# protocol/vdf

Hardware: AMD Instinct MI355X
Metric: MSM GPoints/s at 2^20 (Pallas, Pedersen-commitment MSM of Nova prove_step); prove_step/s in `prove_step` (higher is better)
Workload: dtype u32

## Files before the change

### bindings/rust/vdf-hip-sys/src/lib.rs

```rust
#![allow(non_camel_case_types, non_snake_case)]
use std::os::raw::{c_char, c_int, c_void};

#[repr(C)] pub struct VdfCtx { _private: [u8; 0] }
#[repr(C)] pub struct VdfBases { _private: [u8; 0] }
#[repr(C)] pub struct VdfShape { _private: [u8; 0] }
#[repr(C)] pub struct VdfMsmJob { _private: [u8; 0] }
#[repr(C)] pub struct VdfPp { _private: [u8; 0] }
#[repr(C)] pub struct VdfCircuits { _private: [u8; 0] }
#[repr(C)] pub struct VdfProof { _private: [u8; 0] }
#[repr(C)] pub struct VdfSnark { _private: [u8; 0] }
#[repr(C)] pub struct VdfCs { _private: [u8; 0] }

#[repr(C)] #[derive(Clone, Copy, Debug, PartialEq, Eq)] pub struct VdfFe { pub l: [u64; 4] }
#[repr(C)] #[derive(Clone, Copy, Debug, PartialEq, Eq)] pub struct VdfAffine { pub x: VdfFe, pub y: VdfFe }
#[repr(C)] #[derive(Clone, Copy, Debug, PartialEq, Eq)] pub struct VdfJac { pub x: VdfFe, pub y: VdfFe, pub z: VdfFe }
#[repr(C)] #[derive(Clone, Copy, Debug, PartialEq, Eq)] pub struct VdfState { pub x: VdfFe, pub y: VdfFe, pub i: VdfFe }
pub type VdfAllgatherFn = Option<unsafe extern "C" fn(user: *mut c_void, send: *const c_void, recv: *mut c_void, bytes: usize, stream: *mut c_void) -> c_int>;
#[repr(C)] #[derive(Clone, Copy)] pub struct VdfStepCircuit { pub arity: usize, pub synthesize: Option<unsafe extern "C" fn(self_: *mut c_void, cs: *mut VdfCs, z_in: *const u32, z_out: *mut u32) -> c_int>, pub self_: *mut c_void }
#[repr(C)] #[derive(Clone, Copy, Debug)] pub struct VdfNovaStepInfo { pub comm_W1: VdfAffine, pub X1: [VdfFe; 2], pub comm_T1: VdfAffine, pub comm_T2: VdfAffine, pub r1: [u64; 4], pub r2: [u64; 4] }
#[repr(C)] #[derive(Clone, Copy, Debug)] pub struct VdfNovaAugInputs { pub params: VdfFe, pub i: VdfFe, pub z0: [VdfFe; 3], pub zi: [VdfFe; 3], pub U_comm_W: VdfAffine, pub U_comm_E: VdfAffine, pub U_u: VdfFe, pub U_X: [VdfFe; 2], pub u_comm_W: VdfAffine, pub u_X: [VdfFe; 2], pub T: VdfAffine }
#[repr(C)] #[derive(Clone, Copy, Debug)] pub struct VdfKernelEvent { pub name: [c_char; 24], pub bytes: f64, pub start_ms: f64, pub end_ms: f64 }
#[repr(C)] #[derive(Clone, Copy, Debug)] pub struct VdfHipTuning { pub struct_size: u32, pub msm_direct: i32, pub direct_priority: i32, pub direct_fused: i32, pub light_priority: i32, pub accumulate_fill: i32, pub accumulate_lds: i32, pub slice_len: i32, pub part_bits: i32, pub reduction: i32, pub reduction_quads: i32, pub heavy_min: i32, pub giant_span: i32, pub nifs_lanes: i32, pub shim_cache: i32, pub nifs_fused: i32, pub fold_u128: i32, pub fixup_serial: i32, pub sort_staged: i32, pub glv: i32 }
#[repr(C)] #[derive(Clone, Copy, Debug)] pub struct VdfNovaTuning { pub struct_size: u32, pub flags: u32, pub digit_budget_bytes: u64, pub digit_window: i32, pub early_rows: i32, pub stencil: i32, pub small_window: i32, pub big_window: i32, pub packed_commit: i32, pub lookahead_early: i32, pub gate_accumulate: i32, pub fold_on_rows: i32, pub nifs_ahead: i32, pub early_row_parts: i32, pub lookahead_priority: i32, pub side_accumulate_fill: i32, pub verbose: i32, pub compress_queues: i32, pub rows_at_challenge: i32, pub fold_fused: i32 }
#[repr(C)] #[derive(Clone, Copy, Debug, PartialEq, Eq)] pub struct VdfNovaRoParams { pub struct_size: u32, pub family: i32, pub width: i32, pub full_rounds: i32, pub partial_rounds: i32, pub alpha: i32, pub challenge_bits: i32, pub hash_bits: i32 }
#[repr(C)] #[derive(Clone, Copy, Debug)] pub struct VdfIpaOpening { pub weight: VdfFe, pub k: c_int, pub log_m: c_int, pub lo: *const VdfFe, pub hi: *const VdfFe, pub pattern: *const VdfFe }

#[link(name = "vdf_hip")]
extern "C" {
    pub fn vdf_ctx_create(device_ids: *const c_int, n_devices: c_int, out: *mut *mut VdfCtx) -> c_int;
    pub fn vdf_ctx_destroy(ctx: *mut VdfCtx);
    pub fn vdf_ctx_create_pooled(device_ids: *const c_int, n_devices: c_int, role: c_int, out: *mut *mut VdfCtx) -> c_int;
    pub fn vdf_ctx_create_pooled_near(parent: *mut VdfCtx, role: c_int, out: *mut *mut VdfCtx) -> c_int;
    pub fn vdf_ctx_queue_info(ctx: *mut VdfCtx, pooled: *mut c_int, sharers: *mut c_int, device_streams: *mut c_int) -> c_int;
    pub fn vdf_ctx_set_stream(ctx: *mut VdfCtx, hip_stream: *mut c_void) -> c_int;
    pub fn vdf_ctx_get_stream(ctx: *mut VdfCtx) -> *mut c_void;
    pub fn vdf_ctx_set_async(ctx: *mut VdfCtx, async_: c_int) -> c_int;
    pub fn vdf_ctx_get_async(ctx: *mut VdfCtx, async_: *mut c_int) -> c_int;
    pub fn vdf_ctx_sync(ctx: *mut VdfCtx) -> c_int;
    pub fn vdf_ctx_device(ctx: *mut VdfCtx) -> c_int;
    pub fn vdf_last_error(ctx: *mut VdfCtx) -> *const c_char;
    pub fn vdf_bases_upload(ctx: *mut VdfCtx, curve: c_int, bases: *const VdfAffine, n: usize, out: *mut *mut VdfBases) -> c_int;
    pub fn vdf_bases_validate(ctx: *mut VdfCtx, bases: *const VdfBases, first_bad: *mut usize) -> c_int;
    pub fn vdf_bases_generate(ctx: *mut VdfCtx, curve: c_int, seed: u64, n: usize, out: *mut *mut VdfBases) -> c_int;
    pub fn vdf_bases_generate_range(ctx: *mut VdfCtx, curve: c_int, seed: u64, start: usize, n: usize, out: *mut *mut VdfBases) -> c_int;
    pub fn vdf_bases_generate_family(ctx: *mut VdfCtx, curve: c_int, family: c_int, seed: u64, start: usize, n: usize, out: *mut *mut VdfBases) -> c_int;
    pub fn vdf_bases_generate_label(ctx: *mut VdfCtx, curve: c_int, label: *const u8, label_len: usize, start: usize, n: usize, out: *mut *mut VdfBases) -> c_int;
    pub fn vdf_bases_precompute(ctx: *mut VdfCtx, bases: *mut VdfBases, window_bits: c_int, sets: c_int) -> c_int;
    pub fn vdf_bases_window(bases: *const VdfBases) -> c_int;
    pub fn vdf_bases_precompute_digits(ctx: *mut VdfCtx, bases: *mut VdfBases, window_bits: c_int, ranges: c_int, begin: *const usize, count: *const usize) -> c_int;
    pub fn vdf_digit_table_bytes(window_bits: c_int, generators: usize) -> usize;
    pub fn vdf_bases_table_bytes(bases: *const VdfBases) -> usize;
    pub fn vdf_bases_digit_window(bases: *const VdfBases) -> c_int;
    pub fn vdf_bases_digit_table_bytes(bases: *const VdfBases) -> usize;
    pub fn vdf_bases_download(ctx: *mut VdfCtx, bases: *const VdfBases, offset: usize, n: usize, out: *mut VdfAffine) -> c_int;
    pub fn vdf_bases_len(bases: *const VdfBases) -> usize;
    pub fn vdf_bases_device_ptr(bases: *const VdfBases) -> *const c_void;
    pub fn vdf_bases_free(bases: *mut VdfBases);
    pub fn vdf_msm(ctx: *mut VdfCtx, bases: *const VdfBases, offset: usize, scalars: *const VdfFe, n: usize, is_mont: c_int, out: *mut VdfJac) -> c_int;
    pub fn vdf_msm_batch(ctx: *mut VdfCtx, bases: *const VdfBases, k: c_int, offset: *const usize, scalars: *const *const VdfFe, n: *const usize, is_mont: c_int, out: *mut VdfJac) -> c_int;
    pub fn vdf_msm_job_begin(ctx: *mut VdfCtx, bases: *const VdfBases, k: c_int, offset: *const usize, n: *const usize, is_mont: c_int, out: *mut *mut VdfMsmJob) -> c_int;
    pub fn vdf_msm_job_push(job: *mut VdfMsmJob, g: c_int, scalars: *const VdfFe) -> c_int;
    pub fn vdf_msm_job_finish(job: *mut VdfMsmJob, out: *mut VdfJac) -> c_int;
    pub fn vdf_ctx_set_msm_window(ctx: *mut VdfCtx, window_bits: c_int) -> c_int;
    pub fn vdf_point_sum(ctx: *mut VdfCtx, curve: c_int, points: *const VdfJac, n: usize, out: *mut VdfJac) -> c_int;
    pub fn vdf_msm_sharded(ctx: *mut VdfCtx, shard_bases: *const VdfBases, offset: usize, shard_scalars: *const VdfFe, n: usize, is_mont: c_int, rank: c_int, world: c_int, gather: VdfAllgatherFn, user: *mut c_void, flags: c_int, partial: *mut VdfJac, gathered: *mut VdfJac, out: *mut VdfJac) -> c_int;
    pub fn vdf_msm_multi(ctxs: *const *mut VdfCtx, bases: *const *const VdfBases, offsets: *const usize, scalars: *const *const VdfFe, n: *const usize, k: c_int, is_mont: c_int, out: *mut VdfJac) -> c_int;
    pub fn vdf_ctx_set_timing(ctx: *mut VdfCtx, enable: c_int) -> c_int;
    pub fn vdf_msm_timing(ctx: *mut VdfCtx, ms: *mut f32, calls: *mut c_int) -> c_int;
    pub fn vdf_ctx_set_kernel_timing(ctx: *mut VdfCtx, enable: c_int) -> c_int;
    pub fn vdf_ctx_kernel_events(ctx: *mut VdfCtx, out: *mut VdfKernelEvent, cap: usize, n: *mut usize) -> c_int;
    pub fn mult_pippenger_pallas(out: *mut VdfJac, points: *const VdfAffine, npoints: usize, scalars: *const VdfFe, is_mont: bool);
    pub fn mult_pippenger_vesta(out: *mut VdfJac, points: *const VdfAffine, npoints: usize, scalars: *const VdfFe, is_mont: bool);
    pub fn vdf_shim_set_cache(entries: c_int) -> c_int;
    pub fn vdf_shape_create(ctx: *mut VdfCtx, field: c_int, num_cons: usize, num_cols: usize, rows: *const *const u32, cols: *const *const u32, vals: *const *const VdfFe, nnz: *const usize, out: *mut *mut VdfShape) -> c_int;
    pub fn vdf_shape_free(shape: *mut VdfShape);
    pub fn vdf_spmv3(ctx: *mut VdfCtx, shape: *const VdfShape, z: *const VdfFe, Az: *mut VdfFe, Bz: *mut VdfFe, Cz: *mut VdfFe) -> c_int;
    pub fn vdf_cross_term(ctx: *mut VdfCtx, field: c_int, Az1: *const VdfFe, Bz1: *const VdfFe, Cz1: *const VdfFe, Az2: *const VdfFe, Bz2: *const VdfFe, Cz2: *const VdfFe, u1: *const VdfFe, n: usize, T: *mut VdfFe) -> c_int;
    pub fn vdf_vec_is_zero(ctx: *mut VdfCtx, v: *const VdfFe, n: usize, is_zero: *mut c_int) -> c_int;
    pub fn vdf_axpy(ctx: *mut VdfCtx, field: c_int, a: *const VdfFe, r: *const VdfFe, b: *const VdfFe, n: usize, out: *mut VdfFe) -> c_int;
    pub fn vdf_minroot_witness(ctx: *mut VdfCtx, field: c_int, trace_xy: *const VdfFe, i0: *const VdfFe, t: u64, W_segment: *mut VdfFe) -> c_int;
    pub fn vdf_minroot_step_z(ctx: *mut VdfCtx, field: c_int, trace_xy: *const VdfFe, t: u64, z_in: *const VdfFe, i0: *const VdfFe, u: *const VdfFe, X: *const VdfFe, z: *mut VdfFe) -> c_int;
    pub fn vdf_minroot_step_z_packed(ctx: *mut VdfCtx, field: c_int, trace_xy: *const VdfFe, t: u64, z_in: *const VdfFe, i0: *const VdfFe, u: *const VdfFe, X: *const VdfFe, z: *mut VdfFe, w_packed: *mut VdfFe) -> c_int;
    pub fn vdf_minroot_step_segment(ctx: *mut VdfCtx, field: c_int, trace_xy: *const VdfFe, t: u64, i0: *const VdfFe, vars_per_round: c_int, out: *mut VdfFe) -> c_int;
    pub fn vdf_minroot_step_segment_packed(ctx: *mut VdfCtx, field: c_int, trace_xy: *const VdfFe, t: u64, i0: *const VdfFe, i_in: *const VdfFe, out: *mut VdfFe, packed: *mut VdfFe) -> c_int;
    pub fn vdf_nifs_cross_term(ctx: *mut VdfCtx, shape: *const VdfShape, z2: *const VdfFe, Az1: *const VdfFe, Bz1: *const VdfFe, Cz1: *const VdfFe, u1: *const VdfFe, Az2: *mut VdfFe, Bz2: *mut VdfFe, Cz2: *mut VdfFe, T: *mut VdfFe) -> c_int;
    pub fn vdf_nifs_cross_term_rows(ctx: *mut VdfCtx, shape: *const VdfShape, row_begin: usize, row_count: usize, part: c_int, z2: *const VdfFe, Az1: *const VdfFe, Bz1: *const VdfFe, Cz1: *const VdfFe, u1: *const VdfFe, Az2: *mut VdfFe, Bz2: *mut VdfFe, Cz2: *mut VdfFe, T: *mut VdfFe) -> c_int;
    pub fn vdf_nifs_cross_term_minroot(ctx: *mut VdfCtx, field: c_int, vars_per_round: c_int, t: u64, seg_begin: usize, one_col: usize, row_begin: usize, z2: *const VdfFe, Az1: *const VdfFe, Bz1: *const VdfFe, Cz1: *const VdfFe, u1: *const VdfFe, Az2: *mut VdfFe, Bz2: *mut VdfFe, Cz2: *mut VdfFe, T: *mut VdfFe) -> c_int;
    pub fn vdf_nifs_cross_term_minroot_fold(ctx: *mut VdfCtx, field: c_int, vars_per_round: c_int, t: u64, seg_begin: usize, one_col: usize, row_begin: usize, z2: *const VdfFe, r: *const VdfFe, Az1: *mut VdfFe, Bz1: *mut VdfFe, Cz1: *mut VdfFe, E1: *mut VdfFe, T_prev: *const VdfFe, u1: *const VdfFe, Az2: *mut VdfFe, Bz2: *mut VdfFe, Cz2: *mut VdfFe, T: *mut VdfFe) -> c_int;
    pub fn vdf_fold_many(ctx: *mut VdfCtx, field: c_int, r: *const VdfFe, k: c_int, acc: *const *mut VdfFe, add: *const *const VdfFe, n: *const usize) -> c_int;
    pub fn vdf_ctx_wait(ctx: *mut VdfCtx, other: *mut VdfCtx) -> c_int;
    pub fn vdf_ctx_mark(ctx: *mut VdfCtx, slot: c_int) -> c_int;
    pub fn vdf_ctx_sync_mark(ctx: *mut VdfCtx, slot: c_int) -> c_int;
    pub fn vdf_ctx_wait_mark(ctx: *mut VdfCtx, other: *mut VdfCtx, slot: c_int) -> c_int;
    pub fn vdf_ctx_gate_accumulate(ctx: *mut VdfCtx, other: *mut VdfCtx, slot: c_int) -> c_int;
    pub fn vdf_ctx_set_light_priority(ctx: *mut VdfCtx, priority: c_int) -> c_int;
    pub fn vdf_pair_table(ctx: *mut VdfCtx, field: c_int, lo: *const VdfFe, hi: *const VdfFe, k: c_int, out: *mut VdfFe) -> c_int;
    pub fn vdf_pair_table_pattern(ctx: *mut VdfCtx, field: c_int, lo: *const VdfFe, hi: *const VdfFe, k: c_int, pattern: *const VdfFe, log_m: c_int, out: *mut VdfFe) -> c_int;
    pub fn vdf_ipa_coefficients(ctx: *mut VdfCtx, field: c_int, ops: *const VdfIpaOpening, count: c_int, n: usize, out: *mut VdfFe) -> c_int;
    pub fn vdf_fold_halves(ctx: *mut VdfCtx, field: c_int, k: c_int, v: *const *mut VdfFe, c_lo: *const VdfFe, c_hi: *const VdfFe, n: usize) -> c_int;
    pub fn vdf_reduce(ctx: *mut VdfCtx, field: c_int, kind: c_int, tables: *const *const VdfFe, u: *const VdfFe, n: usize, out: *mut VdfFe) -> c_int;
    pub fn vdf_spmv3_t(ctx: *mut VdfCtx, shape: *const VdfShape, eq: *const VdfFe, rho: *const VdfFe, out: *mut VdfFe) -> c_int;
    pub fn vdf_reduce_batch(ctx: *mut VdfCtx, field: c_int, kind: c_int, count: usize, tables: *const *const VdfFe, u: *const VdfFe, n: usize, out: *mut VdfFe) -> c_int;
    pub fn vdf_fold_halves_batch(ctx: *mut VdfCtx, field: c_int, k: c_int, v: *const *mut VdfFe, c_lo: *const VdfFe, c_hi: *const VdfFe, n: usize) -> c_int;
    pub fn vdf_spmv3_t_batch(ctx: *mut VdfCtx, shape: *const VdfShape, count: usize, eq: *const *const VdfFe, rho: *const VdfFe, out: *const *mut VdfFe) -> c_int;
    pub fn vdf_lincomb_u128(ctx: *mut VdfCtx, field: c_int, count: c_int, v: *const *const VdfFe, n: *const usize, w: *const VdfFe, n_out: usize, out: *mut VdfFe) -> c_int;
    pub fn vdf_relaxed_residual_batch(ctx: *mut VdfCtx, shape: *const VdfShape, count: c_int, z: *const *const VdfFe, E: *const *const VdfFe, u: *const VdfFe, rho: *const VdfFe, out: *mut VdfFe) -> c_int;
    pub fn vdf_ipa_scalars(ctx: *mut VdfCtx, field: c_int, a: *const VdfFe, s: *const VdfFe, n: usize, nj: usize, sL: *mut VdfFe, sR: *mut VdfFe) -> c_int;
    pub fn vdf_scale_pattern(ctx: *mut VdfCtx, field: c_int, s: *mut VdfFe, n: usize, nj: usize, x_lo: *const VdfFe, x_hi: *const VdfFe) -> c_int;
    pub fn vdf_fe_mul(ctx: *mut VdfCtx, field: c_int, a: *const VdfFe, b: *const VdfFe, n: usize, out: *mut VdfFe) -> c_int;
    pub fn vdf_fe_to_mont(ctx: *mut VdfCtx, field: c_int, a: *const VdfFe, n: usize, out: *mut VdfFe) -> c_int;
    pub fn vdf_fe_from_mont(ctx: *mut VdfCtx, field: c_int, a: *const VdfFe, n: usize, out: *mut VdfFe) -> c_int;
    pub fn vdf_fe_mul_chain(ctx: *mut VdfCtx, field: c_int, a: *const VdfFe, n: usize, iters: c_int, out: *mut VdfFe) -> c_int;
    pub fn vdf_hip_tuning_get(out: *mut VdfHipTuning) -> c_int;
    pub fn vdf_hip_tuning_set(in_: *const VdfHipTuning) -> c_int;
    pub fn vdf_ctx_set_accumulate_fill(ctx: *mut VdfCtx, workgroups_per_cu: c_int) -> c_int;
    pub fn vdf_ctx_clock_probe(ctx: *mut VdfCtx, iters: c_int, shader_mhz: *mut f64, kernel_ms: *mut f64) -> c_int;
    pub fn vdf_dev_alloc(ctx: *mut VdfCtx, bytes: usize, out: *mut *mut c_void) -> c_int;
    pub fn vdf_dev_free(ctx: *mut VdfCtx, p: *mut c_void) -> c_int;
    pub fn vdf_dev_mem_info(ctx: *mut VdfCtx, free_bytes: *mut usize, total_bytes: *mut usize) -> c_int;
    pub fn vdf_dev_memcpy(ctx: *mut VdfCtx, dst: *mut c_void, src: *const c_void, bytes: usize) -> c_int;
    pub fn vdf_host_alloc(ctx: *mut VdfCtx, bytes: usize, out: *mut *mut c_void) -> c_int;
    pub fn vdf_host_free(ctx: *mut VdfCtx, p: *mut c_void) -> c_int;
    pub fn vdf_dev_memset(ctx: *mut VdfCtx, dst: *mut c_void, value: c_int, bytes: usize) -> c_int;
    pub fn vdf_version() -> *const c_char;
}

#[link(name = "vdf_nova")]
extern "C" {
    pub fn vdf_minroot_forward_step(field: c_int, mode: c_int, x: *const VdfFe, out: *mut VdfFe) -> c_int;
    pub fn vdf_minroot_inverse_step(field: c_int, x: *const VdfFe, out: *mut VdfFe) -> c_int;
    pub fn vdf_minroot_round(field: c_int, mode: c_int, s: *const VdfState, out: *mut VdfState) -> c_int;
// ... 81 lines not shown
```

### include/vdf_hip.h

```cpp
#ifndef VDF_HIP_H
#define VDF_HIP_H

#include <stdbool.h>
#include <stddef.h>
#include <stdint.h>

#ifdef __cplusplus
extern "C" {
#endif

typedef struct { uint64_t l[4]; } vdf_fe;
typedef struct { vdf_fe x, y; } vdf_affine;
typedef struct { vdf_fe x, y, z; } vdf_jac;

typedef struct vdf_ctx vdf_ctx;
typedef struct vdf_bases vdf_bases;
typedef struct vdf_shape vdf_shape;

enum {
  VDF_OK = 0,
  VDF_ERR_BAD_ARG = 1,
  VDF_ERR_BAD_LENGTH = 2,
  VDF_ERR_NONCANONICAL = 3,
  VDF_ERR_DEVICE = 4,
  VDF_ERR_OOM = 5,
  VDF_ERR_NO_DEVICE = 6
};

enum { VDF_CURVE_PALLAS = 0, VDF_CURVE_VESTA = 1 };
enum { VDF_FIELD_FP = 0, VDF_FIELD_FQ = 1 };

int  vdf_ctx_create(const int* device_ids, int n_devices, vdf_ctx** out);
void vdf_ctx_destroy(vdf_ctx* ctx);
#define VDF_QUEUE_CRITICAL 1
#define VDF_QUEUE_SIDE 2
int  vdf_ctx_create_pooled(const int* device_ids, int n_devices, int role, vdf_ctx** out);
int  vdf_ctx_create_pooled_near(vdf_ctx* parent, int role, vdf_ctx** out);
int  vdf_ctx_queue_info(vdf_ctx* ctx, int* pooled, int* sharers, int* device_streams);
int  vdf_ctx_set_stream(vdf_ctx* ctx, void* hip_stream);
void* vdf_ctx_get_stream(vdf_ctx* ctx);
int  vdf_ctx_set_async(vdf_ctx* ctx, int async);
int  vdf_ctx_get_async(vdf_ctx* ctx, int* async);
int  vdf_ctx_sync(vdf_ctx* ctx);
int  vdf_ctx_device(vdf_ctx* ctx);
const char* vdf_last_error(vdf_ctx* ctx);

int  vdf_bases_upload(vdf_ctx* ctx, int curve, const vdf_affine* bases, size_t n, vdf_bases** out);
int  vdf_bases_validate(vdf_ctx* ctx, const vdf_bases* bases, size_t* first_bad);
int  vdf_bases_generate(vdf_ctx* ctx, int curve, uint64_t seed, size_t n, vdf_bases** out);
int  vdf_bases_generate_range(vdf_ctx* ctx, int curve, uint64_t seed, size_t start, size_t n, vdf_bases** out);
enum { VDF_GENS_KNOWN_DLOG = 0, VDF_GENS_TRY_AND_INCREMENT = 1, VDF_GENS_LABEL_SHAKE = 2  };
int  vdf_bases_generate_family(vdf_ctx* ctx, int curve, int family, uint64_t seed, size_t start, size_t n, vdf_bases** out);
int  vdf_bases_generate_label(vdf_ctx* ctx, int curve, const uint8_t* label, size_t label_len, size_t start, size_t n, vdf_bases** out);
int  vdf_bases_precompute(vdf_ctx* ctx, vdf_bases* bases, int window_bits, int sets);
int  vdf_bases_window(const vdf_bases* bases);
int  vdf_bases_precompute_digits(vdf_ctx* ctx, vdf_bases* bases, int window_bits, int ranges, const size_t begin[], const size_t count[]);
size_t vdf_digit_table_bytes(int window_bits, size_t generators);
size_t vdf_bases_table_bytes(const vdf_bases* bases);
int  vdf_bases_digit_window(const vdf_bases* bases);
size_t vdf_bases_digit_table_bytes(const vdf_bases* bases);
int  vdf_bases_download(vdf_ctx* ctx, const vdf_bases* bases, size_t offset, size_t n, vdf_affine* out);
size_t vdf_bases_len(const vdf_bases* bases);
const void* vdf_bases_device_ptr(const vdf_bases* bases);
void vdf_bases_free(vdf_bases* bases);

int  vdf_msm(vdf_ctx* ctx, const vdf_bases* bases, size_t offset, const vdf_fe* scalars, size_t n,
             int is_mont, vdf_jac* out);
int  vdf_msm_batch(vdf_ctx* ctx, const vdf_bases* bases, int k, const size_t offset[], const vdf_fe* const scalars[],
                   const size_t n[], int is_mont, vdf_jac out[]);
typedef struct vdf_msm_job vdf_msm_job;
int  vdf_msm_job_begin(vdf_ctx* ctx, const vdf_bases* bases, int k, const size_t offset[], const size_t n[], int is_mont,
                       vdf_msm_job** out);
int  vdf_msm_job_push(vdf_msm_job* job, int g, const vdf_fe* scalars);
int  vdf_msm_job_finish(vdf_msm_job* job, vdf_jac out[]);
int  vdf_ctx_set_msm_window(vdf_ctx* ctx, int window_bits);
int  vdf_point_sum(vdf_ctx* ctx, int curve, const vdf_jac* points, size_t n, vdf_jac* out);
typedef int (*vdf_allgather_fn)(void* user, const void* send, void* recv, size_t bytes, void* stream);
enum { VDF_SHARDED_ALWAYS_GATHER = 1 };
int  vdf_msm_sharded(vdf_ctx* ctx, const vdf_bases* shard_bases, size_t offset, const vdf_fe* shard_scalars, size_t n, int is_mont,
                     int rank, int world, vdf_allgather_fn gather, void* user, int flags, vdf_jac* partial, vdf_jac* gathered,
                     vdf_jac* out);
int  vdf_msm_multi(vdf_ctx* const ctxs[], const vdf_bases* const bases[], const size_t offsets[], const vdf_fe* const scalars[],
                   const size_t n[], int k, int is_mont, vdf_jac* out);
int  vdf_ctx_set_timing(vdf_ctx* ctx, int enable);
int  vdf_msm_timing(vdf_ctx* ctx, float ms[4], int* calls);
typedef struct { char name[24]; double bytes; double start_ms, end_ms; } vdf_kernel_event;
int  vdf_ctx_set_kernel_timing(vdf_ctx* ctx, int enable);
int  vdf_ctx_kernel_events(vdf_ctx* ctx, vdf_kernel_event* out, size_t cap, size_t* n);

void mult_pippenger_pallas(vdf_jac* out, const vdf_affine* points, size_t npoints, const vdf_fe* scalars, bool is_mont);
void mult_pippenger_vesta(vdf_jac* out, const vdf_affine* points, size_t npoints, const vdf_fe* scalars, bool is_mont);
int  vdf_shim_set_cache(int entries);

int  vdf_shape_create(vdf_ctx* ctx, int field, size_t num_cons, size_t num_cols,
                      const uint32_t* const rows[3], const uint32_t* const cols[3],
                      const vdf_fe* const vals[3], const size_t nnz[3], vdf_shape** out);
void vdf_shape_free(vdf_shape* shape);
int  vdf_spmv3(vdf_ctx* ctx, const vdf_shape* shape, const vdf_fe* z, vdf_fe* Az, vdf_fe* Bz, vdf_fe* Cz);

int  vdf_cross_term(vdf_ctx* ctx, int field, const vdf_fe* Az1, const vdf_fe* Bz1, const vdf_fe* Cz1,
                    const vdf_fe* Az2, const vdf_fe* Bz2, const vdf_fe* Cz2, const vdf_fe* u1,
                    size_t n, vdf_fe* T);
int  vdf_vec_is_zero(vdf_ctx* ctx, const vdf_fe* v, size_t n, int* is_zero);
int  vdf_axpy(vdf_ctx* ctx, int field, const vdf_fe* a, const vdf_fe* r, const vdf_fe* b, size_t n, vdf_fe* out);

int  vdf_minroot_witness(vdf_ctx* ctx, int field, const vdf_fe* trace_xy, const vdf_fe* i0, uint64_t t,
                         vdf_fe* W_segment);


int  vdf_minroot_step_z(vdf_ctx* ctx, int field, const vdf_fe* trace_xy, uint64_t t, const vdf_fe z_in[3],
                        const vdf_fe* i0, const vdf_fe* u, const vdf_fe X[6], vdf_fe* z);
int  vdf_minroot_step_z_packed(vdf_ctx* ctx, int field, const vdf_fe* trace_xy, uint64_t t, const vdf_fe z_in[3],
                               const vdf_fe* i0, const vdf_fe* u, const vdf_fe X[6], vdf_fe* z, vdf_fe* w_packed);
int  vdf_minroot_step_segment(vdf_ctx* ctx, int field, const vdf_fe* trace_xy, uint64_t t, const vdf_fe* i0, int vars_per_round,
                              vdf_fe* out);
int  vdf_minroot_step_segment_packed(vdf_ctx* ctx, int field, const vdf_fe* trace_xy, uint64_t t, const vdf_fe* i0, const vdf_fe* i_in,
                                     vdf_fe* out, vdf_fe* packed);
int  vdf_nifs_cross_term(vdf_ctx* ctx, const vdf_shape* shape, const vdf_fe* z2, const vdf_fe* Az1, const vdf_fe* Bz1,
                         const vdf_fe* Cz1, const vdf_fe* u1, vdf_fe* Az2, vdf_fe* Bz2, vdf_fe* Cz2, vdf_fe* T);
#define VDF_ROWS_ALL 0
#define VDF_ROWS_INSIDE 1
#define VDF_ROWS_OUTSIDE 2
int  vdf_nifs_cross_term_rows(vdf_ctx* ctx, const vdf_shape* shape, size_t row_begin, size_t row_count, int part, const vdf_fe* z2,
                              const vdf_fe* Az1, const vdf_fe* Bz1, const vdf_fe* Cz1, const vdf_fe* u1, vdf_fe* Az2, vdf_fe* Bz2,
                              vdf_fe* Cz2, vdf_fe* T);
int  vdf_nifs_cross_term_minroot(vdf_ctx* ctx, int field, int vars_per_round, uint64_t t, size_t seg_begin, size_t one_col, size_t row_begin,
                                 const vdf_fe* z2, const vdf_fe* Az1, const vdf_fe* Bz1, const vdf_fe* Cz1, const vdf_fe* u1, vdf_fe* Az2,
                                 vdf_fe* Bz2, vdf_fe* Cz2, vdf_fe* T);
int  vdf_nifs_cross_term_minroot_fold(vdf_ctx* ctx, int field, int vars_per_round, uint64_t t, size_t seg_begin, size_t one_col,
                                      size_t row_begin, const vdf_fe* z2, const vdf_fe* r, vdf_fe* Az1, vdf_fe* Bz1, vdf_fe* Cz1,
                                      vdf_fe* E1, const vdf_fe* T_prev, const vdf_fe* u1, vdf_fe* Az2, vdf_fe* Bz2, vdf_fe* Cz2,
                                      vdf_fe* T);
int  vdf_fold_many(vdf_ctx* ctx, int field, const vdf_fe* r, int k, vdf_fe* const acc[], const vdf_fe* const add[],
                   const size_t n[]);
int  vdf_ctx_wait(vdf_ctx* ctx, vdf_ctx* other);
#define VDF_MARK_SLOTS 16
int  vdf_ctx_mark(vdf_ctx* ctx, int slot);
int  vdf_ctx_sync_mark(vdf_ctx* ctx, int slot);
int  vdf_ctx_wait_mark(vdf_ctx* ctx, vdf_ctx* other, int slot);
int  vdf_ctx_gate_accumulate(vdf_ctx* ctx, vdf_ctx* other, int slot);
int  vdf_ctx_set_light_priority(vdf_ctx* ctx, int priority);

int  vdf_pair_table(vdf_ctx* ctx, int field, const vdf_fe* lo, const vdf_fe* hi, int k, vdf_fe* out);
int  vdf_pair_table_pattern(vdf_ctx* ctx, int field, const vdf_fe* lo, const vdf_fe* hi, int k, const vdf_fe* pattern, int log_m,
                            vdf_fe* out);
typedef struct vdf_ipa_opening {
  vdf_fe weight;
  int k, log_m;
  const vdf_fe* lo;
  const vdf_fe* hi;
  const vdf_fe* pattern;
} vdf_ipa_opening;
int  vdf_ipa_coefficients(vdf_ctx* ctx, int field, const vdf_ipa_opening* ops, int count, size_t n, vdf_fe* out);
int  vdf_fold_halves(vdf_ctx* ctx, int field, int k, vdf_fe* const v[], const vdf_fe c_lo[], const vdf_fe c_hi[], size_t n);
enum { VDF_REDUCE_DOT = 0, VDF_REDUCE_QUADRATIC_ROUND = 1, VDF_REDUCE_R1CS_ROUND = 2, VDF_REDUCE_IPA_CROSS = 3 };
int  vdf_reduce(vdf_ctx* ctx, int field, int kind, const vdf_fe* const tables[], const vdf_fe* u, size_t n, vdf_fe* out);
int  vdf_spmv3_t(vdf_ctx* ctx, const vdf_shape* shape, const vdf_fe* eq, const vdf_fe* rho, vdf_fe* out);
int  vdf_reduce_batch(vdf_ctx* ctx, int field, int kind, size_t count, const vdf_fe* const tables[], const vdf_fe* u, size_t n,
                      vdf_fe* out);
int  vdf_fold_halves_batch(vdf_ctx* ctx, int field, int k, vdf_fe* const v[], const vdf_fe c_lo[], const vdf_fe c_hi[], size_t n);
int  vdf_spmv3_t_batch(vdf_ctx* ctx, const vdf_shape* shape, size_t count, const vdf_fe* const eq[], const vdf_fe rho[],
                       vdf_fe* const out[]);
int  vdf_lincomb_u128(vdf_ctx* ctx, int field, int count, const vdf_fe* const v[], const size_t n[], const vdf_fe w[],
                      size_t n_out, vdf_fe* out);
int  vdf_relaxed_residual_batch(vdf_ctx* ctx, const vdf_shape* shape, int count, const vdf_fe* const z[], const vdf_fe* const E[],
                                const vdf_fe u[], const vdf_fe rho[], vdf_fe* out);
int  vdf_ipa_scalars(vdf_ctx* ctx, int field, const vdf_fe* a, const vdf_fe* s, size_t n, size_t nj, vdf_fe* sL, vdf_fe* sR);
int  vdf_scale_pattern(vdf_ctx* ctx, int field, vdf_fe* s, size_t n, size_t nj, const vdf_fe* x_lo, const vdf_fe* x_hi);

int  vdf_fe_mul(vdf_ctx* ctx, int field, const vdf_fe* a, const vdf_fe* b, size_t n, vdf_fe* out);
int  vdf_fe_to_mont(vdf_ctx* ctx, int field, const vdf_fe* a, size_t n, vdf_fe* out);
int  vdf_fe_from_mont(vdf_ctx* ctx, int field, const vdf_fe* a, size_t n, vdf_fe* out);
int  vdf_fe_mul_chain(vdf_ctx* ctx, int field, const vdf_fe* a, size_t n, int iters, vdf_fe* out);
typedef struct vdf_hip_tuning {
  uint32_t struct_size;
  int32_t msm_direct;
  int32_t direct_priority;
  int32_t direct_fused;
  int32_t light_priority;
  int32_t accumulate_fill;
  int32_t accumulate_lds;
  int32_t slice_len;
  int32_t part_bits;
  int32_t reduction;
  int32_t reduction_quads;
  int32_t heavy_min;
  int32_t giant_span;
  int32_t nifs_lanes;
  int32_t shim_cache;
  int32_t nifs_fused;
  int32_t fold_u128;
  int32_t fixup_serial;
  int32_t sort_staged;
  int32_t glv;
} vdf_hip_tuning;
int  vdf_hip_tuning_get(vdf_hip_tuning* out);
int  vdf_hip_tuning_set(const vdf_hip_tuning* in);
int  vdf_ctx_set_accumulate_fill(vdf_ctx* ctx, int workgroups_per_cu);
int  vdf_ctx_clock_probe(vdf_ctx* ctx, int iters, double* shader_mhz, double* kernel_ms);
int  vdf_dev_alloc(vdf_ctx* ctx, size_t bytes, void** out);
int  vdf_dev_free(vdf_ctx* ctx, void* p);
int  vdf_dev_mem_info(vdf_ctx* ctx, size_t* free_bytes, size_t* total_bytes);
int  vdf_dev_memcpy(vdf_ctx* ctx, void* dst, const void* src, size_t bytes);
int  vdf_host_alloc(vdf_ctx* ctx, size_t bytes, void** out);
int  vdf_host_free(vdf_ctx* ctx, void* p);
int  vdf_dev_memset(vdf_ctx* ctx, void* dst, int value, size_t bytes);
const char* vdf_version(void);

#ifdef __cplusplus
}
#endif
#endif
```

### vdf_amd/_lib.py

```python
from __future__ import annotations

import ctypes as C
import os

_HERE = os.path.dirname(os.path.abspath(__file__))
LIB_PATH = os.environ.get("VDF_HIP_LIB") or os.path.join(_HERE, "libvdf_hip.so")
IS_OVERRIDE = bool(os.environ.get("VDF_HIP_LIB"))

VDF_OK, VDF_ERR_BAD_ARG, VDF_ERR_BAD_LENGTH, VDF_ERR_NONCANONICAL, VDF_ERR_DEVICE, VDF_ERR_OOM, VDF_ERR_NO_DEVICE = range(7)
CURVE_PALLAS, CURVE_VESTA = 0, 1
FIELD_FP, FIELD_FQ = 0, 1
GENS_KNOWN_DLOG, GENS_TRY_AND_INCREMENT = 0, 1

_vp, _sz, _i, _u64 = C.c_void_p, C.c_size_t, C.c_int, C.c_uint64
PROTOTYPES = {
    "vdf_ctx_create": (_i, [C.POINTER(_i), _i, C.POINTER(_vp)]),
    "vdf_ctx_destroy": (None, [_vp]),
    "vdf_ctx_create_pooled": (_i, [C.POINTER(_i), _i, _i, C.POINTER(_vp)]),
    "vdf_ctx_create_pooled_near": (_i, [_vp, _i, C.POINTER(_vp)]),
    "vdf_ctx_queue_info": (_i, [_vp, C.POINTER(_i), C.POINTER(_i), C.POINTER(_i)]),
    "vdf_ctx_set_stream": (_i, [_vp, _vp]),
    "vdf_ctx_get_stream": (_vp, [_vp]),
    "vdf_ctx_set_async": (_i, [_vp, _i]),
    "vdf_ctx_get_async": (_i, [_vp, C.POINTER(_i)]),
    "vdf_ctx_sync": (_i, [_vp]),
    "vdf_ctx_wait": (_i, [_vp, _vp]),
    "vdf_shim_set_cache": (_i, [_i]),
    "vdf_ctx_mark": (_i, [_vp, _i]),
    "vdf_ctx_sync_mark": (_i, [_vp, _i]),
    "vdf_ctx_wait_mark": (_i, [_vp, _vp, _i]),
    "vdf_ctx_gate_accumulate": (_i, [_vp, _vp, _i]),
    "vdf_ctx_set_light_priority": (_i, [_vp, _i]),
    "vdf_ctx_device": (_i, [_vp]),
    "vdf_last_error": (C.c_char_p, [_vp]),
    "vdf_bases_upload": (_i, [_vp, _i, _vp, _sz, C.POINTER(_vp)]),
    "vdf_bases_validate": (_i, [_vp, _vp, C.POINTER(_sz)]),
    "vdf_bases_generate": (_i, [_vp, _i, _u64, _sz, C.POINTER(_vp)]),
    "vdf_bases_generate_range": (_i, [_vp, _i, _u64, _sz, _sz, C.POINTER(_vp)]),
    "vdf_bases_generate_family": (_i, [_vp, _i, _i, _u64, _sz, _sz, C.POINTER(_vp)]),
    "vdf_bases_generate_label": (_i, [_vp, _i, _vp, _sz, _sz, _sz, C.POINTER(_vp)]),
    "vdf_bases_precompute": (_i, [_vp, _vp, _i, _i]),
    "vdf_bases_download": (_i, [_vp, _vp, _sz, _sz, _vp]),
    "vdf_bases_window": (_i, [_vp]),
    "vdf_bases_precompute_digits": (_i, [_vp, _vp, _i, _i, _vp, _vp]),
    "vdf_bases_digit_window": (_i, [_vp]),
    "vdf_bases_digit_table_bytes": (C.c_size_t, [_vp]),
    "vdf_digit_table_bytes": (C.c_size_t, [_i, _sz]),
    "vdf_bases_table_bytes": (C.c_size_t, [_vp]),
    "vdf_bases_len": (_sz, [_vp]),
    "vdf_bases_device_ptr": (_vp, [_vp]),
    "vdf_bases_free": (None, [_vp]),
    "vdf_msm": (_i, [_vp, _vp, _sz, _vp, _sz, _i, _vp]),
    "vdf_msm_batch": (_i, [_vp, _vp, _i, C.POINTER(_sz), C.POINTER(_vp), C.POINTER(_sz), _i, _vp]),
    "vdf_msm_job_begin": (_i, [_vp, _vp, _i, C.POINTER(_sz), C.POINTER(_sz), _i, C.POINTER(_vp)]),
    "vdf_msm_job_push": (_i, [_vp, _i, _vp]),
    "vdf_msm_job_finish": (_i, [_vp, _vp]),
    "vdf_ctx_set_msm_window": (_i, [_vp, _i]),
    "vdf_point_sum": (_i, [_vp, _i, _vp, _sz, _vp]),
    "vdf_ctx_set_timing": (_i, [_vp, _i]),
    "vdf_msm_sharded": (_i, [_vp, _vp, _sz, _vp, _sz, _i, _i, _i, _vp, _vp, _i, _vp, _vp, _vp]),
    "vdf_msm_multi": (_i, [C.POINTER(_vp), C.POINTER(_vp), C.POINTER(_sz), C.POINTER(_vp), C.POINTER(_sz), _i, _i, _vp]),
    "vdf_msm_timing": (_i, [_vp, C.POINTER(C.c_float), C.POINTER(_i)]),
    "vdf_ctx_set_kernel_timing": (_i, [_vp, _i]),
    "vdf_ctx_kernel_events": (_i, [_vp, _vp, _sz, C.POINTER(_sz)]),
    "mult_pippenger_pallas": (None, [_vp, _vp, _sz, _vp, C.c_bool]),
    "mult_pippenger_vesta": (None, [_vp, _vp, _sz, _vp, C.c_bool]),
    "vdf_shape_create": (_i, [_vp, _i, _sz, _sz, C.POINTER(_vp), C.POINTER(_vp), C.POINTER(_vp), C.POINTER(_sz), C.POINTER(_vp)]),
    "vdf_shape_free": (None, [_vp]),
    "vdf_spmv3": (_i, [_vp, _vp, _vp, _vp, _vp, _vp]),
    "vdf_cross_term": (_i, [_vp, _i, _vp, _vp, _vp, _vp, _vp, _vp, _vp, _sz, _vp]),
    "vdf_axpy": (_i, [_vp, _i, _vp, _vp, _vp, _sz, _vp]),
    "vdf_minroot_witness": (_i, [_vp, _i, _vp, _vp, _u64, _vp]),
    "vdf_minroot_step_z": (_i, [_vp, _i, _vp, _u64, _vp, _vp, _vp, _vp, _vp]),
    "vdf_minroot_step_z_packed": (_i, [_vp, _i, _vp, _u64, _vp, _vp, _vp, _vp, _vp, _vp]),
    "vdf_minroot_step_segment": (_i, [_vp, _i, _vp, _u64, _vp, _i, _vp]),
    "vdf_minroot_step_segment_packed": (_i, [_vp, _i, _vp, _u64, _vp, _vp, _vp, _vp]),
    "vdf_vec_is_zero": (_i, [_vp, _vp, _sz, C.POINTER(C.c_int)]),
    "vdf_nifs_cross_term": (_i, [_vp, _vp, _vp, _vp, _vp, _vp, _vp, _vp, _vp, _vp, _vp]),
    "vdf_nifs_cross_term_rows": (_i, [_vp, _vp, C.c_size_t, C.c_size_t, C.c_int, _vp, _vp, _vp, _vp, _vp, _vp, _vp, _vp, _vp]),
    "vdf_nifs_cross_term_minroot": (_i, [_vp, _i, _i, _u64, _sz, _sz, _sz, _vp, _vp, _vp, _vp, _vp, _vp, _vp, _vp, _vp]),
    "vdf_nifs_cross_term_minroot_fold": (_i, [_vp, _i, _i, _u64, _sz, _sz, _sz, _vp, _vp, _vp, _vp, _vp, _vp, _vp, _vp, _vp, _vp, _vp, _vp]),
    "vdf_fold_many": (_i, [_vp, _i, _vp, _i, C.POINTER(_vp), C.POINTER(_vp), C.POINTER(_sz)]),
    "vdf_pair_table": (_i, [_vp, _i, _vp, _vp, _i, _vp]),
    "vdf_pair_table_pattern": (_i, [_vp, _i, _vp, _vp, _i, _vp, _i, _vp]),
    "vdf_ipa_coefficients": (_i, [_vp, _i, _vp, _i, _sz, _vp]),
    "vdf_fold_halves": (_i, [_vp, _i, _i, C.POINTER(_vp), _vp, _vp, _sz]),
    "vdf_reduce": (_i, [_vp, _i, _i, C.POINTER(_vp), _vp, _sz, _vp]),
    "vdf_spmv3_t": (_i, [_vp, _vp, _vp, _vp, _vp]),
    "vdf_reduce_batch": (_i, [_vp, _i, _i, _sz, C.POINTER(_vp), _vp, _sz, _vp]),
    "vdf_fold_halves_batch": (_i, [_vp, _i, _i, C.POINTER(_vp), _vp, _vp, _sz]),
    "vdf_spmv3_t_batch": (_i, [_vp, _vp, _sz, C.POINTER(_vp), _vp, C.POINTER(_vp)]),
    "vdf_lincomb_u128": (_i, [_vp, _i, _i, C.POINTER(_vp), C.POINTER(_sz), _vp, _sz, _vp]),
    "vdf_relaxed_residual_batch": (_i, [_vp, _vp, _i, C.POINTER(_vp), C.POINTER(_vp), _vp, _vp, _vp]),
    "vdf_ipa_scalars": (_i, [_vp, _i, _vp, _vp, _sz, _sz, _vp, _vp]),
    "vdf_scale_pattern": (_i, [_vp, _i, _vp, _sz, _sz, _vp, _vp]),
    "vdf_fe_mul": (_i, [_vp, _i, _vp, _vp, _sz, _vp]),
    "vdf_fe_to_mont": (_i, [_vp, _i, _vp, _sz, _vp]),
    "vdf_fe_from_mont": (_i, [_vp, _i, _vp, _sz, _vp]),
    "vdf_fe_mul_chain": (_i, [_vp, _i, _vp, _sz, _i, _vp]),
    "vdf_hip_tuning_get": (_i, [_vp]),
    "vdf_hip_tuning_set": (_i, [_vp]),
    "vdf_ctx_set_accumulate_fill": (_i, [_vp, _i]),
    "vdf_ctx_clock_probe": (_i, [_vp, _i, C.POINTER(C.c_double), C.POINTER(C.c_double)]),
    "vdf_dev_alloc": (_i, [_vp, _sz, C.POINTER(_vp)]),
    "vdf_dev_free": (_i, [_vp, _vp]),
    "vdf_dev_mem_info": (_i, [_vp, C.POINTER(_sz), C.POINTER(_sz)]),
    "vdf_dev_memcpy": (_i, [_vp, _vp, _vp, _sz]),
    "vdf_dev_memset": (_i, [_vp, _vp, _i, _sz]),
    "vdf_host_alloc": (_i, [_vp, _sz, C.POINTER(_vp)]),
    "vdf_host_free": (_i, [_vp, _vp]),
    "vdf_version": (C.c_char_p, []),
}


def load() -> C.CDLL:
    if not os.path.exists(LIB_PATH):
        raise ImportError(
            f"{LIB_PATH} is missing: build it with `python -c 'import __graft_entry__ as g; g.build()'` "
            "(hipcc --offload-arch=gfx950). vdf_amd has no CPU fallback.")
    if IS_OVERRIDE:
        import sys
        print("vdf_amd: VDF_HIP_LIB override in force: loading %s (not the shipped library)" % LIB_PATH, file=sys.stderr)
    lib = C.CDLL(LIB_PATH, mode=C.RTLD_GLOBAL)
    for name, (res, args) in PROTOTYPES.items():
        fn = getattr(lib, name)
        fn.restype = res
# ... 6 lines not shown
```

### vdf_amd/csrc/abi.hip

```cpp
#include <algorithm>
#include <cstring>
#include <cstdio>
#include <cstdlib>
#include <thread>
#include <functional>
#include <map>
#include <array>
#include <new>
#include <memory>
#include <atomic>
#include <deque>
#include <mutex>
#include <initializer_list>
#include <utility>
#include "internal.h"
#include "fe.cuh"

using vdf::Status;

namespace {

thread_local std::string g_create_err;
std::mutex g_default_mu;
vdf_ctx* g_default_ctx = nullptr;
// ... 9 lines not shown

bool ptr_is_device(const void* p) {
  if (!p) return false;
  if (ptr_is_mapped_host(p)) return true;
  hipPointerAttribute_t a;
  hipError_t e = hipPointerGetAttributes(&a, p);
  if (e != hipSuccess) { (void)hipGetLastError(); return false; }
  return a.type == hipMemoryTypeDevice || a.type == hipMemoryTypeManaged;
}

struct Staging {
  vdf_ctx* ctx;
  std::vector<void*> temps;
  struct Out { void* host; void* dev; size_t bytes; };
  std::vector<Out> outs;
  Out pinned_out{nullptr, nullptr, 0};
  bool any_host = false;
  size_t small_used = 0;
  explicit Staging(vdf_ctx* c) : ctx(c) {}
  ~Staging() { for (void* t : temps) (void)hipFree(t); }
  Status temp(size_t bytes, void** t) {
    const size_t need = (bytes + 255) / 256 * 256;
    if (need <= 1024 && ctx->small_pool && small_used + need <= vdf_ctx::SMALL_POOL_BYTES) {
      *t = vdf::bytes_of(ctx->small_pool) + small_used;
      small_used += need;
      return Status{};
    }
    VDF_TRY_HIP(hipMalloc(t, bytes));
    temps.push_back(*t);
    return Status{};
  }
  Status in(const void* p, size_t bytes, const void** dev) {
    if (bytes == 0) { *dev = p; return Status{}; }
    if (!p) return Status{VDF_ERR_BAD_ARG, "null input pointer"};
    if (ptr_is_device(p)) { *dev = p; return Status{}; }
    any_host = true;
    void* t = nullptr;
    VDF_TRY(temp(bytes, &t));
    VDF_TRY_HIP(hipMemcpyAsync(t, p, bytes, hipMemcpyHostToDevice, ctx->stream));
    *dev = t;
    return Status{};
  }
  Status out(void* p, size_t bytes, void** dev) {
    if (bytes == 0) { *dev = p; return Status{}; }
    if (!p) return Status{VDF_ERR_BAD_ARG, "null output pointer"};
    if (ptr_is_device(p)) { *dev = p; return Status{}; }
    any_host = true;
    if (bytes <= vdf_ctx::PINNED_OUT_BYTES && ctx->h_out && !pinned_out.host) {
      pinned_out = {p, ctx->h_out, bytes};
      *dev = ctx->h_out_dev;
      return Status{};
    }
    void* t = nullptr;
    VDF_TRY(temp(bytes, &t));
    outs.push_back({p, t, bytes});
    *dev = t;
    return Status{};
  }
  Status finish() {
    for (auto& o : outs) VDF_TRY_HIP(hipMemcpyAsync(o.host, o.dev, o.bytes, hipMemcpyDeviceToHost, ctx->stream));
    if (any_host || !ctx->async) VDF_TRY_HIP(hipStreamSynchronize(ctx->stream));
    if (pinned_out.host) std::memcpy(pinned_out.host, pinned_out.dev, pinned_out.bytes);
    return Status{};
  }
};

int fail(vdf_ctx* ctx, const Status& s) {
  if (ctx) ctx->err = s.msg; else g_create_err = s.msg;
  return s.code;
}


std::once_flag g_tune_once;
std::mutex g_tune_mu;
std::deque<vdf_hip_tuning> g_tune_snapshots;
std::atomic<const vdf_hip_tuning*> g_tune{nullptr};
vdf_hip_tuning tuning_defaults() {
  vdf_hip_tuning t{};
  t.struct_size = (uint32_t)sizeof(vdf_hip_tuning);
  t.msm_direct = 1; t.direct_priority = 2; t.direct_fused = 1; t.light_priority = 3; t.accumulate_fill = 0;
  t.accumulate_lds = 0; t.slice_len = 0; t.part_bits = -1; t.reduction = 1; t.reduction_quads = 0; t.heavy_min = 0;
  t.giant_span = 0; t.nifs_lanes = 0; t.shim_cache = 0; t.nifs_fused = 1; t.fold_u128 = 1;
  t.fixup_serial = 1; t.sort_staged = 1; t.glv = 1;
  return t;
}
bool tuning_valid(const vdf_hip_tuning& t) {
  auto in = [](int v, int lo, int hi) { return v >= lo && v <= hi; };
  return in(t.msm_direct, 0, 1) && in(t.direct_priority, 0, 3) && in(t.direct_fused, 0, 1) && in(t.light_priority, 0, 3) &&
         in(t.accumulate_fill, 0, 3) && in(t.accumulate_lds, 0, 65536) && in(t.slice_len, 0, 65536) && in(t.part_bits, -1, 19) &&
         in(t.reduction, 0, 1) && (t.reduction_quads == 0 || in(t.reduction_quads, 64, 65536)) &&
         (t.heavy_min == 0 || in(t.heavy_min, 1, 4096)) && (t.giant_span == 0 || in(t.giant_span, 16, 1 << 20)) &&
         (t.nifs_lanes == 0 || t.nifs_lanes == 1 || t.nifs_lanes == 4 || t.nifs_lanes == 8) && in(t.shim_cache, 0, 64) &&
         in(t.nifs_fused, 0, 1) && in(t.fold_u128, 0, 1) && in(t.fixup_serial, 0, 1) && in(t.sort_staged, 0, 1) && in(t.glv, 0, 1);
}
void tuning_publish(const vdf_hip_tuning& t) {
  g_tune_snapshots.push_back(t);
  g_tune_snapshots.back().struct_size = (uint32_t)sizeof(vdf_hip_tuning);
  g_tune.store(&g_tune_snapshots.back(), std::memory_order_release);
}
void tuning_from_env() {
  vdf_hip_tuning t = tuning_defaults();
  const struct { const char* name; int32_t* field; } vars[] = {
      {"VDF_MSM_DIRECT", &t.msm_direct}, {"VDF_MSM_DIRECT_PRIO", &t.direct_priority}, {"VDF_MSM_DIRECT_FUSED", &t.direct_fused},
      {"VDF_MSM_LIGHT_PRIO", &t.light_priority}, {"VDF_MSM_ACC_WG", &t.accumulate_fill}, {"VDF_MSM_ACC_LDS", &t.accumulate_lds},
      {"VDF_MSM_L", &t.slice_len}, {"VDF_MSM_PB", &t.part_bits}, {"VDF_MSM_RED", &t.reduction},
      {"VDF_MSM_RED_QUADS", &t.reduction_quads}, {"VDF_MSM_HEAVY_MIN", &t.heavy_min}, {"VDF_MSM_GIANT_SPAN", &t.giant_span},
      {"VDF_NIFS_LANES", &t.nifs_lanes}, {"VDF_SHIM_CACHE", &t.shim_cache}, {"VDF_NIFS_FUSED", &t.nifs_fused}, {"VDF_FOLD_U128", &t.fold_u128},
      {"VDF_MSM_FIXUP_SERIAL", &t.fixup_serial}, {"VDF_MSM_SORT_STAGED", &t.sort_staged}, {"VDF_MSM_GLV", &t.glv}};
  for (const auto& v : vars) {
    const char* e = std::getenv(v.name);
    if (!e || !*e) continue;
    const int32_t old = *v.field;
    *v.field = (int32_t)std::atol(e);
    if (!tuning_valid(t)) *v.field = old;
  }
  std::lock_guard<std::mutex> lock(g_tune_mu);
  tuning_publish(t);
}
}
namespace vdf {
thread_local KSink* tl_ksink = nullptr;
const vdf_hip_tuning& tuning() {
  std::call_once(g_tune_once, tuning_from_env);
  return *g_tune.load(std::memory_order_acquire);
}
}
extern "C" int vdf_hip_tuning_get(vdf_hip_tuning* out) {
  if (!out) return VDF_ERR_BAD_ARG;
  *out = vdf::tuning();
  return VDF_OK;
}
extern "C" int vdf_hip_tuning_set(const vdf_hip_tuning* in) {
  if (!in || in->struct_size != sizeof(vdf_hip_tuning) || !tuning_valid(*in)) return VDF_ERR_BAD_ARG;
  (void)vdf::tuning();
  std::lock_guard<std::mutex> lock(g_tune_mu);
  tuning_publish(*in);
  return VDF_OK;
}
namespace {
struct SinkScope {
  vdf::KSink* prev;
  explicit SinkScope(vdf_ctx* c) : prev(vdf::tl_ksink) { vdf::tl_ksink = c->ktiming ? &c->ksink : nullptr; }
  ~SinkScope() { vdf::tl_ksink = prev; }
};

template <class F>
int guarded(vdf_ctx* ctx, F&& body) {
  if (!ctx) { g_create_err = "null context"; return VDF_ERR_BAD_ARG; }
  try {
    std::lock_guard<std::mutex> lock(ctx->mu);
    SinkScope sink_scope(ctx);
    hipError_t e = hipSetDevice(ctx->device);
    if (e != hipSuccess) return fail(ctx, vdf::hip_status(e, "hipSetDevice"));
    Status s = body();
    if (!s.ok()) return fail(ctx, s);
    return VDF_OK;
  } catch (const std::bad_alloc&) {
    ctx->err = "host allocation failed";
    return VDF_ERR_OOM;
  } catch (const std::exception& ex) {
    ctx->err = ex.what();
    return VDF_ERR_DEVICE;
  } catch (...) {
    ctx->err = "unknown failure";
    return VDF_ERR_DEVICE;
  }
}

Status ensure_ws(vdf_ctx* ctx, size_t bytes) {
  if (ctx->ws_bytes >= bytes) return Status{};
  if (ctx->job_open) return Status{VDF_ERR_BAD_ARG, "the MSM workspace cannot grow while a job is open on this context"};
  if (ctx->ws) { VDF_TRY_HIP(hipStreamSynchronize(ctx->stream)); (void)hipFree(ctx->ws); ctx->ws = nullptr; ctx->ws_bytes = 0; }
  VDF_TRY_HIP(hipMalloc(&ctx->ws, bytes));
  ctx->ws_bytes = bytes;
  return Status{};
}

constexpr size_t DIRECT_MAX_SCALARS = (size_t)1 << 17;
bool direct_enabled() { return vdf::tuning().msm_direct != 0; }

constexpr size_t GLV_MIN_POINTS = 1u << 12;
#ifndef VDF_GLV_MAX_LOG2
#define VDF_GLV_MAX_LOG2 21
#endif
constexpr size_t GLV_MAX_POINTS = (size_t)1 << VDF_GLV_MAX_LOG2;
Status msm_core(vdf_ctx* ctx, const vdf_bases* bases, int groups, const size_t* offset, const vdf_fe* const* scalars,
                const size_t* n, int is_mont, vdf_jac* out) {
  if (!bases || !out || !offset || !scalars || !n) return Status{VDF_ERR_BAD_ARG, "null bases/out/arrays"};
  if (groups < 1 || groups > vdf::MSM_MAX_GROUPS) return Status{VDF_ERR_BAD_ARG, "1..4 MSMs per batch"};
  if (ctx->job_open) return Status{VDF_ERR_BAD_ARG, "an MSM job is open on this context: its workspace is in use"};
  if (bases->ctx != ctx && bases->ctx->device != ctx->device) return Status{VDF_ERR_BAD_ARG, "bases live on another device"};
  size_t ntot = 0, nmax = 0;
  for (int g = 0; g < groups; ++g) {
    if (offset[g] > bases->n || n[g] > bases->n - offset[g]) return Status{VDF_ERR_BAD_LENGTH, "offset + n exceeds the generator table"};
    ntot += n[g];
    if (n[g] > nmax) nmax = n[g];
  }
  if (ntot >= (1ull << 27)) return Status{VDF_ERR_BAD_LENGTH, "n too large (max 2^27 - 1 points per call)"};
  Staging st(ctx);
  void* d_out = nullptr;
  VDF_TRY(st.out(out, groups * sizeof(vdf_jac), &d_out));
  if (ntot == 0) {
    VDF_TRY_HIP(hipMemsetAsync(d_out, 0, groups * sizeof(vdf_jac), ctx->stream));
    return st.finish();
  }
  const void* d_scalars[vdf::MSM_MAX_GROUPS] = {nullptr, nullptr, nullptr, nullptr};
  for (int g = 0; g < groups; ++g) VDF_TRY(st.in(scalars[g], n[g] * sizeof(vdf_fe), &d_scalars[g]));
  if (bases->d_digits && ctx->msm_window == 0 && ntot <= DIRECT_MAX_SCALARS && direct_enabled()) {
    size_t slot0[vdf::MSM_MAX_GROUPS] = {0, 0, 0, 0};
    bool inside = true;
    for (int g = 0; g < groups && inside; ++g) {
      int r = 0;
      while (r < bases->dg_ranges && !(offset[g] >= bases->dg_begin[r] && offset[g] + n[g] <= bases->dg_begin[r] + bases->dg_count[r])) ++r;
      if (r == bases->dg_ranges) inside = n[g] == 0;
      else slot0[g] = bases->dg_slot0[r] + (offset[g] - bases->dg_begin[r]);
    }
    if (inside) {
      VDF_TRY(ensure_ws(ctx, vdf::direct_ws_bytes(groups, n, bases->dg_c, ctx->num_cus)));
      hipEvent_t* dev = nullptr;
      vdf_ctx::TimedCall dtc;
      int have = 0;
      struct Giveback { vdf_ctx* c; vdf_ctx::TimedCall* t; int* have; bool armed; ~Giveback() { if (armed) for (int i = 0; i < *have; ++i) c->ev_pool.push_back(t->ev[i]); } }
          giveback{ctx, &dtc, &have, true};
      if (ctx->timing) {
        for (int i = 0; i < 4; ++i) {
          if (!ctx->ev_pool.empty()) { dtc.ev[i] = ctx->ev_pool.back(); ctx->ev_pool.pop_back(); }
          else VDF_TRY_HIP(hipEventCreate(&dtc.ev[i]));
          have = i + 1;
        }
        dev = dtc.ev;
        VDF_TRY_HIP(hipEventRecord(dev[0], ctx->stream));
        VDF_TRY_HIP(hipEventRecord(dev[1], ctx->stream));
      }
      if (!ctx->direct_arrived) {
        VDF_TRY_HIP(hipMalloc(reinterpret_cast<void**>(&ctx->direct_arrived), 64));
        VDF_TRY_HIP(hipMemsetAsync(ctx->direct_arrived, 0, 64, ctx->stream));
      }
      VDF_TRY(vdf::msm_direct_run(bases->curve, groups, n, slot0, d_scalars, is_mont != 0, bases->dg_c, ctx->num_cus, bases->d_digits, ctx->ws, d_out,
                                  ctx->direct_arrived, ctx->stream));
      if (dev) {
        VDF_TRY_HIP(hipEventRecord(dev[2], ctx->stream));
        VDF_TRY_HIP(hipEventRecord(dev[3], ctx->stream));
        ctx->timed.push_back(dtc);
      }
      giveback.armed = false;
      return st.finish();
    }
  }
  vdf::MsmPlan plan;
  const char* pts;
  if (bases->d_table && (ctx->msm_window == 0 || ctx->msm_window == bases->tbl_c)) {
    if (!vdf::msm_plan_feasible(groups, bases->tbl_c, bases->tbl_sets))
      return Status{VDF_ERR_BAD_ARG, "a batch this wide does not fit the sort under this table's window and bucket sets: fewer MSMs per call"};
    plan = vdf::msm_make_plan(groups, n, offset, bases->tbl_c, bases->tbl_sets, bases->tbl_tables, ctx->num_cus, ctx->acc_fill);
    plan.tstride = (uint32_t)bases->n;
    pts = vdf::cbytes_of(bases->d_table);
  } else if (groups == 1 && offset[0] == 0 && n[0] == bases->n && n[0] >= GLV_MIN_POINTS && n[0] <= GLV_MAX_POINTS && ctx->msm_window == 0 &&
             vdf::tuning().glv) {
    vdf_bases* mb = const_cast<vdf_bases*>(bases);
    const void* pts2 = nullptr;
    if (bases->ephemeral) {
      const size_t pbytes = 2 * bases->n * sizeof(vdf_affine);
      if (ctx->glv_pts_bytes < pbytes) {
        VDF_TRY_HIP(hipStreamSynchronize(ctx->stream));
        if (ctx->glv_pts) (void)hipFree(ctx->glv_pts);
        ctx->glv_pts = nullptr; ctx->glv_pts_bytes = 0;
        VDF_TRY_HIP(hipMalloc(&ctx->glv_pts, pbytes));
        ctx->glv_pts_bytes = pbytes;
      }
      VDF_TRY(vdf::glv_points(bases->curve, bases->d_pts, bases->n, ctx->glv_pts, ctx->stream));
      pts2 = ctx->glv_pts;
    } else {
      std::lock_guard<std::mutex> lock(mb->glv_mu);
      if (!mb->d_pts2) {
        void* p2 = nullptr;
        VDF_TRY_HIP(hipMalloc(&p2, 2 * bases->n * sizeof(vdf_affine)));
        Status sg = vdf::glv_points(bases->curve, bases->d_pts, bases->n, p2, ctx->stream);
        if (sg.code == VDF_OK && hipStreamSynchronize(ctx->stream) != hipSuccess) sg = Status{VDF_ERR_DEVICE, "glv points"};
        if (sg.code != VDF_OK) { (void)hipFree(p2); return sg; }
        mb->d_pts2 = p2;
      }
      pts2 = mb->d_pts2;
    }
    const size_t need = 2 * n[0] * sizeof(vdf_fe);
    if (ctx->glv_bytes < need) {
      VDF_TRY_HIP(hipStreamSynchronize(ctx->stream));
      if (ctx->glv_scalars) (void)hipFree(ctx->glv_scalars);
      ctx->glv_scalars = nullptr; ctx->glv_bytes = 0;
      VDF_TRY_HIP(hipMalloc(&ctx->glv_scalars, need));
      ctx->glv_bytes = need;
    }
    VDF_TRY(vdf::glv_split(bases->curve, d_scalars[0], n[0], is_mont != 0, ctx->glv_scalars, ctx->stream));
    d_scalars[0] = ctx->glv_scalars;
    is_mont = 0;
    const size_t n2[1] = {2 * n[0]}, off2[1] = {0};
    const int ca = vdf::msm_auto_window(n2[0]);
    const int c = ca >= 15 ? 16 : 13;
    plan = vdf::msm_make_plan(1, n2, off2, c, 0, 0, ctx->num_cus, ctx->acc_fill, 132);
    plan.tstride = 0;
    pts = vdf::cbytes_of(pts2);
    ntot = n2[0];
  } else {
    int c = ctx->msm_window ? ctx->msm_window : vdf::msm_auto_window(nmax);
    while (c > 4 && !vdf::msm_plan_feasible(groups, c, 0)) --c;
    plan = vdf::msm_make_plan(groups, n, offset, c, 0, 0, ctx->num_cus, ctx->acc_fill);
    plan.tstride = 0;
    pts = vdf::cbytes_of(bases->d_pts);
  }
  if ((size_t)plan.tstride * plan.tables + bases->n >= (1ull << 31)) return Status{VDF_ERR_BAD_LENGTH, "table index exceeds 31 bits"};
  if ((uint64_t)ntot * plan.windows >= 0xFFF00000ull) return Status{VDF_ERR_BAD_LENGTH, "n * windows exceeds 32-bit entry positions"};
  VDF_TRY(ensure_ws(ctx, plan.ws_bytes));
  hipEvent_t* ev = nullptr;
  vdf_ctx::TimedCall tc;
  if (ctx->timing) {
    for (int i = 0; i < 4; ++i) {
      if (!ctx->ev_pool.empty()) { tc.ev[i] = ctx->ev_pool.back(); ctx->ev_pool.pop_back(); }
      else VDF_TRY_HIP(hipEventCreate(&tc.ev[i]));
    }
    ev = tc.ev;
  }
  hipEvent_t gate = ctx->acc_gate;
  ctx->acc_gate = nullptr;
  VDF_TRY(vdf::msm_run(bases->curve, plan, pts, d_scalars, is_mont != 0, ctx->ws, d_out, ctx->stream, ev, nullptr, gate, std::min(ctx->light_prio, (int)vdf::tuning().light_priority)));
  if (ev) ctx->timed.push_back(tc);
  return st.finish();
}

vdf_ctx* default_ctx() {
  std::lock_guard<std::mutex> lock(g_default_mu);
  if (!g_default_ctx) {
    int dev = 0;
    if (vdf_ctx_create(&dev, 1, &g_default_ctx) != VDF_OK) g_default_ctx = nullptr;
  }
  return g_default_ctx;
// ... 325 lines not shown
    if (n && !bases) return Status{VDF_ERR_BAD_ARG, "null bases"};
    vdf_bases* b = new vdf_bases();
    b->ctx = ctx; b->curve = curve; b->n = n;
    if (n) {
      hipError_t e = hipMalloc(&b->d_pts, n * sizeof(vdf_affine));
      if (e != hipSuccess) { delete b; return vdf::hip_status(e, "hipMalloc(bases)"); }
      e = hipMemcpyAsync(b->d_pts, bases, n * sizeof(vdf_affine), hipMemcpyDefault, ctx->stream);
      if (e == hipSuccess) e = hipStreamSynchronize(ctx->stream);
      if (e != hipSuccess) { (void)hipFree(b->d_pts); delete b; return vdf::hip_status(e, "upload bases"); }
    }
    *out = b;
    return Status{};
  });
}

int vdf_bases_validate(vdf_ctx* ctx, const vdf_bases* bases, size_t* first_bad) {
  return guarded(ctx, [&]() -> Status {
    if (!bases || (bases->ctx != ctx && bases->ctx->device != ctx->device)) return Status{VDF_ERR_BAD_ARG, "bad bases handle"};
    if (first_bad) *first_bad = 0;
    if (bases->n == 0) return Status{};
    uint32_t* d_flags = reinterpret_cast<uint32_t*>(ctx->small_pool);
    const uint32_t init[2] = {0u, 0xFFFFFFFFu};
    VDF_TRY_HIP(hipMemcpyAsync(d_flags, init, sizeof(init), hipMemcpyHostToDevice, ctx->stream));
    VDF_TRY(vdf::bases_validate(bases->curve, bases->d_pts, bases->n, d_flags, ctx->stream));
    uint32_t res[2];
    VDF_TRY_HIP(hipMemcpyAsync(res, d_flags, sizeof(res), hipMemcpyDeviceToHost, ctx->stream));
    VDF_TRY_HIP(hipStreamSynchronize(ctx->stream));
    if (res[0] == 0) return Status{};
    if (first_bad) *first_bad = res[1];
    if (res[0] & 1u) return Status{VDF_ERR_NONCANONICAL, "a generator coordinate is not a canonical field element"};
    return Status{VDF_ERR_BAD_ARG, "a generator is neither the identity nor a point of the curve"};
  });
}

int vdf_bases_generate(vdf_ctx* ctx, int curve, uint64_t seed, size_t n, vdf_bases** out) {
  return vdf_bases_generate_range(ctx, curve, seed, 0, n, out);
}

int vdf_bases_generate_range(vdf_ctx* ctx, int curve, uint64_t seed, size_t start, size_t n, vdf_bases** out) {
  return vdf_bases_generate_family(ctx, curve, VDF_GENS_KNOWN_DLOG, seed, start, n, out);
}

int vdf_bases_generate_family(vdf_ctx* ctx, int curve, int family, uint64_t seed, size_t start, size_t n, vdf_bases** out) {
  return guarded(ctx, [&]() -> Status {
    if (!out) return Status{VDF_ERR_BAD_ARG, "null out"};
    *out = nullptr;
    VDF_TRY(vdf::check_curve(curve));
    if (n >= (1ull << 31)) return Status{VDF_ERR_BAD_LENGTH, "too many bases"};
    vdf_bases* b = new vdf_bases();
    b->ctx = ctx; b->curve = curve; b->n = n;
    if (n) {
      hipError_t e = hipMalloc(&b->d_pts, n * sizeof(vdf_affine));
      if (e != hipSuccess) { delete b; return vdf::hip_status(e, "hipMalloc(bases)"); }
      Status s = vdf::bases_generate(curve, family, seed, start, n, b->d_pts, ctx->stream);
      if (s.ok()) s = vdf::hip_status(hipStreamSynchronize(ctx->stream), "bases_generate");
      if (!s.ok()) { (void)hipFree(b->d_pts); delete b; return s; }
    }
    *out = b;
    return Status{};
  });
}

int vdf_bases_generate_label(vdf_ctx* ctx, int curve, const uint8_t* label, size_t label_len, size_t start, size_t n, vdf_bases** out) {
  return guarded(ctx, [&]() -> Status {
    if (!out) return Status{VDF_ERR_BAD_ARG, "null out"};
    *out = nullptr;
    VDF_TRY(vdf::check_curve(curve));
    if (n >= (1ull << 31)) return Status{VDF_ERR_BAD_LENGTH, "too many bases"};
    if (label_len > 64 || (label_len && !label)) return Status{VDF_ERR_BAD_LENGTH, "label of at most 64 bytes"};
    vdf_bases* b = new vdf_bases();
    b->ctx = ctx; b->curve = curve; b->n = n;
    if (n) {
      hipError_t e = hipMalloc(&b->d_pts, n * sizeof(vdf_affine));
      if (e != hipSuccess) { delete b; return vdf::hip_status(e, "hipMalloc(bases)"); }
      Status s = vdf::bases_generate_label(curve, label, label_len, start, n, b->d_pts, ctx->stream);
      if (s.ok()) s = vdf::hip_status(hipStreamSynchronize(ctx->stream), "bases_generate_label");
      if (!s.ok()) { (void)hipFree(b->d_pts); delete b; return s; }
    }
    *out = b;
    return Status{};
  });
}

int vdf_bases_precompute(vdf_ctx* ctx, vdf_bases* bases, int window_bits, int sets) {
  return guarded(ctx, [&]() -> Status {
    if (!bases || bases->ctx != ctx) return Status{VDF_ERR_BAD_ARG, "bad bases handle"};
    if (window_bits == 0) window_bits = bases->n >= ((size_t)1 << 22) ? 20 : (bases->n >= ((size_t)1 << 19) ? 17 : 16);
    if (window_bits < 4 || window_bits > 20) return Status{VDF_ERR_BAD_ARG, "window_bits must be 0 (recommended) or 4..20"};
    const int windows = (256 + window_bits - 1) / window_bits;
    if (sets <= 0) sets = 1;
    if (sets > windows) sets = windows;
    while (windows % sets) ++sets;
    const int tables = windows / sets;
    if (bases->d_table) { (void)hipFree(bases->d_table); bases->d_table = nullptr; }
    bases->tbl_c = bases->tbl_sets = bases->tbl_tables = 0;
    if (bases->n == 0 || tables == 1) return Status{};
    VDF_TRY_HIP(hipMalloc(&bases->d_table, (size_t)tables * bases->n * sizeof(vdf_affine)));
    Status s = vdf::bases_precompute(bases->curve, bases->d_pts, bases->n, window_bits, sets, tables, bases->d_table, ctx->stream);
    if (s.ok()) s = vdf::hip_status(hipStreamSynchronize(ctx->stream), "bases_precompute");
    if (!s.ok()) { (void)hipFree(bases->d_table); bases->d_table = nullptr; return s; }
    bases->tbl_c = window_bits; bases->tbl_sets = sets; bases->tbl_tables = tables;
    return Status{};
  });
}

int vdf_bases_precompute_digits(vdf_ctx* ctx, vdf_bases* bases, int window_bits, int ranges, const size_t begin[], const size_t count[]) {
  return guarded(ctx, [&]() -> Status {
    if (!bases || bases->ctx != ctx) return Status{VDF_ERR_BAD_ARG, "bad bases handle"};
    if (bases->d_digits) { (void)hipFree(bases->d_digits); bases->d_digits = nullptr; }
    bases->dg_c = bases->dg_ranges = 0;
    if (ranges == 0) return Status{};
    if (ranges < 0 || ranges > 4 || !begin || !count) return Status{VDF_ERR_BAD_ARG, "1..4 generator ranges"};
    if (window_bits == 0) window_bits = 10;
    if (window_bits < 4 || window_bits > 12) return Status{VDF_ERR_BAD_ARG, "digit window must be 0 (recommended) or 4..12"};
    size_t slots = 0;
    for (int r = 0; r < ranges; ++r) {
      if (begin[r] > bases->n || count[r] > bases->n - begin[r]) return Status{VDF_ERR_BAD_LENGTH, "range exceeds the generator table"};
      for (int q = 0; q < r; ++q)
        if (begin[r] < begin[q] + count[q] && begin[q] < begin[r] + count[r]) return Status{VDF_ERR_BAD_ARG, "generator ranges overlap"};
      slots += count[r];
    }
    if (slots == 0) return Status{};
    const int W = vdf::direct_windows(window_bits);
    if (slots * W >= (1ull << 31)) return Status{VDF_ERR_BAD_LENGTH, "too many generators for a digit table"};
    const size_t bytes = ((slots * W) << (window_bits - 1)) * sizeof(vdf_affine);
    size_t free_b = 0, total_b = 0;
    VDF_TRY_HIP(hipMemGetInfo(&free_b, &total_b));
    if (bytes + ((size_t)1 << 30) > free_b) return Status{VDF_ERR_OOM, "the digit table does not fit the free device memory"};
    if (hipMalloc(&bases->d_digits, bytes) != hipSuccess) {
      (void)hipGetLastError();
      bases->d_digits = nullptr;
      return Status{VDF_ERR_OOM, "the digit table could not be allocated"};
    }
    size_t slot0 = 0;
    Status s{};
    for (int r = 0; r < ranges && s.ok(); ++r) {
      s = vdf::digits_build(bases->curve, bases->d_pts, begin[r], count[r], slot0, window_bits, bases->d_digits, ctx->stream);
      bases->dg_begin[r] = begin[r]; bases->dg_count[r] = count[r]; bases->dg_slot0[r] = slot0;
      slot0 += count[r];
    }
    if (!s.ok()) { (void)hipFree(bases->d_digits); bases->d_digits = nullptr; return s; }
    bases->dg_c = window_bits; bases->dg_ranges = ranges; bases->dg_bytes = bytes;
    return Status{};
  });
}

int vdf_bases_digit_window(const vdf_bases* bases) { return bases && bases->d_digits ? bases->dg_c : 0; }
size_t vdf_bases_digit_table_bytes(const vdf_bases* bases) { return bases && bases->d_digits ? bases->dg_bytes : 0; }

int vdf_bases_window(const vdf_bases* bases) { return bases && bases->d_table ? bases->tbl_c : 0; }
size_t vdf_bases_table_bytes(const vdf_bases* bases) { return bases && bases->d_table ? (size_t)bases->tbl_tables * bases->n * 64 : 0; }
size_t vdf_digit_table_bytes(int window_bits, size_t generators) {
  if (window_bits < 4 || window_bits > 12) return 0;
  return generators * (size_t)vdf::direct_windows(window_bits) * ((size_t)64 << (window_bits - 1));
}

int vdf_bases_download(vdf_ctx* ctx, const vdf_bases* bases, size_t offset, size_t n, vdf_affine* out) {
  return guarded(ctx, [&]() -> Status {
    if (!bases || bases->ctx != ctx || (n && !out)) return Status{VDF_ERR_BAD_ARG, "bad arguments"};
    if (offset > bases->n || n > bases->n - offset) return Status{VDF_ERR_BAD_LENGTH, "range exceeds the generator table"};
    if (n == 0) return Status{};
    VDF_TRY_HIP(hipMemcpyAsync(out, vdf::cbytes_of(bases->d_pts) + offset * 64, n * 64, hipMemcpyDefault, ctx->stream));
    VDF_TRY_HIP(hipStreamSynchronize(ctx->stream));
    return Status{};
  });
}

size_t vdf_bases_len(const vdf_bases* bases) { return bases ? bases->n : 0; }
const void* vdf_bases_device_ptr(const vdf_bases* bases) { return bases ? bases->d_pts : nullptr; }

void vdf_bases_free(vdf_bases* bases) {
  if (!bases) return;
  if (bases->ctx) {
    std::lock_guard<std::mutex> lock(bases->ctx->mu);
    (void)hipSetDevice(bases->ctx->device);
    (void)hipStreamSynchronize(bases->ctx->stream);
    if (bases->d_pts) (void)hipFree(bases->d_pts);
    if (bases->d_table) (void)hipFree(bases->d_table);
    if (bases->d_digits) (void)hipFree(bases->d_digits);
    if (bases->d_pts2) (void)hipFree(bases->d_pts2);
  }
  delete bases;
}

int vdf_msm(vdf_ctx* ctx, const vdf_bases* bases, size_t offset, const vdf_fe* scalars, size_t n, int is_mont, vdf_jac* out) {
  return guarded(ctx, [&]() -> Status { return msm_core(ctx, bases, 1, &offset, &scalars, &n, is_mont, out); });
}

int vdf_msm_batch(vdf_ctx* ctx, const vdf_bases* bases, int k, const size_t offset[], const vdf_fe* const scalars[],
                  const size_t n[], int is_mont, vdf_jac out[]) {
  return guarded(ctx, [&]() -> Status { return msm_core(ctx, bases, k, offset, scalars, n, is_mont, out); });
}

struct vdf_msm_job {
  vdf_ctx* ctx = nullptr;
  const vdf_bases* bases = nullptr;
  int k = 0, is_mont = 0;
  vdf::MsmPlan plan[vdf::MSM_MAX_GROUPS];
  size_t ws_off[vdf::MSM_MAX_GROUPS] = {0, 0, 0, 0};
  size_t tail_off = 0;
  bool pushed[vdf::MSM_MAX_GROUPS] = {false, false, false, false};
  const char* pts = nullptr;
};

int vdf_msm_job_begin(vdf_ctx* ctx, const vdf_bases* bases, int k, const size_t offset[], const size_t n[], int is_mont,
                      vdf_msm_job** out) {
  return guarded(ctx, [&]() -> Status {
    if (!out) return Status{VDF_ERR_BAD_ARG, "null out"};
    *out = nullptr;
    if (!bases || !offset || !n) return Status{VDF_ERR_BAD_ARG, "null argument"};
    if (k < 1 || k > vdf::MSM_MAX_GROUPS) return Status{VDF_ERR_BAD_ARG, "1..4 vectors per job"};
    if (bases->ctx != ctx && bases->ctx->device != ctx->device) return Status{VDF_ERR_BAD_ARG, "bases live on another device"};
    if (ctx->job_open) return Status{VDF_ERR_BAD_ARG, "another MSM job is open on this context"};
    if (!bases->d_table || bases->tbl_sets != 1)
      return Status{VDF_ERR_BAD_ARG, "MSM jobs need a fixed-base table with one bucket set (vdf_bases_precompute(c, 1))"};
    std::unique_ptr<vdf_msm_job> job(new vdf_msm_job());
    job->ctx = ctx; job->bases = bases; job->k = k; job->is_mont = is_mont;
    job->pts = vdf::cbytes_of(bases->d_table);
    size_t off = 0;
    for (int g = 0; g < k; ++g) {
      if (offset[g] > bases->n || n[g] > bases->n - offset[g]) return Status{VDF_ERR_BAD_LENGTH, "offset + n exceeds the generator table"};
      if (n[g] == 0 || n[g] >= (1ull << 27)) return Status{VDF_ERR_BAD_LENGTH, "every vector of a job needs 1 .. 2^27 - 1 elements"};
      job->plan[g] = vdf::msm_make_plan(1, &n[g], &offset[g], bases->tbl_c, 1, bases->tbl_tables, ctx->num_cus, ctx->acc_fill);
      job->plan[g].tstride = (uint32_t)bases->n;
      if ((uint64_t)n[g] * job->plan[g].windows >= 0xFFF00000ull) return Status{VDF_ERR_BAD_LENGTH, "n * windows exceeds 32-bit entry positions"};
      job->ws_off[g] = off;
      off += (job->plan[g].ws_bytes + 255) / 256 * 256;
    }
    if ((size_t)bases->n * (bases->tbl_tables + 1) >= (1ull << 31)) return Status{VDF_ERR_BAD_LENGTH, "table index exceeds 31 bits"};
    job->tail_off = off;
    off += vdf::msm_tail_ws_bytes(k, 1, job->plan[0].nbk);
    VDF_TRY(ensure_ws(ctx, off));
    for (int g = 0; g < k; ++g) {
      if (!ctx->side[g]) VDF_TRY_HIP(hipStreamCreateWithFlags(&ctx->side[g], hipStreamNonBlocking));
      if (!ctx->side_go[g]) VDF_TRY_HIP(hipEventCreateWithFlags(&ctx->side_go[g], hipEventDisableTiming));
      if (!ctx->side_done[g]) VDF_TRY_HIP(hipEventCreateWithFlags(&ctx->side_done[g], hipEventDisableTiming));
    }
    ctx->job_open = true;
    *out = job.release();
    return Status{};
  });
}

int vdf_msm_job_push(vdf_msm_job* job, int g, const vdf_fe* scalars) {
  if (!job) return VDF_ERR_BAD_ARG;
  vdf_ctx* ctx = job->ctx;
  return guarded(ctx, [&]() -> Status {
    if (g < 0 || g >= job->k) return Status{VDF_ERR_BAD_ARG, "vector index out of range"};
    if (job->pushed[g]) return Status{VDF_ERR_BAD_ARG, "vector already pushed"};
    if (!ptr_is_device(scalars)) return Status{VDF_ERR_BAD_ARG, "job vectors live in device memory"};
    VDF_TRY_HIP(hipEventRecord(ctx->side_go[g], ctx->stream));
    VDF_TRY_HIP(hipStreamWaitEvent(ctx->side[g], ctx->side_go[g], 0));
    const void* sc[vdf::MSM_MAX_GROUPS] = {scalars, nullptr, nullptr, nullptr};
    char* ws = vdf::bytes_of(ctx->ws);
    char* buckets = ws + job->tail_off + (size_t)g * job->plan[g].nbk * 128;
    VDF_TRY(vdf::msm_run(job->bases->curve, job->plan[g], job->pts, sc, job->is_mont != 0, ws + job->ws_off[g], nullptr,
                         ctx->side[g], nullptr, buckets));
    VDF_TRY_HIP(hipEventRecord(ctx->side_done[g], ctx->side[g]));
    job->pushed[g] = true;
    return Status{};
  });
}
// ... 1038 lines not shown
```

### vdf_amd/csrc/internal.h

```cpp
#pragma once
#include <hip/hip_runtime.h>
#include <stdint.h>
#include <memory>
#include <mutex>
#include <string>
#include <type_traits>
#include <vector>
#include "../../include/vdf_hip.h"
#include "pasta_constants.h"

namespace vdf {
struct KRecord { const char* name; double bytes; hipEvent_t e0, e1; };
struct KSink {
  std::vector<KRecord> rec;
  std::vector<hipEvent_t> pool;
};
extern thread_local KSink* tl_ksink;
struct KTimer {
  hipStream_t s; KSink* k; KRecord r;
  KTimer(hipStream_t st, const char* name, double bytes) : s(st), k(tl_ksink) {
    if (!k) return;
    r.name = name; r.bytes = bytes; r.e0 = r.e1 = nullptr;
    for (hipEvent_t* e : {&r.e0, &r.e1}) {
      if (!k->pool.empty()) { *e = k->pool.back(); k->pool.pop_back(); }
      else if (hipEventCreate(e) != hipSuccess) { (void)hipGetLastError(); *e = nullptr; }
    }
    if (r.e0 && r.e1) (void)hipEventRecord(r.e0, s); else k = nullptr;
  }
  ~KTimer() {
    if (!k) return;
    (void)hipEventRecord(r.e1, s);
    k->rec.push_back(r);
  }
  KTimer(const KTimer&) = delete;
  KTimer& operator=(const KTimer&) = delete;
};
}

namespace vdf { const vdf_hip_tuning& tuning(); }

struct vdf_queue_family {
  int device = 0;
  static constexpr int N = 3;
  hipStream_t s[N] = {};
  bool used[N] = {};
  ~vdf_queue_family();
};

struct vdf_ctx {
  int device = 0;
  hipStream_t stream = nullptr;
  int pool_slot = -1;
  std::shared_ptr<vdf_queue_family> family;
  int family_idx = -1;
  bool foreign_stream = false;
  bool async = false;
  int msm_window = 0;
  std::mutex mu;
  std::string err;
  void* ws = nullptr;
  size_t ws_bytes = 0;
  void* d_out = nullptr;
  static constexpr size_t SMALL_POOL_BYTES = 16 * 1024;
  void* small_pool = nullptr;
  static constexpr size_t PINNED_OUT_BYTES = 256;
  void* h_out = nullptr;
  void* h_out_dev = nullptr;
  int num_cus = 256;
  bool timing = false;
  bool ktiming = false;
  vdf::KSink ksink;
  struct TimedCall { hipEvent_t ev[4]; };
  std::vector<TimedCall> timed;
  std::vector<hipEvent_t> ev_pool;
  hipEvent_t wait_ev = nullptr;
  hipEvent_t marks[VDF_MARK_SLOTS] = {};
  hipStream_t side[4] = {nullptr, nullptr, nullptr, nullptr};
  hipEvent_t side_go[4] = {nullptr, nullptr, nullptr, nullptr}, side_done[4] = {nullptr, nullptr, nullptr, nullptr};
  bool job_open = false;
  void* reduce_scratch = nullptr;
  void* ipa_host = nullptr;
  void* ipa_dev = nullptr;
  size_t ipa_cap = 0;
  hipEvent_t ipa_copied = nullptr;
  int acc_fill = 0;
  int light_prio = 3;
  hipEvent_t acc_gate = nullptr;
  void* glv_scalars = nullptr;
  size_t glv_bytes = 0;
  void* glv_pts = nullptr;
  size_t glv_pts_bytes = 0;
  uint32_t* direct_arrived = nullptr;
};

struct vdf_bases {
  vdf_ctx* ctx = nullptr;
  int curve = 0;
  size_t n = 0;
  void* d_pts = nullptr;
  void* d_pts2 = nullptr;
  std::mutex glv_mu;
  bool ephemeral = false;
  int tbl_c = 0, tbl_sets = 0, tbl_tables = 0;
  void* d_table = nullptr;
  int dg_c = 0, dg_ranges = 0;
  size_t dg_begin[4] = {0, 0, 0, 0}, dg_count[4] = {0, 0, 0, 0}, dg_slot0[4] = {0, 0, 0, 0};
  void* d_digits = nullptr;
  size_t dg_bytes = 0;
};

struct vdf_shape {
  vdf_ctx* ctx = nullptr;
  int field = 0;
  size_t num_cons = 0, num_cols = 0;
  size_t nnz[3] = {0, 0, 0};
  uint32_t* d_rowptr[3] = {nullptr, nullptr, nullptr};
  uint32_t* d_col[3] = {nullptr, nullptr, nullptr};
  uint32_t* d_coef[3] = {nullptr, nullptr, nullptr};
  void* d_dict = nullptr;
  size_t dict_len = 0;
  uint32_t* d_t_colptr = nullptr;
  uint32_t* d_t_row = nullptr;
  uint32_t* d_t_cm = nullptr;
  uint32_t* d_t_heavy = nullptr;
  size_t t_nheavy = 0, t_nbig = 0;
  uint32_t* d_long = nullptr;
  size_t n_long = 0;
  uint32_t* d_long_rowlist = nullptr;
  size_t n_long_rowlist = 0;
  std::vector<uint64_t> h_nnz_prefix;
  std::vector<uint32_t> h_long_rows;
};
#define VDF_LONG_ROW 8

namespace vdf {

struct Status {
  int code = VDF_OK;
  std::string msg;
  bool ok() const { return code == VDF_OK; }
};

inline Status hip_status(hipError_t e, const char* what) {
  Status s;
  if (e != hipSuccess) {
    s.code = (e == hipErrorOutOfMemory) ? VDF_ERR_OOM : VDF_ERR_DEVICE;
    s.msg = std::string(what) + ": " + hipGetErrorString(e);
  }
  return s;
}

#define VDF_TRY_HIP(expr)                                   \
  do {                                                      \
    hipError_t e__ = (expr);                                \
    if (e__ != hipSuccess) return ::vdf::hip_status(e__, #expr); \
  } while (0)
#define VDF_TRY(expr)                 \
  do {                                \
    ::vdf::Status s__ = (expr);       \
    if (!s__.ok()) return s__;        \
  } while (0)

template <class P> struct FieldTag { using type = P; };
template <class Tag> using tag_t = typename Tag::type;
constexpr int field_id(FieldTag<FpParams>) { return VDF_FIELD_FP; }
constexpr int field_id(FieldTag<FqParams>) { return VDF_FIELD_FQ; }

template <class F, class... Tags> Status dispatch_body(F&& f, Tags... tags) {
  if constexpr (std::is_void<decltype(f(tags...))>::value) {
    f(tags...);
    VDF_TRY_HIP(hipGetLastError());
    return Status{};
  } else {
    return f(tags...);
  }
}

template <class F> Status with_field(int field, F&& f) {
  if (field == VDF_FIELD_FP) return dispatch_body(f, FieldTag<FpParams>{});
  if (field == VDF_FIELD_FQ) return dispatch_body(f, FieldTag<FqParams>{});
  return Status{VDF_ERR_BAD_ARG, "unknown field"};
}
template <class F> Status with_curve(int curve, F&& f) {
  if (curve == VDF_CURVE_PALLAS) return dispatch_body(f, FieldTag<FpParams>{}, FieldTag<FqParams>{});
  if (curve == VDF_CURVE_VESTA) return dispatch_body(f, FieldTag<FqParams>{}, FieldTag<FpParams>{});
  return Status{VDF_ERR_BAD_ARG, "unknown curve"};
}
inline Status check_field(int field) { return with_field(field, [](auto) { return Status{}; }); }
inline Status check_curve(int curve) { return with_curve(curve, [](auto, auto) { return Status{}; }); }
inline int field_of_curve_scalar(int curve) {
  int field = -1;
  (void)with_curve(curve, [&](auto, auto scalar) { field = field_id(scalar); return Status{}; });
  return field;
}
template <int... Vs, class F> Status with_int(int v, const char* otherwise, F&& f) {
  Status st{VDF_ERR_BAD_ARG, otherwise};
  (void)(... || (v == Vs && ((st = dispatch_body(f, std::integral_constant<int, Vs>{})), true)));
  return st;
}
template <class F> Status with_bool(bool v, F&& f) {
  return v ? dispatch_body(f, std::true_type{}) : dispatch_body(f, std::false_type{});
}

inline const char* cbytes_of(const void* p) { return static_cast<const char*>(p); }
inline char* bytes_of(void* p) { return static_cast<char*>(p); }
inline dim3 grid_for(size_t n) { return dim3((unsigned)((n + 255) / 256)); }

constexpr int MSM_MAX_GROUPS = 4;
struct MsmPlan {
  int groups = 1;
  uint32_t gn[MSM_MAX_GROUPS] = {0, 0, 0, 0};
  uint32_t goff[MSM_MAX_GROUPS] = {0, 0, 0, 0};
  uint32_t gblk_end[MSM_MAX_GROUPS] = {0, 0, 0, 0};
  uint32_t n = 0;
  int c = 0;
  int windows = 0;
  bool signed_scalars = false;
  int sets = 0;
  int gsets = 0;
  int tables = 0;
  uint32_t nbk = 0;
  int pb = 0, fb = 0;
  uint32_t bins = 0;
  uint32_t chA = 0;
  uint32_t nblkA = 0;
  uint32_t L = 0;
  uint32_t Lfixed = 0;
  uint32_t slots = 0;
  uint32_t nthreads = 0;
  uint32_t tstride = 0;
  size_t ws_bytes = 0;
};
MsmPlan msm_make_plan(int groups, const size_t* n, const size_t* offsets, int c, int sets, int tables, int num_cus, int acc_fill = 0,
                      int scalar_bits = 256);
Status glv_points(int curve, const void* d_pts, size_t n, void* d_out, hipStream_t stream);
Status glv_split(int curve, const void* d_scalars, size_t n, bool is_mont, void* d_out, hipStream_t stream);
inline MsmPlan msm_make_plan(size_t n, int c, int sets, int tables, int num_cus) {
  const size_t zero = 0;
  return msm_make_plan(1, &n, &zero, c, sets, tables, num_cus);
}
int msm_auto_window(size_t n);
bool msm_plan_feasible(int groups, int c, int sets);
Status msm_run(int curve, const MsmPlan& plan, const void* d_points, const void* const* d_scalars, bool is_mont,
               void* ws, void* d_out, hipStream_t stream, hipEvent_t* ev = nullptr, void* ext_bucket_acc = nullptr,
               hipEvent_t acc_gate = nullptr, int prio = 3);
size_t msm_tail_ws_bytes(int groups, int sets, uint32_t nbk);
Status msm_tail(int curve, int c, int sets, int groups, uint32_t nbk, void* tail_ws, void* d_out, hipStream_t stream, int prio = 3);
Status bases_generate(int curve, int family, uint64_t seed, size_t start, size_t n, void* d_pts, hipStream_t stream);
int direct_windows(int c);
Status digits_build(int curve, const void* d_pts, size_t first, size_t nslots, size_t slot0, int c, void* d_digits, hipStream_t stream);
size_t direct_ws_bytes(int groups, const size_t* n, int c, int num_cus);
Status msm_direct_run(int curve, int groups, const size_t* n, const size_t* slot0, const void* const* d_scalars, bool is_mont,
                      int c, int num_cus, const void* d_digits, void* ws, void* d_out, uint32_t* arrived, hipStream_t stream);
Status bases_generate_label(int curve, const uint8_t* label, size_t len, size_t start, size_t n, void* d_pts, hipStream_t stream);
Status point_sum(int curve, const void* d_jac, size_t n, void* d_out, hipStream_t stream);
Status bases_validate(int curve, const void* d_pts, size_t n, uint32_t* d_flags, hipStream_t stream);
Status bases_precompute(int curve, const void* d_pts, size_t n, int c, int sets, int tables, void* d_table,
                        hipStream_t stream);

Status vec_axpy(int field, const void* a, const void* r, const void* b, size_t n, void* out, hipStream_t s);
Status vec_cross_term(int field, const void* az1, const void* bz1, const void* cz1, const void* az2,
                      const void* bz2, const void* cz2, const void* u1, size_t n, void* T, hipStream_t s);
Status vec_minroot_witness(int field, const void* trace_xy, const void* i0, uint64_t t, void* W, hipStream_t s);
Status vec_spmv_long(int field, const uint32_t* const rowptr[3], const uint32_t* const col[3], const uint32_t* const coef[3],
                     const void* dict, const void* z, const uint32_t* long_rows, size_t n_long, void* const out[3], hipStream_t s);
Status vec_spmv(int field, const uint32_t* rowptr, const uint32_t* col, const uint32_t* coef, const void* dict,
                const void* z, size_t rows, void* out, hipStream_t s);
Status vec_step_segment(int field, const void* trace_xy, uint64_t t, const vdf_fe* i0, int per, void* out, void* packed,
                        const vdf_fe* i_in, hipStream_t s);
Status vec_step_z(int field, const void* trace_xy, uint64_t t, const vdf_fe z_in[3], const vdf_fe* i0, const vdf_fe* u,
                  const vdf_fe X[6], void* z, void* packed, hipStream_t s);
Status vec_nifs_cross(int field, const uint32_t* const rowptr[3], const uint32_t* const col[3],
                      const uint32_t* const coef[3], const void* dict, const void* z2, const void* az1, const void* bz1,
                      const void* cz1, const vdf_fe* u1, size_t rows, size_t skip_begin, size_t skip_len,
                      const uint32_t* long_rowlist, size_t n_long_rows, void* az2, void* bz2, void* cz2, void* T,
                      double alg_bytes, hipStream_t s);
int nifs_cross_lanes(size_t rows);
Status vec_nifs_cross_minroot(int field, int per, uint64_t t, size_t seg_begin, size_t one_col, size_t row0, const void* z2,
                              const void* az1, const void* bz1, const void* cz1, const vdf_fe* u1, void* az2, void* bz2, void* cz2,
                              void* T, hipStream_t s);
Status vec_nifs_cross_minroot_fold(int field, int per, uint64_t t, size_t seg_begin, size_t one_col, size_t row0, const void* z2,
                                   const vdf_fe* r, void* az1, void* bz1, void* cz1, void* e1, const void* tprev, const vdf_fe* u1,
                                   void* az2, void* bz2, void* cz2, void* T, hipStream_t s);
Status vec_fold_many(int field, const vdf_fe* r, int k, void* const acc[], const void* const add[], const size_t n[],
                     hipStream_t s);
constexpr int LINCOMB_MAX = 64;
constexpr int RESIDUAL_BATCH_MAX = 64;
Status vec_lincomb_u128(int field, int count, const void* const v[], const size_t n[], const vdf_fe w[], size_t n_out, void* out,
                        hipStream_t s);
size_t residual_item_bytes();
void residual_pack(int count, const void* const z[], const void* const E[], const vdf_fe u[], const vdf_fe rho[], void* block);
Status vec_relaxed_residual_batch(int field, const uint32_t* const rowptr[3], const uint32_t* const col[3], const uint32_t* const coef[3],
                                  const void* dict, const void* block, int count, size_t rows, const uint32_t* long_rowlist,
                                  size_t n_long_rows, void* out, double alg_bytes, hipStream_t s);
Status vec_mul(int field, const void* a, const void* b, size_t n, void* out, hipStream_t s);
Status vec_any_nonzero(const void* v, size_t n, uint32_t* d_flag, hipStream_t s);
Status vec_to_mont(int field, const void* a, size_t n, void* out, hipStream_t s);
Status vec_from_mont(int field, const void* a, size_t n, void* out, hipStream_t s);
Status vec_mul_chain(int field, const void* a, size_t n, int iters, void* out, hipStream_t s);
Status vec_clock_probe(int iters, int workgroups, unsigned long long* d_out3, hipStream_t s);

Status snark_pair_table(int field, const vdf_fe* lo, const vdf_fe* hi, int k, void* out, hipStream_t s);
size_t snark_ipa_block_bytes(int count);
void snark_ipa_pack(const vdf_ipa_opening* ops, int count, void* block);
Status snark_field_one(int field, vdf_fe* out);
Status snark_ipa_coefficients(int field, const void* block, int count, size_t n, void* out, hipStream_t s);
Status snark_fold_halves(int field, int k, void* const v[], const vdf_fe c_lo[], const vdf_fe c_hi[], size_t n, hipStream_t s);
size_t snark_reduce_scratch_bytes();
Status snark_reduce(int field, int kind, const void* const tables[], const vdf_fe* u, size_t n, void* scratch, void* out,
                    hipStream_t s);
Status snark_spmvt(int field, const uint32_t* colptr, const uint32_t* rows, const uint32_t* cm, const uint32_t* heavy,
                   size_t nheavy, size_t nbig, const void* dict, const void* eq, const vdf_fe* rho, size_t ncols, void* out, void* scratch,
                   hipStream_t s);
Status snark_ipa_scalars(int field, const void* a, const void* sv, size_t n, size_t nj, void* sL, void* sR, hipStream_t s);
Status snark_scale_pattern(int field, void* sv, size_t n, size_t nj, const vdf_fe* x_lo, const vdf_fe* x_hi, hipStream_t s);
constexpr int SNARK_FOLD_BATCH_MAX = 320;
constexpr int SNARK_REDUCE_BATCH_MAX = 512;
// ... 15 lines not shown
```

### vdf_amd/csrc/msm.hip

```cpp
#include <cstdlib>
#include <cstring>
#include "internal.h"
#include "ec.cuh"
#include "ecq.cuh"

namespace vdf {

static constexpr uint32_t SIGN_BIT = 0x80000000u;

__device__ __forceinline__ void raise_wave_priority(int wave_prio = 3) {
  if (wave_prio >= 3) __builtin_amdgcn_s_setprio(3);
  else if (wave_prio == 2) __builtin_amdgcn_s_setprio(2);
  else if (wave_prio == 1) __builtin_amdgcn_s_setprio(1);
}
static constexpr int ACC_WG_PER_CU = 3;
static constexpr int ACC_WG_FILL = 2;
static constexpr uint32_t HEAVY_MIN = 6;
static constexpr uint32_t GIANT_SPAN = 64;
static constexpr uint32_t GIANT_CHUNK = 32;
static constexpr uint32_t GIANT_PARTS = 256;
static constexpr uint32_t MAX_GIANTS = 192;
__device__ __forceinline__ uint32_t giant_parts(uint32_t span) {
  const uint32_t p = (span + GIANT_CHUNK - 1) / GIANT_CHUNK;
  return p > GIANT_PARTS ? GIANT_PARTS : p;
}

__device__ __forceinline__ uint32_t slice_len(uint32_t ne, uint32_t slots, uint32_t fixed) {
  if (fixed) return fixed;
  const uint32_t L = (ne + slots - 1) / slots;
  return L < 8u ? 8u : L;
}
static constexpr uint32_t RED_QUADS = 8192;

struct WsLayout {
  size_t countsA, pcount, pstart, recs, bcount, bstart, tstart, sorted, bucket_acc, heads, heavy, giant, partials, wsum, total;
  uint32_t red_seg, red_threads_per_set, red_block, red_blocks_per_set;
};

static size_t align_up(size_t x, size_t a) { return (x + a - 1) / a * a; }

struct RedGeom { uint32_t seg, threads_per_set, block, blocks_per_set; };
static RedGeom red_geom(size_t nkeys, uint32_t nbk) {
  RedGeom r;
  uint32_t seg = 2;
  const uint32_t quads = tuning().reduction_quads ? (uint32_t)tuning().reduction_quads : RED_QUADS;
  while (seg < 64 && nkeys / seg > quads) seg <<= 1;
  if (seg > nbk) seg = nbk;
  r.seg = seg;
  r.threads_per_set = nbk / seg;
  r.block = r.threads_per_set < 64 ? r.threads_per_set : 64;
  r.blocks_per_set = r.threads_per_set / r.block;
  return r;
}

struct MatGeom {
  uint32_t Lb, nrows, ncols, nsums;
  uint32_t Q, sums_per_wg, wgs_per_set;
  uint32_t bA, bB;
  size_t sums_bytes, scratch_bytes;
};
static MatGeom mat_geom(size_t gsets, uint32_t nbk) {
  MatGeom g;
  uint32_t m = 0;
  while ((1u << m) < nbk) ++m;
  g.Lb = (m + 1) / 2;
  g.ncols = 1u << g.Lb;
  g.nrows = nbk >> g.Lb;
  g.nsums = g.nrows + g.ncols;
  uint32_t q = g.nrows / 2;
  if (q < 1) q = 1;
  if (q > 64) q = 64;
  g.Q = q;
  g.sums_per_wg = 64 / g.Q;
  g.wgs_per_set = (g.nsums + g.sums_per_wg - 1) / g.sums_per_wg;
  g.bA = (g.ncols + 63) / 64;
  g.bB = (g.nrows + 63) / 64;
  g.sums_bytes = align_up(gsets * g.nsums * 128, 256);
  g.scratch_bytes = g.sums_bytes + align_up(gsets * (g.bA + g.bB) * 128, 256);
  return g;
}
static bool use_matrix_reduction(uint32_t nbk) {
  return tuning().reduction != 0 && nbk >= 16;
}

static WsLayout ws_layout(const MsmPlan& p) {
  WsLayout w{};
  size_t off = 0;
  const size_t nkeys = (size_t)p.gsets * p.nbk;
  auto take = [&](size_t bytes) { size_t o = off; off = align_up(off + bytes, 256); return o; };
  w.countsA = take((size_t)p.nblkA * p.bins * 4);
  w.pcount = take((size_t)p.bins * 4);
  w.pstart = take(((size_t)p.bins + 1) * 4);
  w.recs = take((size_t)p.windows * p.n * 8);
  w.bcount = take(nkeys * 4);
  w.bstart = take((nkeys + 1) * 4);
  w.tstart = take(((size_t)p.nthreads + 1) * 4);
  w.sorted = take(((size_t)p.windows * p.n + 64) * 4);
  w.bucket_acc = take(nkeys * 128);
  w.heads = take((size_t)p.nthreads * 128);
  w.heavy = take((nkeys + 4 + 2 * MAX_GIANTS) * 4);
  w.giant = take((size_t)MAX_GIANTS * GIANT_PARTS * 128);
  const RedGeom rg = red_geom(nkeys, p.nbk);
  w.red_seg = rg.seg; w.red_threads_per_set = rg.threads_per_set; w.red_block = rg.block;
  w.red_blocks_per_set = rg.blocks_per_set;
  {
    const size_t seg_bytes = (size_t)p.gsets * w.red_blocks_per_set * 128;
    const size_t mat_bytes = mat_geom(p.gsets, p.nbk).scratch_bytes;
    w.partials = take(seg_bytes > mat_bytes ? seg_bytes : mat_bytes);
  }
  w.wsum = take((size_t)p.gsets * 128);
  w.total = off;
  return w;
}

int msm_auto_window(size_t n) {
  int lg = 0;
  while (((size_t)1 << (lg + 1)) <= n) ++lg;
  int c = lg - 4;
  if (c < 4) c = 4;
  if (c > 16) c = 16;
  return c;
}

bool msm_plan_feasible(int groups, int c, int sets) {
  const int windows = (256 + c - 1) / c;
  if (sets <= 0) sets = windows;
  const int over = c - 1 - 10;
  return ((uint64_t)groups * sets << (over > 0 ? over : 0)) <= 8192u;
}

MsmPlan msm_make_plan(int groups, const size_t* gn, const size_t* goff, int c, int sets, int tables, int num_cus, int acc_fill, int scalar_bits) {
  MsmPlan p;
  p.groups = groups;
  size_t n = 0, nmax = 0;
  for (int g = 0; g < groups; ++g) {
    p.gn[g] = (uint32_t)gn[g];
    p.goff[g] = (uint32_t)goff[g];
    n += gn[g];
    if (gn[g] > nmax) nmax = gn[g];
  }
  p.n = (uint32_t)n;
  p.c = c;
  p.windows = (scalar_bits + c - 1) / c;
  p.signed_scalars = scalar_bits != 256;
  if (sets <= 0 || tables <= 0) { sets = p.windows; tables = 1; }
  p.sets = sets;
  p.gsets = groups * sets;
  p.tables = tables;
  p.nbk = 1u << (c - 1);
  p.pb = 0;
  while (p.pb < c - 1 && ((uint32_t)p.gsets << p.pb) < (uint32_t)num_cus) ++p.pb;
  if (tuning().part_bits >= 0 && tuning().part_bits <= c - 1) p.pb = tuning().part_bits;
  const int fine_max = c >= 18 && tuning().part_bits < 0 && !tuning().sort_staged ? 8 : 10;
  while (c - 1 - p.pb > fine_max) ++p.pb;
  while (p.pb > 0 && ((uint32_t)p.gsets << p.pb) > 8192u) --p.pb;
  p.fb = c - 1 - p.pb;
  p.bins = (uint32_t)p.gsets << p.pb;
  size_t chA = (n + 511) / 512;
  chA = (chA + 255) / 256 * 256;
  if (chA < 256) chA = 256;
  const size_t chA_max = p.bins > 512 ? 16384 : 4096;
  if (chA > chA_max) chA = chA_max;
  p.chA = (uint32_t)chA;
  uint32_t blk = 0;
  for (int g = 0; g < groups; ++g) {
    blk += (uint32_t)((gn[g] + chA - 1) / chA);
    p.gblk_end[g] = blk;
  }
  p.nblkA = blk ? blk : 1;
  size_t ne = (size_t)n * p.windows;
  int acc_wg = acc_fill ? acc_fill : tuning().accumulate_fill;
  if (acc_wg == 0) acc_wg = (groups == 1 && ne >= ((size_t)1 << 22)) ? ACC_WG_PER_CU : ACC_WG_FILL;
  if (acc_wg < 1 || acc_wg > ACC_WG_PER_CU) acc_wg = ACC_WG_FILL;
  const size_t slots = (size_t)num_cus * acc_wg * 256;
  size_t L = (ne + slots - 1) / slots;
  if (L < 8) L = 8;
  p.L = (uint32_t)L;
  p.Lfixed = 0;
  p.slots = (uint32_t)slots;
  p.nthreads = (uint32_t)slots;
  if (tuning().slice_len >= 1 && tuning().slice_len <= 65536) {
    const long v = tuning().slice_len;
    p.L = p.Lfixed = (uint32_t)v; p.nthreads = (uint32_t)((ne + v - 1) / v); if (p.nthreads < 1) p.nthreads = 1;
  }
  p.ws_bytes = ws_layout(p).total;
  return p;
}

struct DigitIter {
  const uint32_t* col;
  uint32_t carry;
  __device__ __forceinline__ uint32_t next(int w, int c) {
    const int bit = w * c;
    const int l = bit >> 5, sh = bit & 31;
    const uint32_t lo = (l < 8) ? col[l * 256] : 0u;
    const uint32_t hi = (l + 1 < 9) ? col[(l + 1) * 256] : 0u;
    const uint64_t two = ((uint64_t)hi << 32) | lo;
    const uint32_t raw = ((uint32_t)(two >> sh) & ((1u << c) - 1u)) + carry;
    if (raw > (1u << (c - 1))) { carry = 1; return ((1u << c) - raw) | SIGN_BIT; }
    carry = 0;
    return raw;
  }
};
template <class SP>
__device__ __forceinline__ void stage_scalar(uint32_t* limbs, Fe<SP> s, int is_mont) {
  if (is_mont) s = fe_from_mont(s);
#pragma unroll
  for (int l = 0; l < 8; ++l) limbs[l * 256 + threadIdx.x] = s.v[l];
  limbs[8 * 256 + threadIdx.x] = 0;
}

struct PartGroups {
  const uint32_t* scalars[MSM_MAX_GROUPS];
  uint32_t n[MSM_MAX_GROUPS], off[MSM_MAX_GROUPS], blk_end[MSM_MAX_GROUPS];
  int groups;
  int signed_scalars;
};

template <class SP, bool SCATTER>
__global__ __launch_bounds__(256) void k_part(PartGroups pg, int is_mont, int c, int windows, int sets, int pb, int fb,
                                              uint32_t bins, uint32_t chA, uint32_t tstride,
                                              uint32_t* __restrict__ countsA, const uint32_t* __restrict__ pstart,
                                              uint32_t* __restrict__ recsP, uint16_t* __restrict__ recsK, int wave_prio) {
  raise_wave_priority(wave_prio);
  __shared__ uint32_t limbs[9 * 256];
  extern __shared__ uint32_t cur[];
  uint32_t* mine = countsA + (size_t)blockIdx.x * bins;
  for (uint32_t b = threadIdx.x; b < bins; b += 256) cur[b] = SCATTER ? pstart[b] + mine[b] : 0u;
  __syncthreads();
  int g = 0;
  while (g < pg.groups - 1 && blockIdx.x >= pg.blk_end[g]) ++g;
  const uint32_t blk0 = g ? pg.blk_end[g - 1] : 0u;
  const uint32_t* __restrict__ scalars = pg.scalars[g];
  const uint32_t n = pg.n[g];
  const uint32_t lo = (blockIdx.x - blk0) * chA;
  const uint32_t hi = (lo + chA < n) ? lo + chA : n;
  const uint32_t fmask = (1u << fb) - 1u;
  const uint32_t set0 = (uint32_t)g * (uint32_t)sets;
  const uint32_t pbase = pg.off[g];
  uint32_t i = lo + threadIdx.x;
  Fe<SP> nxt = fe_zero<SP>();
  if (i < hi) nxt = fe_load<SP>(scalars + (size_t)i * 8);
  for (; i < hi; i += 256) {
    const Fe<SP> curs = nxt;
    if (i + 256 < hi) nxt = fe_load<SP>(scalars + (size_t)(i + 256) * 8);
    Fe<SP> mags = curs;
    uint32_t ssign = 0;
    if (pg.signed_scalars) { ssign = mags.v[7] & SIGN_BIT; mags.v[7] &= ~SIGN_BIT; }
    stage_scalar<SP>(limbs, mags, is_mont);
    DigitIter it{limbs + threadIdx.x, 0u};
    for (int w = 0; w < windows; ++w) {
      const uint32_t d = it.next(w, c) ^ ssign;
      const uint32_t mag = d & ~SIGN_BIT;
      if (!mag) continue;
      const uint32_t s = (uint32_t)w % (uint32_t)sets, j = (uint32_t)w / (uint32_t)sets;
      const uint32_t bin = ((set0 + s) << pb) | ((mag - 1) >> fb);
      const uint32_t pos = atomicAdd(&cur[bin], 1u);
      if (SCATTER) { recsP[pos] = (j * tstride + pbase + i) | (d & SIGN_BIT); recsK[pos] = (uint16_t)((mag - 1) & fmask); }
    }
  }
  if (!SCATTER) {
    __syncthreads();
    for (uint32_t b = threadIdx.x; b < bins; b += 256) mine[b] = cur[b];
  }
}

static constexpr uint32_t PART_STAGE_BINS = 512;
template <class SP>
__global__ __launch_bounds__(256) void k_part_staged(PartGroups pg, int is_mont, int c, int windows, int sets, int pb, int fb,
                                                     uint32_t bins, uint32_t chA, uint32_t tstride,
                                                     const uint32_t* __restrict__ countsA, const uint32_t* __restrict__ pstart,
                                                     uint32_t* __restrict__ recsP, uint16_t* __restrict__ recsK, int wave_prio) {
  raise_wave_priority(wave_prio);
  __shared__ uint32_t limbs[9 * 256];
  __shared__ uint32_t cur[PART_STAGE_BINS];
  __shared__ uint32_t tcnt[PART_STAGE_BINS];
  __shared__ uint32_t toff[PART_STAGE_BINS + 1];
  __shared__ uint32_t tpos[PART_STAGE_BINS];
  __shared__ uint32_t stage[256 * 16];
  __shared__ uint32_t skb[256 * 16];
  const uint32_t* mine = countsA + (size_t)blockIdx.x * bins;
  for (uint32_t b = threadIdx.x; b < bins; b += 256) { cur[b] = pstart[b] + mine[b]; tcnt[b] = 0; }
  int g = 0;
  while (g < pg.groups - 1 && blockIdx.x >= pg.blk_end[g]) ++g;
  const uint32_t blk0 = g ? pg.blk_end[g - 1] : 0u;
  const uint32_t* __restrict__ scalars = pg.scalars[g];
  const uint32_t n = pg.n[g];
  const uint32_t lo = (blockIdx.x - blk0) * chA;
  const uint32_t hi = (lo + chA < n) ? lo + chA : n;
  const uint32_t fmask = (1u << fb) - 1u;
  const uint32_t set0 = (uint32_t)g * (uint32_t)sets;
  const uint32_t pbase = pg.off[g];
  const uint32_t per_lane = (bins + 63) / 64;
  Fe<SP> nxt = fe_zero<SP>();
  if (lo + threadIdx.x < hi) nxt = fe_load<SP>(scalars + (size_t)(lo + threadIdx.x) * 8);
  __syncthreads();
  for (uint32_t base = lo; base < hi; base += 256) {
    const uint32_t i = base + threadIdx.x;
    Fe<SP> mags = nxt;
    if (i + 256 < hi) nxt = fe_load<SP>(scalars + (size_t)(i + 256) * 8);
    uint32_t ssign = 0;
    if (i < hi) {
      if (pg.signed_scalars) { ssign = mags.v[7] & SIGN_BIT; mags.v[7] &= ~SIGN_BIT; }
      stage_scalar<SP>(limbs, mags, is_mont);
      DigitIter it{limbs + threadIdx.x, 0u};
      for (int w = 0; w < windows; ++w) {
        const uint32_t mag = it.next(w, c) & ~SIGN_BIT;
        if (!mag) continue;
        atomicAdd(&tcnt[((set0 + (uint32_t)w % (uint32_t)sets) << pb) | ((mag - 1) >> fb)], 1u);
      }
    }
    __syncthreads();
    if (threadIdx.x < 64) {
      uint32_t run = 0;
      const uint32_t b0 = threadIdx.x * per_lane;
      for (uint32_t k = 0; k < per_lane; ++k) if (b0 + k < bins) run += tcnt[b0 + k];
      uint32_t incl = run;
#pragma unroll
      for (int d = 1; d < 64; d <<= 1) { const uint32_t o = __shfl_up(incl, d, 64); if ((int)threadIdx.x >= d) incl += o; }
      uint32_t off = incl - run;
      for (uint32_t k = 0; k < per_lane; ++k) if (b0 + k < bins) { toff[b0 + k] = off; tpos[b0 + k] = off; off += tcnt[b0 + k]; }
      if (threadIdx.x == 63) toff[bins] = incl;
    }
    __syncthreads();
    if (i < hi) {
      DigitIter it{limbs + threadIdx.x, 0u};
      for (int w = 0; w < windows; ++w) {
        const uint32_t d = it.next(w, c) ^ ssign;
        const uint32_t mag = d & ~SIGN_BIT;
        if (!mag) continue;
        const uint32_t s = (uint32_t)w % (uint32_t)sets, j = (uint32_t)w / (uint32_t)sets;
        const uint32_t bin = ((set0 + s) << pb) | ((mag - 1) >> fb);
        const uint32_t p = atomicAdd(&tpos[bin], 1u);
        stage[p] = (j * tstride + pbase + i) | (d & SIGN_BIT);
        skb[p] = ((mag - 1) & fmask) | (bin << 16);
      }
    }
    __syncthreads();
    const uint32_t tile_n = toff[bins];
    for (uint32_t q = threadIdx.x; q < tile_n; q += 256) {
      const uint32_t kb = skb[q], b = kb >> 16;
      const uint32_t pos = cur[b] + (q - toff[b]);
      recsP[pos] = stage[q];
      recsK[pos] = (uint16_t)kb;
    }
    __syncthreads();
    for (uint32_t b = threadIdx.x; b < bins; b += 256) { cur[b] += tcnt[b]; tcnt[b] = 0; }
    __syncthreads();
  }
}

__global__ __launch_bounds__(256) void k_part_scan(uint32_t* __restrict__ countsA, uint32_t bins, uint32_t nblk,
                                                   uint32_t* __restrict__ pcount, uint32_t* __restrict__ heavy,
                                                   uint32_t* __restrict__ giant_done, int wave_prio) {
  raise_wave_priority(wave_prio);
  __shared__ uint32_t sc[256];
  const uint32_t b = blockIdx.x;
  uint32_t carry = 0;
  for (uint32_t k0 = 0; k0 < nblk; k0 += 256) {
    const uint32_t k = k0 + threadIdx.x;
    const uint32_t v = (k < nblk) ? countsA[(size_t)k * bins + b] : 0u;
    sc[threadIdx.x] = v;
    __syncthreads();
    for (uint32_t d = 1; d < 256; d <<= 1) {
      const uint32_t t = (threadIdx.x >= d) ? sc[threadIdx.x - d] : 0u;
      __syncthreads();
      sc[threadIdx.x] += t;
      __syncthreads();
    }
    if (k < nblk) countsA[(size_t)k * bins + b] = carry + sc[threadIdx.x] - v;
    const uint32_t tot = sc[255];
    __syncthreads();
    carry += tot;
  }
  if (threadIdx.x == 0) pcount[b] = carry;
  if (b == 0 && threadIdx.x == 0) { heavy[0] = 0; giant_done[-1] = 0; }
  if (b == 0 && threadIdx.x < MAX_GIANTS) giant_done[threadIdx.x] = 0;
}

__global__ __launch_bounds__(1024) void k_scan_keys(const uint32_t* __restrict__ bcount, uint32_t nkeys,
                                                    uint32_t* __restrict__ bstart, int wave_prio) {
  raise_wave_priority(wave_prio);
  __shared__ uint32_t part[1024];
  const uint32_t per = (nkeys + 1023) / 1024;
  const uint32_t lo = threadIdx.x * per < nkeys ? threadIdx.x * per : nkeys;
  const uint32_t hi = (lo + per < nkeys) ? lo + per : nkeys;
  uint32_t sum = 0;
  uint32_t i = lo;
  for (; i + 8 <= hi; i += 8) {
    uint32_t v[8];
#pragma unroll
    for (int u = 0; u < 8; ++u) v[u] = bcount[i + u];
#pragma unroll
    for (int u = 0; u < 8; ++u) sum += v[u];
  }
  for (; i < hi; ++i) sum += bcount[i];
  part[threadIdx.x] = sum;
  __syncthreads();
  for (uint32_t d = 1; d < 1024; d <<= 1) {
    uint32_t v = (threadIdx.x >= d) ? part[threadIdx.x - d] : 0u;
    __syncthreads();
    part[threadIdx.x] += v;
    __syncthreads();
  }
  uint32_t run = part[threadIdx.x] - sum;
  i = lo;
  for (; i + 8 <= hi; i += 8) {
    uint32_t v[8];
#pragma unroll
    for (int u = 0; u < 8; ++u) v[u] = bcount[i + u];
#pragma unroll
    for (int u = 0; u < 8; ++u) { bstart[i + u] = run; run += v[u]; }
  }
  for (; i < hi; ++i) { bstart[i] = run; run += bcount[i]; }
  if (threadIdx.x == 1023) bstart[nkeys] = part[1023];
}

__device__ __forceinline__ uint32_t lds_take_slot(uint32_t* h, uint32_t key) {
  const uint32_t first = __builtin_amdgcn_readfirstlane(key);
// ... 317 lines not shown
    bool queued = false;
    if (tl - tf > giant_span) {
      const uint32_t idx = atomicAdd(q.giant_count, 1u);
      if (idx < MAX_GIANTS) { q.giants[idx] = g; queued = true; }
    }
    if (!queued) q.items[atomicAdd(q.count, 1u)] = g;
    return;
  }
  XYZZ<P> acc = xyzz_load<P>(bucket_acc + (size_t)g * 128);
  bool have = !fe_is_zero(acc.zz), flip = false;
  if (have) { acc.x = fe_canon(acc.x); acc.y = fe_canon(acc.y); acc.zz = fe_canon(acc.zz); acc.zzz = fe_canon(acc.zzz); }
  XYZZ<P> nxt = xyzz_load<P>(heads + (size_t)(tf + 1) * 128);
  for (uint32_t t = tf + 1; t <= tl; ++t) {
    XYZZ<P> cur = nxt;
    if (t < tl) nxt = xyzz_load<P>(heads + (size_t)(t + 1) * 128);
    if (fe_is_zero(cur.zz)) continue;
    cur.x = fe_canon(cur.x); cur.y = fe_canon(cur.y); cur.zz = fe_canon(cur.zz); cur.zzz = fe_canon(cur.zzz);
    if (have && flip) cur.y = fe_neg_nz(cur.y);
    xyzz_add_lazy<P>(acc, have, flip, cur);
  }
  xyzz_store<P>(bucket_acc + (size_t)g * 128, xyzz_lazy_resolve<P>(acc, have, flip));
}

template <class P>
__global__ __launch_bounds__(64) void k_fixup_heavy(const uint32_t* __restrict__ bstart, uint32_t nkeys, uint32_t slots,
                                                    uint32_t Lfixed, char* __restrict__ bucket_acc,
                                                    const char* __restrict__ heads, uint32_t* __restrict__ heavy,
                                                    char* __restrict__ giant, int wave_prio) {
  raise_wave_priority(wave_prio);
  const HeavyLayout q = heavy_layout(heavy, nkeys);
  const uint32_t count = *q.count;
  uint32_t ngiant = *q.giant_count;
  if (ngiant > MAX_GIANTS) ngiant = MAX_GIANTS;
  if (count == 0 && ngiant == 0) return;
  const uint32_t L = slice_len(bstart[nkeys], slots, Lfixed);
  const uint32_t quad = threadIdx.x >> 2;
  const uint32_t part = blockIdx.x % GIANT_PARTS, ngroups = gridDim.x / GIANT_PARTS;
  if (blockIdx.x < ngroups * GIANT_PARTS)
    for (uint32_t my = blockIdx.x / GIANT_PARTS; my < ngiant; my += ngroups) {
      const uint32_t g = q.giants[my];
      const uint32_t s = bstart[g], e = bstart[g + 1];
      const uint32_t tf = s / L, tl = (e - 1) / L, span = tl - tf;
      const uint32_t parts = giant_parts(span);
      if (part >= parts) continue;
      const uint32_t chunk = (span + parts - 1) / parts;
      const uint32_t t0 = tf + 1 + part * chunk;
      const uint32_t t1 = (t0 + chunk - 1 < tl) ? t0 + chunk - 1 : tl;
      QPoint<P> acc = qpoint_identity<P>();
      for (uint32_t t = t0 + quad; t <= t1; t += 16) acc = qpoint_add<P>(acc, qpoint_load_lazy<P>(heads + (size_t)t * 128));
      acc = qpoint_wave_sum(acc);
      char* slot = giant + ((size_t)my * GIANT_PARTS + part) * 128;
      if (quad == 0) qpoint_store<P>(slot, acc);
      __threadfence();
      uint32_t arrived = 0;
      if (threadIdx.x == 0) arrived = atomicAdd(&q.done[my], 1u);
      arrived = (uint32_t)__builtin_amdgcn_readfirstlane(arrived);
      if (arrived != parts - 1) continue;
      __threadfence();
      QPoint<P> tot = qpoint_identity<P>();
      for (uint32_t p = quad; p < parts; p += 16) tot = qpoint_add<P>(tot, qpoint_load<P>(giant + ((size_t)my * GIANT_PARTS + p) * 128));
      tot = qpoint_wave_sum(tot);
      if (quad == 0) {
        QPoint<P> base = qpoint_load_lazy<P>(bucket_acc + (size_t)g * 128);
        qpoint_store<P>(bucket_acc + (size_t)g * 128, qpoint_add<P>(base, tot));
      }
    }
  for (uint32_t item = blockIdx.x; item < count; item += gridDim.x) {
    const uint32_t g = q.items[item];
    const uint32_t s = bstart[g], e = bstart[g + 1];
    const uint32_t tf = s / L, tl = (e - 1) / L;
    QPoint<P> acc = qpoint_identity<P>();
    for (uint32_t t = tf + 1 + quad; t <= tl; t += 16) acc = qpoint_add<P>(acc, qpoint_load_lazy<P>(heads + (size_t)t * 128));
    acc = qpoint_wave_sum(acc);
    if (quad == 0) {
      QPoint<P> base = qpoint_load_lazy<P>(bucket_acc + (size_t)g * 128);
      qpoint_store<P>(bucket_acc + (size_t)g * 128, qpoint_add<P>(base, acc));
    }
  }
}

template <class P>
__global__ __launch_bounds__(256) void k_reduce1(const char* __restrict__ bucket_acc, uint32_t nbk, uint32_t nseg,
                                                 uint32_t threads_per_set, uint32_t blocks_per_set,
                                                 char* __restrict__ partials, int wave_prio) {
  raise_wave_priority(wave_prio);
  extern __shared__ __align__(16) char lds_raw[];
  const uint32_t nlog = blockDim.x >> 2;
  const uint32_t lt = threadIdx.x >> 2;
  const uint32_t set = blockIdx.x / blocks_per_set;
  const uint32_t blk = blockIdx.x % blocks_per_set;
  const uint32_t seg = blk * nlog + lt;
  const uint32_t base = seg * nseg;
  QPoint<P> run = qpoint_identity<P>(), tot = qpoint_identity<P>();
  if (seg < threads_per_set) {
    const char* bp = bucket_acc + ((size_t)set * nbk + base) * 128;
    for (int l = (int)nseg - 1; l >= 0; --l) {
      run = qpoint_add<P>(run, qpoint_load_lazy<P>(bp + (size_t)l * 128));
      tot = qpoint_add<P>(tot, run);
    }
    if (base) {
      QPoint<P> m = qpoint_identity<P>();
      for (int bit = 31 - __builtin_clz(base); bit >= 0; --bit) {
        m = qpoint_dbl<P>(m);
        if ((base >> bit) & 1u) m = qpoint_add<P>(m, run);
      }
      tot = qpoint_add<P>(tot, m);
    }
  }
  qpoint_store<P>(lds_raw + (size_t)lt * 128, tot);
  __syncthreads();
  for (uint32_t stride = nlog >> 1; stride >= 1; stride >>= 1) {
    if (lt < stride) {
      tot = qpoint_add<P>(tot, qpoint_load<P>(lds_raw + (size_t)(lt + stride) * 128));
      qpoint_store<P>(lds_raw + (size_t)lt * 128, tot);
    }
    __syncthreads();
  }
  if (lt == 0) qpoint_store<P>(partials + (size_t)blockIdx.x * 128, tot);
}

template <class P>
__global__ __launch_bounds__(256) void k_reduce2(const char* __restrict__ partials, uint32_t blocks_per_set,
                                                 char* __restrict__ wsum, int wave_prio) {
  raise_wave_priority(wave_prio);
  __shared__ __align__(16) char lds_raw[64 * 128];
  const uint32_t set = blockIdx.x;
  const uint32_t lt = threadIdx.x >> 2;
  QPoint<P> acc = qpoint_identity<P>();
  for (uint32_t i = lt; i < blocks_per_set; i += 64)
    acc = qpoint_add<P>(acc, qpoint_load<P>(partials + ((size_t)set * blocks_per_set + i) * 128));
  qpoint_store<P>(lds_raw + (size_t)lt * 128, acc);
  __syncthreads();
  for (uint32_t stride = 32; stride >= 1; stride >>= 1) {
    if (lt < stride) {
      acc = qpoint_add<P>(acc, qpoint_load<P>(lds_raw + (size_t)(lt + stride) * 128));
      qpoint_store<P>(lds_raw + (size_t)lt * 128, acc);
    }
    __syncthreads();
  }
  if (lt == 0) qpoint_store<P>(wsum + (size_t)set * 128, acc);
}

template <class P>
__global__ __launch_bounds__(256) void k_red_sums(const char* __restrict__ bucket_acc, uint32_t nbk, uint32_t Lb, uint32_t Q,
                                                  uint32_t wgs_per_set, char* __restrict__ sums, int wave_prio) {
  raise_wave_priority(wave_prio);
  __shared__ __align__(16) char lds_raw[64 * 128];
  const uint32_t ncols = 1u << Lb, nrows = nbk >> Lb, nsums = nrows + ncols;
  const uint32_t set = blockIdx.x / wgs_per_set, blk = blockIdx.x % wgs_per_set;
  const uint32_t lt = threadIdx.x >> 2, sub = lt / Q, qi = lt % Q;
  const uint32_t sidx = blk * (64 / Q) + sub;
  const char* bp = bucket_acc + (size_t)set * nbk * 128;
  QPoint<P> acc = qpoint_identity<P>();
  if (sidx < nrows) {
    for (uint32_t l = qi; l < ncols; l += Q) acc = qpoint_add<P>(acc, qpoint_load_lazy<P>(bp + ((size_t)sidx * ncols + l) * 128));
  } else if (sidx < nsums) {
    const uint32_t l = sidx - nrows;
    for (uint32_t h = qi; h < nrows; h += Q) acc = qpoint_add<P>(acc, qpoint_load_lazy<P>(bp + ((size_t)h * ncols + l) * 128));
  }
  qpoint_store<P>(lds_raw + (size_t)lt * 128, acc);
  __syncthreads();
  for (uint32_t stride = Q >> 1; stride >= 1; stride >>= 1) {
    if (qi < stride) {
      acc = qpoint_add<P>(acc, qpoint_load<P>(lds_raw + (size_t)(lt + stride) * 128));
      qpoint_store<P>(lds_raw + (size_t)lt * 128, acc);
    }
    __syncthreads();
  }
  if (qi == 0 && sidx < nsums) qpoint_store<P>(sums + ((size_t)set * nsums + sidx) * 128, acc);
}

template <class P>
__global__ __launch_bounds__(256) void k_red_weights(const char* __restrict__ sums, uint32_t nbk, uint32_t Lb, uint32_t bA,
                                                     uint32_t bB, char* __restrict__ partials, int wave_prio) {
  raise_wave_priority(wave_prio);
  __shared__ __align__(16) char lds_raw[64 * 128];
  const uint32_t ncols = 1u << Lb, nrows = nbk >> Lb, nsums = nrows + ncols;
  const uint32_t set = blockIdx.x / (bA + bB), blk = blockIdx.x % (bA + bB);
  const uint32_t lt = threadIdx.x >> 2;
  const bool col = blk < bA;
  const uint32_t idx = (col ? blk : blk - bA) * 64 + lt;
  const uint32_t weight = col ? idx + 1 : idx;
  QPoint<P> tot = qpoint_identity<P>();
  if (idx < (col ? ncols : nrows) && weight) {
    const QPoint<P> pt = qpoint_load<P>(sums + ((size_t)set * nsums + (col ? nrows + idx : idx)) * 128);
    const QPoint<P> mpt = qpoint_neg<P>(pt);
    const uint32_t h3 = 3u * weight;
    for (int bit = 31 - __builtin_clz(h3); bit >= 1; --bit) {
      tot = qpoint_dbl<P>(tot);
      const uint32_t hb = (h3 >> bit) & 1u, wb = (weight >> bit) & 1u;
      if (hb != wb) tot = qpoint_add<P>(tot, hb ? pt : mpt);
    }
  }
  qpoint_store<P>(lds_raw + (size_t)lt * 128, tot);
  __syncthreads();
  for (uint32_t stride = 32; stride >= 1; stride >>= 1) {
    if (lt < stride) {
      tot = qpoint_add<P>(tot, qpoint_load<P>(lds_raw + (size_t)(lt + stride) * 128));
      qpoint_store<P>(lds_raw + (size_t)lt * 128, tot);
    }
    __syncthreads();
  }
  if (lt == 0) qpoint_store<P>(partials + ((size_t)set * (bA + bB) + blk) * 128, tot);
}

template <class P>
__global__ __launch_bounds__(256) void k_red_combine(const char* __restrict__ partials, uint32_t Lb, uint32_t bA, uint32_t bB,
                                                     char* __restrict__ wsum, char* __restrict__ out_jac, int wave_prio) {
  raise_wave_priority(wave_prio);
  __shared__ __align__(16) char lds_raw[64 * 128];
  const uint32_t set = blockIdx.x;
  const uint32_t lt = threadIdx.x >> 2, half = lt >> 5, qi = lt & 31u;
  const char* base = partials + (size_t)set * (bA + bB) * 128 + (half ? (size_t)bA * 128 : 0);
  const uint32_t count = half ? bB : bA;
  QPoint<P> acc = qpoint_identity<P>();
  for (uint32_t i = qi; i < count; i += 32) acc = qpoint_add<P>(acc, qpoint_load<P>(base + (size_t)i * 128));
  qpoint_store<P>(lds_raw + (size_t)lt * 128, acc);
  __syncthreads();
  for (uint32_t stride = 16; stride >= 1; stride >>= 1) {
    if (qi < stride) {
      acc = qpoint_add<P>(acc, qpoint_load<P>(lds_raw + (size_t)(lt + stride) * 128));
      qpoint_store<P>(lds_raw + (size_t)lt * 128, acc);
    }
    __syncthreads();
  }
  if (lt == 32) {
    for (uint32_t k = 0; k < Lb; ++k) acc = qpoint_dbl<P>(acc);
    qpoint_store<P>(lds_raw + (size_t)32 * 128, acc);
  }
  __syncthreads();
  if (lt == 0) {
    const QPoint<P> res = qpoint_add<P>(acc, qpoint_load<P>(lds_raw + (size_t)32 * 128));
    if (!out_jac) {
      qpoint_store<P>(wsum + (size_t)set * 128, res);
    } else {
      const Jac<P> j = xyzz_to_jac(qpoint_gather(res));
      if (threadIdx.x == 0) {
        fe_store<P>(out_jac + (size_t)set * 96, j.x);
        fe_store<P>(out_jac + (size_t)set * 96 + 32, j.y);
        fe_store<P>(out_jac + (size_t)set * 96 + 64, j.z);
      }
    }
  }
}

template <class P>
__global__ __launch_bounds__(64) void k_final(const char* __restrict__ wsum_all, int sets, int c, char* __restrict__ out_all, int wave_prio) {
  raise_wave_priority(wave_prio);
  if (threadIdx.x >= 4) return;
  const char* wsum = wsum_all + (size_t)blockIdx.x * sets * 128;
  char* out_jac = out_all + (size_t)blockIdx.x * 96;
  QPoint<P> acc = qpoint_identity<P>();
  for (int s = sets - 1; s >= 0; --s) {
    if (s != sets - 1)
      for (int k = 0; k < c; ++k) acc = qpoint_dbl<P>(acc);
    acc = qpoint_add<P>(acc, qpoint_load<P>(wsum + (size_t)s * 128));
  }
  const Jac<P> j = xyzz_to_jac(qpoint_gather(acc));
  if (threadIdx.x == 0) {
    fe_store<P>(out_jac, j.x);
    fe_store<P>(out_jac + 32, j.y);
    fe_store<P>(out_jac + 64, j.z);
  }
}

__device__ __forceinline__ uint64_t splitmix64(uint64_t x) {
  uint64_t z = x + 0x9E3779B97F4A7C15ull;
  z = (z ^ (z >> 30)) * 0xBF58476D1CE4E5B9ull;
  z = (z ^ (z >> 27)) * 0x94D049BB133111EBull;
  return z ^ (z >> 31);
}

template <class P>
__global__ __launch_bounds__(256) void k_bases_generate(uint64_t seed, uint64_t start, uint32_t n, char* __restrict__ pts) {
  const uint32_t i = blockIdx.x * 256 + threadIdx.x;
  if (i >= n) return;
  const uint64_t k = splitmix64(seed * 0xD1342543DE82EF95ull + (start + i)) | 1ull;
  Affine<P> g;
#pragma unroll
  for (int l = 0; l < 8; ++l) { g.x.v[l] = P::GEN_X[l]; g.y.v[l] = P::GEN_Y[l]; }
  XYZZ<P> r = xyzz_mul_u64(g, k);
  affine_store<P>(pts + (size_t)i * 64, xyzz_to_affine(r));
}

template <class P>
__device__ bool fe_sqrt(const Fe<P>& a, Fe<P>& root) {
  if (fe_is_zero(a)) { root = a; return true; }
  uint32_t e[8];
  Fe<P> z;
#pragma unroll
  for (int i = 0; i < 8; ++i) { e[i] = P::TS_EXP[i]; z.v[i] = P::TS_Z[i]; }
  const Fe<P> w = fe_pow(a, e);
  Fe<P> x = fe_mul(a, w);
  Fe<P> b = fe_mul(x, w);
  const Fe<P> one = fe_one<P>();
  int v = 32;
  while (!fe_eq(b, one)) {
    int k = 0;
    Fe<P> t = b;
    while (!fe_eq(t, one)) { t = fe_sqr(t); ++k; if (k == v) return false; }
    Fe<P> zz = z;
    for (int i = 0; i < v - k - 1; ++i) zz = fe_sqr(zz);
    x = fe_mul(x, zz);
    z = fe_sqr(zz);
    b = fe_mul(b, z);
    v = k;
  }
  root = x;
  return true;
}

__device__ __forceinline__ uint64_t rotl64(uint64_t x, int k) { return (x << k) | (x >> (64 - k)); }
// ... 188 lines not shown
    uint32_t carry = 0;
#pragma unroll
    for (int j = 0; j < 5; ++j) {
      if (i + j < 8) {
        const uint64_t t = (uint64_t)c[i] * m[j] + p[i + j] + carry;
        p[i + j] = (uint32_t)t;
        carry = (uint32_t)(t >> 32);
      }
    }
    if (i + 5 < 8) p[i + 5] = carry;
  }
  uint64_t cy = 0;
#pragma unroll
  for (int i = 0; i < 8; ++i) {
    if (SUB) { const uint64_t d = (uint64_t)acc[i] - p[i] - cy; acc[i] = (uint32_t)d; cy = (d >> 63) & 1u; }
    else { const uint64_t d = (uint64_t)acc[i] + p[i] + cy; acc[i] = (uint32_t)d; cy = d >> 32; }
  }
}
__device__ __forceinline__ void to_sign_magnitude(uint32_t v[8]) {
  const uint32_t neg = v[7] >> 31;
  if (neg) {
    uint64_t cy = 1;
#pragma unroll
    for (int i = 0; i < 8; ++i) { const uint64_t d = (uint64_t)(~v[i]) + cy; v[i] = (uint32_t)d; cy = d >> 32; }
  }
  v[7] = (v[7] & 0x7FFFFFFFu) | (neg << 31);
}
template <class SP>
__global__ __launch_bounds__(256) void k_glv_split(const uint32_t* __restrict__ scalars, uint32_t n, int is_mont, uint32_t* __restrict__ out) {
  const uint32_t i = blockIdx.x * 256 + threadIdx.x;
  if (i >= n) return;
  Fe<SP> k = fe_load<SP>(scalars + (size_t)i * 8);
  if (is_mont) k = fe_from_mont(k);
  uint32_t g1[8], g2[8], a1[5], a2[5], nb1[5], b2[5], c1[5], c2[5];
#pragma unroll
  for (int l = 0; l < 8; ++l) { g1[l] = SP::GLV_G1[l]; g2[l] = SP::GLV_G2[l]; }
#pragma unroll
  for (int l = 0; l < 5; ++l) { a1[l] = SP::GLV_A1[l]; a2[l] = SP::GLV_A2[l]; nb1[l] = SP::GLV_NB1[l]; b2[l] = SP::GLV_B2[l]; }
  mul_shift_382(k.v, g1, c1);
  mul_shift_382(k.v, g2, c2);
  uint32_t k1[8], k2[8];
#pragma unroll
  for (int l = 0; l < 8; ++l) { k1[l] = k.v[l]; k2[l] = 0; }
  muladd_5x5<true>(k1, c1, a1);
  muladd_5x5<true>(k1, c2, a2);
  muladd_5x5<false>(k2, c1, nb1);
  muladd_5x5<true>(k2, c2, b2);
  to_sign_magnitude(k1);
  to_sign_magnitude(k2);
#pragma unroll
  for (int l = 0; l < 8; ++l) { out[(size_t)i * 8 + l] = k1[l]; out[((size_t)n + i) * 8 + l] = k2[l]; }
}
Status glv_points(int curve, const void* d_pts, size_t n, void* d_out, hipStream_t stream) {
  return with_curve(curve, [&](auto base, auto) {
    hipLaunchKernelGGL((k_glv_points<tag_t<decltype(base)>>), grid_for(n), dim3(256), 0, stream, cbytes_of(d_pts), (uint32_t)n, bytes_of(d_out));
  });
}
Status glv_split(int curve, const void* d_scalars, size_t n, bool is_mont, void* d_out, hipStream_t stream) {
  KTimer kt(stream, "k_glv_split", 96.0 * n);
  return with_curve(curve, [&](auto, auto scalar) {
    hipLaunchKernelGGL((k_glv_split<tag_t<decltype(scalar)>>), grid_for(n), dim3(256), 0, stream, reinterpret_cast<const uint32_t*>(d_scalars), (uint32_t)n,
                       is_mont ? 1 : 0, reinterpret_cast<uint32_t*>(d_out));
  });
}

template <class P>
__global__ __launch_bounds__(256) void k_precompute(const char* __restrict__ pts, uint32_t n, int shift, int tables,
                                                    char* __restrict__ table) {
  const uint32_t i = blockIdx.x * 256 + threadIdx.x;
  if (i >= n) return;
  Affine<P> a = affine_load<P>(pts + (size_t)i * 64);
  affine_store<P>(table + (size_t)i * 64, a);
  XYZZ<P> r = xyzz_from_affine(a);
  for (int j = 1; j < tables; ++j) {
    for (int k = 0; k < shift; ++k) r = xyzz_dbl(r);
    Affine<P> o = xyzz_to_affine(r);
    affine_store<P>(table + ((size_t)j * n + i) * 64, o);
    r = xyzz_from_affine(o);
  }
}

template <class P>
static Status msm_tail_t(int c, int sets, int groups, uint32_t nbk, const char* bucket_acc, char* partials, char* wsum,
                         void* d_out, hipStream_t st, int prio) {
  const uint32_t gsets = (uint32_t)(groups * sets);
  if (use_matrix_reduction(nbk)) {
    const MatGeom g = mat_geom(gsets, nbk);
    char* sums = partials;
    char* parts = partials + g.sums_bytes;
    hipLaunchKernelGGL((k_red_sums<P>), dim3(gsets * g.wgs_per_set), dim3(256), 0, st, bucket_acc, nbk, g.Lb, g.Q, g.wgs_per_set, sums, prio);
    hipLaunchKernelGGL((k_red_weights<P>), dim3(gsets * (g.bA + g.bB)), dim3(256), 0, st, sums, nbk, g.Lb, g.bA, g.bB, parts, prio);
    char* direct = sets == 1 ? bytes_of(d_out) : nullptr;
    hipLaunchKernelGGL((k_red_combine<P>), dim3(gsets), dim3(256), 0, st, parts, g.Lb, g.bA, g.bB, wsum, direct, prio);
    if (direct) {
      VDF_TRY_HIP(hipGetLastError());
      return Status{};
    }
  } else {
    const RedGeom rg = red_geom((size_t)gsets * nbk, nbk);
    hipLaunchKernelGGL((k_reduce1<P>), dim3(gsets * rg.blocks_per_set), dim3(rg.block * 4), (size_t)rg.block * 128, st,
                       bucket_acc, nbk, rg.seg, rg.threads_per_set, rg.blocks_per_set, partials, prio);
    hipLaunchKernelGGL((k_reduce2<P>), dim3(gsets), dim3(256), 0, st, partials, rg.blocks_per_set, wsum, prio);
  }
  hipLaunchKernelGGL((k_final<P>), dim3(groups), dim3(64), 0, st, wsum, sets, c, bytes_of(d_out), prio);
  VDF_TRY_HIP(hipGetLastError());
  return Status{};
}

template <class P, class SP>
static Status msm_run_t(const MsmPlan& p, const void* d_points, const void* const* d_scalars, bool is_mont, void* ws,
                        void* d_out, hipStream_t st, hipEvent_t* ev, char* ext_bucket_acc, hipEvent_t acc_gate, int prio) {
  const WsLayout w = ws_layout(p);
  char* base = bytes_of(ws);
  uint32_t* countsA = reinterpret_cast<uint32_t*>(base + w.countsA);
  uint32_t* pcount = reinterpret_cast<uint32_t*>(base + w.pcount);
  uint32_t* pstart = reinterpret_cast<uint32_t*>(base + w.pstart);
  uint32_t* recsP = reinterpret_cast<uint32_t*>(base + w.recs);
  uint16_t* recsK = reinterpret_cast<uint16_t*>(base + w.recs + (size_t)p.windows * p.n * 4);
  uint32_t* bstart = reinterpret_cast<uint32_t*>(base + w.bstart);
  uint32_t* sorted = reinterpret_cast<uint32_t*>(base + w.sorted);
  char* bucket_acc = ext_bucket_acc ? ext_bucket_acc : base + w.bucket_acc;
  char* heads = base + w.heads;
  uint32_t* heavy = reinterpret_cast<uint32_t*>(base + w.heavy);
  char* partials = base + w.partials;
  char* wsum = base + w.wsum;
  const uint32_t nkeys = (uint32_t)p.gsets * p.nbk;
  const uint32_t nf = 1u << p.fb;
  PartGroups pg{};
  pg.groups = p.groups;
  pg.signed_scalars = p.signed_scalars ? 1 : 0;
  for (int g = 0; g < p.groups; ++g) {
    pg.scalars[g] = reinterpret_cast<const uint32_t*>(d_scalars[g]);
    pg.n[g] = p.gn[g]; pg.off[g] = p.goff[g]; pg.blk_end[g] = p.gblk_end[g];
  }
  const size_t lds_bins = (size_t)p.bins * 4;

  if (ev) VDF_TRY_HIP(hipEventRecord(ev[0], st));
  {
  KTimer kt(st, "msm_sort(5 launches)", 0.0);
  hipLaunchKernelGGL((k_part<SP, false>), dim3(p.nblkA), dim3(256), lds_bins, st, pg, is_mont ? 1 : 0, p.c, p.windows,
                     p.sets, p.pb, p.fb, p.bins, p.chA, p.tstride, countsA, pstart, recsP, recsK, prio);
  hipLaunchKernelGGL(k_part_scan, dim3(p.bins), dim3(256), 0, st, countsA, p.bins, p.nblkA, pcount, heavy, heavy + 1 + nkeys + 2, prio);
  hipLaunchKernelGGL(k_scan_keys, dim3(1), dim3(1024), 0, st, pcount, p.bins, pstart, prio);
  if (tuning().sort_staged && p.bins <= PART_STAGE_BINS && p.windows <= 16)
    hipLaunchKernelGGL((k_part_staged<SP>), dim3(p.nblkA), dim3(256), 0, st, pg, is_mont ? 1 : 0, p.c, p.windows,
                       p.sets, p.pb, p.fb, p.bins, p.chA, p.tstride, countsA, pstart, recsP, recsK, prio);
  else
    hipLaunchKernelGGL((k_part<SP, true>), dim3(p.nblkA), dim3(256), lds_bins, st, pg, is_mont ? 1 : 0, p.c, p.windows,
                       p.sets, p.pb, p.fb, p.bins, p.chA, p.tstride, countsA, pstart, recsP, recsK, prio);
  if (tuning().sort_staged && nf <= 256)
    hipLaunchKernelGGL(k_fine_staged<4>, dim3(p.bins), dim3(1024), 0, st, recsP, recsK, pstart, p.bins, nf, bstart, sorted, bucket_acc, p.slots, p.Lfixed,
                       reinterpret_cast<uint32_t*>(base + w.tstart), prio);
  else if (tuning().sort_staged)
    hipLaunchKernelGGL(k_fine_staged<8>, dim3(p.bins), dim3(1024), 0, st, recsP, recsK, pstart, p.bins, nf, bstart, sorted, bucket_acc, p.slots, p.Lfixed,
                       reinterpret_cast<uint32_t*>(base + w.tstart), prio);
  else
    hipLaunchKernelGGL(k_fine, dim3(p.bins), dim3(1024), 0, st, recsP, recsK, pstart, p.bins, nf, bstart, sorted, bucket_acc, p.slots, p.Lfixed,
                       reinterpret_cast<uint32_t*>(base + w.tstart), prio);
  }
  if (ev) VDF_TRY_HIP(hipEventRecord(ev[1], st));
  if (acc_gate) VDF_TRY_HIP(hipStreamWaitEvent(st, acc_gate, 0));
  {
  KTimer kt(st, "k_accumulate", 96.0 * p.n);
  const unsigned acc_lds = (unsigned)(tuning().accumulate_lds >= 0 && tuning().accumulate_lds <= 65536 ? tuning().accumulate_lds : 0);
  hipLaunchKernelGGL((k_accumulate<P>), dim3((p.nthreads + 255) / 256), dim3(256), acc_lds, st, sorted, bstart, nkeys,
                     reinterpret_cast<const uint32_t*>(base + w.tstart), cbytes_of(d_points), bucket_acc, heads, p.slots, p.Lfixed, p.nthreads);
  }
  if (ev) VDF_TRY_HIP(hipEventRecord(ev[2], st));
  const FixupTune tune = fixup_tune();
  KTimer kt_tail(st, ext_bucket_acc ? "msm_fixup(2 launches)" : "msm_tail(fixup+reduce)", 0.0);
  if (tuning().fixup_serial)
    hipLaunchKernelGGL((k_fixup_serial<P>), dim3((nkeys + 255) / 256), dim3(256), 0, st, bstart, nkeys, p.slots, p.Lfixed, bucket_acc, heads,
                       heavy, tune.heavy_min, tune.giant_span, prio);
  else
    hipLaunchKernelGGL((k_fixup<P>), dim3((nkeys * 4 + 255) / 256), dim3(256), 0, st, bstart, nkeys, p.slots, p.Lfixed, bucket_acc, heads,
                       heavy, tune.heavy_min, tune.giant_span, prio);
  hipLaunchKernelGGL((k_fixup_heavy<P>), dim3(16 * GIANT_PARTS), dim3(64), 0, st, bstart, nkeys, p.slots, p.Lfixed, bucket_acc, heads, heavy,
                     base + w.giant, prio);
  if (!ext_bucket_acc) VDF_TRY(msm_tail_t<P>(p.c, p.sets, p.groups, p.nbk, bucket_acc, partials, wsum, d_out, st, prio));
  if (ev) VDF_TRY_HIP(hipEventRecord(ev[3], st));
  VDF_TRY_HIP(hipGetLastError());
  return Status{};
}

Status msm_run(int curve, const MsmPlan& plan, const void* d_points, const void* const* d_scalars, bool is_mont, void* ws,
               void* d_out, hipStream_t stream, hipEvent_t* ev, void* ext_bucket_acc, hipEvent_t acc_gate, int prio) {
  char* ext = bytes_of(ext_bucket_acc);
  prio = std::min(prio, (int)tuning().light_priority);
  return with_curve(curve, [&](auto base, auto scalar) {
    return msm_run_t<tag_t<decltype(base)>, tag_t<decltype(scalar)>>(plan, d_points, d_scalars, is_mont, ws, d_out, stream, ev, ext, acc_gate, prio);
  });
}

static size_t tail_scratch_bytes(size_t gsets, uint32_t nbk) {
  const RedGeom rg = red_geom(gsets * nbk, nbk);
  const size_t seg = align_up(gsets * rg.blocks_per_set * 128, 256), mat = mat_geom(gsets, nbk).scratch_bytes;
  return seg > mat ? seg : mat;
}
size_t msm_tail_ws_bytes(int groups, int sets, uint32_t nbk) {
  const size_t gsets = (size_t)groups * sets;
  return align_up(gsets * nbk * 128, 256) + tail_scratch_bytes(gsets, nbk) + align_up(gsets * 128, 256);
}
Status msm_tail(int curve, int c, int sets, int groups, uint32_t nbk, void* tail_ws, void* d_out, hipStream_t stream, int prio) {
  const size_t gsets = (size_t)groups * sets;
  prio = std::min(prio, (int)tuning().light_priority);
  char* bucket_acc = bytes_of(tail_ws);
  char* partials = bucket_acc + align_up(gsets * nbk * 128, 256);
  char* wsum = partials + tail_scratch_bytes(gsets, nbk);
  return with_curve(curve, [&](auto base, auto) {
    return msm_tail_t<tag_t<decltype(base)>>(c, sets, groups, nbk, bucket_acc, partials, wsum, d_out, stream, prio);
  });
}

template <class P>
__global__ __launch_bounds__(64) void k_point_sum(const char* __restrict__ pts, uint32_t n, char* __restrict__ out, int wave_prio) {
  raise_wave_priority(wave_prio);
  const uint32_t quad = threadIdx.x >> 2;
  QPoint<P> acc = qpoint_identity<P>();
  for (uint32_t i = quad; i < n; i += 16) {
    Jac<P> j;
    j.x = fe_load<P>(pts + (size_t)i * 96);
    j.y = fe_load<P>(pts + (size_t)i * 96 + 32);
    j.z = fe_load<P>(pts + (size_t)i * 96 + 64);
    acc = qpoint_add<P>(acc, qpoint_scatter(jac_to_xyzz(j)));
  }
  acc = qpoint_wave_sum(acc);
  const Jac<P> j = xyzz_to_jac(qpoint_gather(acc));
  if (threadIdx.x == 0) {
    fe_store<P>(out, j.x);
    fe_store<P>(out + 32, j.y);
    fe_store<P>(out + 64, j.z);
  }
}

Status point_sum(int curve, const void* d_jac, size_t n, void* d_out, hipStream_t stream) {
  const int prio = std::min(3, (int)tuning().light_priority);
  return with_curve(curve, [&](auto base, auto) {
    hipLaunchKernelGGL((k_point_sum<tag_t<decltype(base)>>), dim3(1), dim3(64), 0, stream, cbytes_of(d_jac), (uint32_t)n, bytes_of(d_out), prio);
  });
}

Status bases_generate(int curve, int family, uint64_t seed, size_t start, size_t n, void* d_pts, hipStream_t stream) {
  if (n == 0) return Status{};
  if (family == VDF_GENS_TRY_AND_INCREMENT)
    return with_curve(curve, [&](auto base, auto) {
      hipLaunchKernelGGL((k_bases_generate_tai<tag_t<decltype(base)>>), grid_for(n), dim3(256), 0, stream, seed, (uint64_t)start, (uint32_t)n,
                         bytes_of(d_pts));
    });
  if (family != VDF_GENS_KNOWN_DLOG) return Status{VDF_ERR_BAD_ARG, "unknown generator family"};
  return with_curve(curve, [&](auto base, auto) {
    hipLaunchKernelGGL((k_bases_generate<tag_t<decltype(base)>>), grid_for(n), dim3(256), 0, stream, seed, (uint64_t)start, (uint32_t)n, bytes_of(d_pts));
  });
}

Status bases_generate_label(int curve, const uint8_t* label, size_t len, size_t start, size_t n, void* d_pts, hipStream_t stream) {
  if (n == 0) return Status{};
  if (len > 64 || (len && !label)) return Status{VDF_ERR_BAD_LENGTH, "label of at most 64 bytes"};
  GenLabel gl;
  std::memset(&gl, 0, sizeof(gl));
  if (len) std::memcpy(gl.bytes, label, len);
  gl.len = (uint32_t)len;
  return with_curve(curve, [&](auto base, auto) {
// ... 24 lines not shown
```

### vdf_amd/hip.py

```python
from __future__ import annotations

import ctypes as C
import weakref
from typing import Optional, Sequence

import numpy as np

from . import _lib
from ._lib import lib, CURVE_PALLAS, CURVE_VESTA, FIELD_FP, FIELD_FQ


class HipTuning(C.Structure):
    _fields_ = [("struct_size", C.c_uint32)] + [(k, C.c_int32) for k in (
        "msm_direct", "direct_priority", "direct_fused", "light_priority", "accumulate_fill", "accumulate_lds", "slice_len", "part_bits",
        "reduction", "reduction_quads", "heavy_min", "giant_span", "nifs_lanes", "shim_cache", "nifs_fused", "fold_u128", "fixup_serial", "sort_staged", "glv")]


def tuning_get() -> HipTuning:
    t = HipTuning()
    rc = lib.vdf_hip_tuning_get(C.byref(t))
    if rc != 0:
        raise VdfError(rc, "vdf_hip_tuning_get")
    return t


def tuning_set(**fields) -> HipTuning:
    t = tuning_get()
    for k, v in fields.items():
        if k not in dict(HipTuning._fields_):
            raise KeyError(k)
        setattr(t, k, int(v))
    rc = lib.vdf_hip_tuning_set(C.byref(t))
    if rc != 0:
        raise VdfError(rc, "vdf_hip_tuning_set: a field is out of range")
    return t


class IpaOpening(C.Structure):
    _fields_ = [("weight", C.c_uint64 * 4), ("k", C.c_int), ("log_m", C.c_int), ("lo", C.c_void_p), ("hi", C.c_void_p),
                ("pattern", C.c_void_p)]


class VdfError(RuntimeError):
    def __init__(self, code: int, msg: str):
        super().__init__(f"vdf_hip error {code}: {msg}")
        self.code = code


def ints_to_limbs(vals: Sequence[int]) -> np.ndarray:
    buf = b"".join(int(v).to_bytes(32, "little") for v in vals)
    return np.frombuffer(buf, dtype="<u8").reshape(-1, 4).copy()


def limbs_to_ints(arr: np.ndarray) -> list:
    a = np.ascontiguousarray(arr, dtype="<u8").reshape(-1, 4)
    raw = a.tobytes()
    return [int.from_bytes(raw[32 * i:32 * i + 32], "little") for i in range(a.shape[0])]


def _ptr(x) -> Optional[int]:
    if x is None:
        return None
    if isinstance(x, np.ndarray):
        if not x.flags["C_CONTIGUOUS"]:
            raise ValueError("numpy buffers must be C-contiguous")
        return x.ctypes.data
    if hasattr(x, "data_ptr"):
        if not x.is_contiguous():
            raise ValueError("tensors must be contiguous")
        return x.data_ptr()
    if isinstance(x, int):
        return x
    raise TypeError(type(x))


class Bases:
    def __init__(self, ctx: "Context", handle: int, curve: int):
        self.ctx, self.handle, self.curve = ctx, handle, curve
        ctx._children.add(self)

    def __len__(self) -> int:
        return lib.vdf_bases_len(self.handle)

    def validate(self) -> None:
        bad = C.c_size_t()
        rc = lib.vdf_bases_validate(self.ctx.handle, self.handle, C.byref(bad))
        if rc != 0:
            raise VdfError(rc, (lib.vdf_last_error(self.ctx.handle) or b"").decode() + f" (index {bad.value})")

    @property
    def device_ptr(self) -> int:
        return lib.vdf_bases_device_ptr(self.handle)

    def precompute(self, window_bits: int = 16, sets: int = 1) -> None:
        self.ctx._check(lib.vdf_bases_precompute(self.ctx.handle, self.handle, window_bits, sets))

    @property
    def window(self) -> int:
        return lib.vdf_bases_window(self.handle)

    def precompute_digits(self, ranges, window_bits: int = 0) -> None:
        k = len(ranges)
        b = (C.c_size_t * max(k, 1))(*[int(r[0]) for r in ranges])
        n = (C.c_size_t * max(k, 1))(*[int(r[1]) for r in ranges])
        self.ctx._check(lib.vdf_bases_precompute_digits(self.ctx.handle, self.handle, window_bits, k, b, n))

    @property
    def digit_window(self) -> int:
        return lib.vdf_bases_digit_window(self.handle)

    def download(self, offset: int = 0, n: Optional[int] = None) -> np.ndarray:
        n = len(self) - offset if n is None else n
        out = np.zeros((n, 8), dtype="<u8")
        self.ctx._check(lib.vdf_bases_download(self.ctx.handle, self.handle, offset, n, _ptr(out)))
        return out

    def free(self) -> None:
        if self.handle and self.ctx.handle:
            lib.vdf_bases_free(self.handle)
        self.handle = None

    def __del__(self):
        try:
            self.free()
        except Exception:
            pass


_ALLGATHER = C.CFUNCTYPE(C.c_int, C.c_void_p, C.c_void_p, C.c_void_p, C.c_size_t, C.c_void_p)


def msm_multi(ctxs, bases, scalars, n, offsets=None, is_mont: bool = False):
    k = len(ctxs)
    out = np.zeros(12, dtype="<u8")
    offs = (C.c_size_t * k)(*(offsets or [0] * k))
    rc = lib.vdf_msm_multi((C.c_void_p * k)(*[c.handle for c in ctxs]), (C.c_void_p * k)(*[b.handle for b in bases]), offs,
                           (C.c_void_p * k)(*[_ptr(x) for x in scalars]), (C.c_size_t * k)(*[int(x) for x in n]), k,
                           int(is_mont), out.ctypes.data)
    ctxs[0]._check(rc)
    return out


class Shape:
    def __init__(self, ctx: "Context", handle: int, field: int, num_cons: int, num_cols: int):
        self.ctx, self.handle, self.field, self.num_cons, self.num_cols = ctx, handle, field, num_cons, num_cols
        ctx._children.add(self)

    def free(self) -> None:
        if self.handle and self.ctx.handle:
            lib.vdf_shape_free(self.handle)
        self.handle = None

    def __del__(self):
        try:
            self.free()
        except Exception:
            pass


class MsmJob:

    def __init__(self, ctx: "Context", handle: int, k: int):
        self.ctx, self.handle, self.k = ctx, handle, k

    def push(self, g: int, scalars) -> None:
        self.ctx._check(lib.vdf_msm_job_push(self.handle, g, _ptr(scalars)))

    def finish(self, out=None):
        if out is None:
            out = np.zeros((self.k, 12), dtype="<u8")
        h, self.handle = self.handle, None
        self.ctx._check(lib.vdf_msm_job_finish(h, _ptr(out)))
        return out


QUEUE_CRITICAL, QUEUE_SIDE = 1, 2


class Context:

    def __init__(self, device: int = 0, pooled_role: int = 0):
        h = C.c_void_p()
# ... 331 lines not shown
```

Measured before the change: 0.9387.

## Add per-bit power table for fixed-base MSM with sparse signed-digit recoding

Precomputes a 257-row table of 2^i multiples of each generator and, for single-group MSMs, recodes each scalar into sparse odd signed digits at arbitrary bit positions, so each digit maps to a table row. This removes per-window doubling and the cross-window combine, leaving a single reduction over the bucket range with an odd-bucket weighting. The cost is a very large device table (257×n affine points, gated by a memory budget and free-memory check) and more complex partitioning and reduction paths.

```diff
diff --git a/bindings/rust/vdf-hip-sys/src/lib.rs b/bindings/rust/vdf-hip-sys/src/lib.rs
--- a/bindings/rust/vdf-hip-sys/src/lib.rs
+++ b/bindings/rust/vdf-hip-sys/src/lib.rs
@@ -20,7 +20,7 @@
 #[repr(C)] #[derive(Clone, Copy, Debug)] pub struct VdfNovaStepInfo { pub comm_W1: VdfAffine, pub X1: [VdfFe; 2], pub comm_T1: VdfAffine, pub comm_T2: VdfAffine, pub r1: [u64; 4], pub r2: [u64; 4] }
 #[repr(C)] #[derive(Clone, Copy, Debug)] pub struct VdfNovaAugInputs { pub params: VdfFe, pub i: VdfFe, pub z0: [VdfFe; 3], pub zi: [VdfFe; 3], pub U_comm_W: VdfAffine, pub U_comm_E: VdfAffine, pub U_u: VdfFe, pub U_X: [VdfFe; 2], pub u_comm_W: VdfAffine, pub u_X: [VdfFe; 2], pub T: VdfAffine }
 #[repr(C)] #[derive(Clone, Copy, Debug)] pub struct VdfKernelEvent { pub name: [c_char; 24], pub bytes: f64, pub start_ms: f64, pub end_ms: f64 }
-#[repr(C)] #[derive(Clone, Copy, Debug)] pub struct VdfHipTuning { pub struct_size: u32, pub msm_direct: i32, pub direct_priority: i32, pub direct_fused: i32, pub light_priority: i32, pub accumulate_fill: i32, pub accumulate_lds: i32, pub slice_len: i32, pub part_bits: i32, pub reduction: i32, pub reduction_quads: i32, pub heavy_min: i32, pub giant_span: i32, pub nifs_lanes: i32, pub shim_cache: i32, pub nifs_fused: i32, pub fold_u128: i32, pub fixup_serial: i32, pub sort_staged: i32, pub glv: i32 }
+#[repr(C)] #[derive(Clone, Copy, Debug)] pub struct VdfHipTuning { pub struct_size: u32, pub msm_direct: i32, pub direct_priority: i32, pub direct_fused: i32, pub light_priority: i32, pub accumulate_fill: i32, pub accumulate_lds: i32, pub slice_len: i32, pub part_bits: i32, pub reduction: i32, pub reduction_quads: i32, pub heavy_min: i32, pub giant_span: i32, pub nifs_lanes: i32, pub shim_cache: i32, pub nifs_fused: i32, pub fold_u128: i32, pub fixup_serial: i32, pub sort_staged: i32, pub glv: i32, pub power_table: i32, pub power_width: i32, pub power_table_budget_gib: i32 }
 #[repr(C)] #[derive(Clone, Copy, Debug)] pub struct VdfNovaTuning { pub struct_size: u32, pub flags: u32, pub digit_budget_bytes: u64, pub digit_window: i32, pub early_rows: i32, pub stencil: i32, pub small_window: i32, pub big_window: i32, pub packed_commit: i32, pub lookahead_early: i32, pub gate_accumulate: i32, pub fold_on_rows: i32, pub nifs_ahead: i32, pub early_row_parts: i32, pub lookahead_priority: i32, pub side_accumulate_fill: i32, pub verbose: i32, pub compress_queues: i32, pub rows_at_challenge: i32, pub fold_fused: i32 }
 #[repr(C)] #[derive(Clone, Copy, Debug, PartialEq, Eq)] pub struct VdfNovaRoParams { pub struct_size: u32, pub family: i32, pub width: i32, pub full_rounds: i32, pub partial_rounds: i32, pub alpha: i32, pub challenge_bits: i32, pub hash_bits: i32 }
 #[repr(C)] #[derive(Clone, Copy, Debug)] pub struct VdfIpaOpening { pub weight: VdfFe, pub k: c_int, pub log_m: c_int, pub lo: *const VdfFe, pub hi: *const VdfFe, pub pattern: *const VdfFe }
@@ -47,6 +47,11 @@
     pub fn vdf_bases_generate_label(ctx: *mut VdfCtx, curve: c_int, label: *const u8, label_len: usize, start: usize, n: usize, out: *mut *mut VdfBases) -> c_int;
     pub fn vdf_bases_precompute(ctx: *mut VdfCtx, bases: *mut VdfBases, window_bits: c_int, sets: c_int) -> c_int;
     pub fn vdf_bases_window(bases: *const VdfBases) -> c_int;
+    pub fn vdf_bases_precompute_powers(ctx: *mut VdfCtx, bases: *mut VdfBases, width: c_int) -> c_int;
+    pub fn vdf_bases_power_width(bases: *const VdfBases) -> c_int;
+    pub fn vdf_bases_power_table_bytes(bases: *const VdfBases) -> usize;
+    pub fn vdf_bases_power_row_download(ctx: *mut VdfCtx, bases: *const VdfBases, row: c_int, offset: usize, n: usize, out: *mut VdfAffine) -> c_int;
+    pub fn vdf_power_recode(scalar: *const u32, width: c_int, capacity: c_int, positions: *mut u32, digits: *mut c_int) -> c_int;
     pub fn vdf_bases_precompute_digits(ctx: *mut VdfCtx, bases: *mut VdfBases, window_bits: c_int, ranges: c_int, begin: *const usize, count: *const usize) -> c_int;
     pub fn vdf_digit_table_bytes(window_bits: c_int, generators: usize) -> usize;
     pub fn vdf_bases_table_bytes(bases: *const VdfBases) -> usize;
diff --git a/include/vdf_hip.h b/include/vdf_hip.h
--- a/include/vdf_hip.h
+++ b/include/vdf_hip.h
@@ -54,6 +54,11 @@
 int  vdf_bases_generate_label(vdf_ctx* ctx, int curve, const uint8_t* label, size_t label_len, size_t start, size_t n, vdf_bases** out);
 int  vdf_bases_precompute(vdf_ctx* ctx, vdf_bases* bases, int window_bits, int sets);
 int  vdf_bases_window(const vdf_bases* bases);
+int  vdf_bases_precompute_powers(vdf_ctx* ctx, vdf_bases* bases, int width);
+int  vdf_bases_power_width(const vdf_bases* bases);
+size_t vdf_bases_power_table_bytes(const vdf_bases* bases);
+int  vdf_bases_power_row_download(vdf_ctx* ctx, const vdf_bases* bases, int row, size_t offset, size_t n, vdf_affine* out);
+int  vdf_power_recode(const uint32_t scalar[8], int width, int capacity, uint32_t* positions, int* digits);
 int  vdf_bases_precompute_digits(vdf_ctx* ctx, vdf_bases* bases, int window_bits, int ranges, const size_t begin[], const size_t count[]);
 size_t vdf_digit_table_bytes(int window_bits, size_t generators);
 size_t vdf_bases_table_bytes(const vdf_bases* bases);
@@ -193,6 +198,9 @@
   int32_t fixup_serial;
   int32_t sort_staged;
   int32_t glv;
+  int32_t power_table;
+  int32_t power_width;
+  int32_t power_table_budget_gib;
 } vdf_hip_tuning;
 int  vdf_hip_tuning_get(vdf_hip_tuning* out);
 int  vdf_hip_tuning_set(const vdf_hip_tuning* in);
diff --git a/vdf_amd/_lib.py b/vdf_amd/_lib.py
--- a/vdf_amd/_lib.py
+++ b/vdf_amd/_lib.py
@@ -42,6 +42,11 @@
     "vdf_bases_precompute": (_i, [_vp, _vp, _i, _i]),
     "vdf_bases_download": (_i, [_vp, _vp, _sz, _sz, _vp]),
     "vdf_bases_window": (_i, [_vp]),
+    "vdf_bases_precompute_powers": (_i, [_vp, _vp, _i]),
+    "vdf_bases_power_width": (_i, [_vp]),
+    "vdf_bases_power_table_bytes": (C.c_size_t, [_vp]),
+    "vdf_bases_power_row_download": (_i, [_vp, _vp, _i, _sz, _sz, _vp]),
+    "vdf_power_recode": (_i, [_vp, _i, _i, _vp, _vp]),
     "vdf_bases_precompute_digits": (_i, [_vp, _vp, _i, _i, _vp, _vp]),
     "vdf_bases_digit_window": (_i, [_vp]),
     "vdf_bases_digit_table_bytes": (C.c_size_t, [_vp]),
diff --git a/vdf_amd/csrc/abi.hip b/vdf_amd/csrc/abi.hip
--- a/vdf_amd/csrc/abi.hip
+++ b/vdf_amd/csrc/abi.hip
@@ -115,6 +115,7 @@
   t.accumulate_lds = 0; t.slice_len = 0; t.part_bits = -1; t.reduction = 1; t.reduction_quads = 0; t.heavy_min = 0;
   t.giant_span = 0; t.nifs_lanes = 0; t.shim_cache = 0; t.nifs_fused = 1; t.fold_u128 = 1;
   t.fixup_serial = 1; t.sort_staged = 1; t.glv = 1;
+  t.power_table = 1; t.power_width = 19; t.power_table_budget_gib = 20;
   return t;
 }
 bool tuning_valid(const vdf_hip_tuning& t) {
@@ -124,7 +125,8 @@
          in(t.reduction, 0, 1) && (t.reduction_quads == 0 || in(t.reduction_quads, 64, 65536)) &&
          (t.heavy_min == 0 || in(t.heavy_min, 1, 4096)) && (t.giant_span == 0 || in(t.giant_span, 16, 1 << 20)) &&
          (t.nifs_lanes == 0 || t.nifs_lanes == 1 || t.nifs_lanes == 4 || t.nifs_lanes == 8) && in(t.shim_cache, 0, 64) &&
-         in(t.nifs_fused, 0, 1) && in(t.fold_u128, 0, 1) && in(t.fixup_serial, 0, 1) && in(t.sort_staged, 0, 1) && in(t.glv, 0, 1);
+         in(t.nifs_fused, 0, 1) && in(t.fold_u128, 0, 1) && in(t.fixup_serial, 0, 1) && in(t.sort_staged, 0, 1) && in(t.glv, 0, 1) &&
+         in(t.power_table, 0, 1) && in(t.power_width, vdf::POWER_MIN_WIDTH, vdf::POWER_MAX_WIDTH) && in(t.power_table_budget_gib, 0, 1024);
 }
 void tuning_publish(const vdf_hip_tuning& t) {
   g_tune_snapshots.push_back(t);
@@ -139,7 +141,8 @@
       {"VDF_MSM_L", &t.slice_len}, {"VDF_MSM_PB", &t.part_bits}, {"VDF_MSM_RED", &t.reduction},
       {"VDF_MSM_RED_QUADS", &t.reduction_quads}, {"VDF_MSM_HEAVY_MIN", &t.heavy_min}, {"VDF_MSM_GIANT_SPAN", &t.giant_span},
       {"VDF_NIFS_LANES", &t.nifs_lanes}, {"VDF_SHIM_CACHE", &t.shim_cache}, {"VDF_NIFS_FUSED", &t.nifs_fused}, {"VDF_FOLD_U128", &t.fold_u128},
-      {"VDF_MSM_FIXUP_SERIAL", &t.fixup_serial}, {"VDF_MSM_SORT_STAGED", &t.sort_staged}, {"VDF_MSM_GLV", &t.glv}};
+      {"VDF_MSM_FIXUP_SERIAL", &t.fixup_serial}, {"VDF_MSM_SORT_STAGED", &t.sort_staged}, {"VDF_MSM_GLV", &t.glv},
+      {"VDF_MSM_POWER_TABLE", &t.power_table}, {"VDF_MSM_POWER_WIDTH", &t.power_width}, {"VDF_MSM_POWER_BUDGET_GIB", &t.power_table_budget_gib}};
   for (const auto& v : vars) {
     const char* e = std::getenv(v.name);
     if (!e || !*e) continue;
@@ -282,7 +285,11 @@
   }
   vdf::MsmPlan plan;
   const char* pts;
-  if (bases->d_table && (ctx->msm_window == 0 || ctx->msm_window == bases->tbl_c)) {
+  if (groups == 1 && bases->d_powers && ctx->msm_window == 0 && vdf::tuning().power_table) {
+    plan = vdf::msm_make_plan(1, n, offset, 0, 1, 0, ctx->num_cus, ctx->acc_fill, 256, bases->pw_width);
+    plan.tstride = (uint32_t)bases->n;
+    pts = vdf::cbytes_of(bases->d_powers);
+  } else if (bases->d_table && (ctx->msm_window == 0 || ctx->msm_window == bases->tbl_c)) {
     if (!vdf::msm_plan_feasible(groups, bases->tbl_c, bases->tbl_sets))
       return Status{VDF_ERR_BAD_ARG, "a batch this wide does not fit the sort under this table's window and bucket sets: fewer MSMs per call"};
     plan = vdf::msm_make_plan(groups, n, offset, bases->tbl_c, bases->tbl_sets, bases->tbl_tables, ctx->num_cus, ctx->acc_fill);
@@ -774,9 +781,75 @@
   });
 }
 
+extern "C++" {
+namespace {
+void power_table_drop(vdf_bases* bases) {
+  if (bases->d_powers) (void)hipFree(bases->d_powers);
+  bases->d_powers = nullptr; bases->pw_width = 0; bases->pw_bytes = 0;
+}
+Status power_table_build(vdf_ctx* ctx, vdf_bases* bases, int width) {
+  power_table_drop(bases);
+  if (bases->n == 0) return Status{};
+  if ((uint64_t)bases->n * (vdf::POWER_ROWS + 1) >= (1ull << 31)) return Status{VDF_ERR_BAD_LENGTH, "table index exceeds 31 bits"};
+  const size_t bytes = (size_t)vdf::POWER_ROWS * bases->n * sizeof(vdf_affine);
+  if (hipMalloc(&bases->d_powers, bytes) != hipSuccess) {
+    (void)hipGetLastError();
+    bases->d_powers = nullptr;
+    return Status{VDF_ERR_OOM, "the power table could not be allocated"};
+  }
+  Status s = vdf::bases_precompute(bases->curve, bases->d_pts, bases->n, 1, 1, vdf::POWER_ROWS, bases->d_powers, ctx->stream);
+  if (s.ok()) s = vdf::hip_status(hipStreamSynchronize(ctx->stream), "power table");
+  if (!s.ok()) { power_table_drop(bases); return s; }
+  bases->pw_width = width; bases->pw_bytes = bytes;
+  return Status{};
+}
+}
+}
+
+int vdf_bases_precompute_powers(vdf_ctx* ctx, vdf_bases* bases, int width) {
+  return guarded(ctx, [&]() -> Status {
+    if (!bases || bases->ctx != ctx) return Status{VDF_ERR_BAD_ARG, "bad bases handle"};
+    if (width < 0) { power_table_drop(bases); return Status{}; }
+    if (width == 0) width = vdf::tuning().power_width;
+    if (width < vdf::POWER_MIN_WIDTH || width > vdf::POWER_MAX_WIDTH) return Status{VDF_ERR_BAD_ARG, "digit width must be 0 (default), 5..20, or negative to drop the table"};
+    return power_table_build(ctx, bases, width);
+  });
+}
+int vdf_bases_power_width(const vdf_bases* bases) { return bases && bases->d_powers ? bases->pw_width : 0; }
+size_t vdf_bases_power_table_bytes(const vdf_bases* bases) { return bases && bases->d_powers ? bases->pw_bytes : 0; }
+int vdf_bases_power_row_download(vdf_ctx* ctx, const vdf_bases* bases, int row, size_t offset, size_t n, vdf_affine* out) {
+  return guarded(ctx, [&]() -> Status {
+    if (!bases || bases->ctx != ctx || (n && !out)) return Status{VDF_ERR_BAD_ARG, "bad arguments"};
+    if (!bases->d_powers || row < 0 || row >= vdf::POWER_ROWS) return Status{VDF_ERR_BAD_ARG, "no such row of a power table"};
+    if (offset > bases->n || n > bases->n - offset) return Status{VDF_ERR_BAD_LENGTH, "range exceeds the generator table"};
+    if (n == 0) return Status{};
+    VDF_TRY_HIP(hipMemcpyAsync(out, vdf::cbytes_of(bases->d_powers) + ((size_t)row * bases->n + offset) * 64, n * 64, hipMemcpyDefault, ctx->stream));
+    VDF_TRY_HIP(hipStreamSynchronize(ctx->stream));
+    return Status{};
+  });
+}
+int vdf_power_recode(const uint32_t scalar[8], int width, int capacity, uint32_t* positions, int* digits) {
+  if (!scalar || width < 2 || width > 24 || capacity < 0 || (capacity && (!positions || !digits))) return -1;
+  struct HostLimbs { const uint32_t* v; uint32_t operator()(int l) const { return v[l]; } };
+  vdf::PowerDigitIter<HostLimbs> it(HostLimbs{scalar}, width);
+  int count = 0;
+  uint32_t pos, d;
+  while (it.next(pos, d)) {
+    if (count < capacity) {
+      positions[count] = pos;
+      const int mag = (int)(d & 0x7FFFFFFFu);
+      digits[count] = (d >> 31) ? -mag : mag;
+    }
+    ++count;
+  }
+  return count;
+}
+
 int vdf_bases_precompute(vdf_ctx* ctx, vdf_bases* bases, int window_bits, int sets) {
   return guarded(ctx, [&]() -> Status {
     if (!bases || bases->ctx != ctx) return Status{VDF_ERR_BAD_ARG, "bad bases handle"};
+    const bool recommended = window_bits == 0;
+    power_table_drop(bases);
     if (window_bits == 0) window_bits = bases->n >= ((size_t)1 << 22) ? 20 : (bases->n >= ((size_t)1 << 19) ? 17 : 16);
     if (window_bits < 4 || window_bits > 20) return Status{VDF_ERR_BAD_ARG, "window_bits must be 0 (recommended) or 4..20"};
     const int windows = (256 + window_bits - 1) / window_bits;
@@ -792,6 +865,13 @@
     if (s.ok()) s = vdf::hip_status(hipStreamSynchronize(ctx->stream), "bases_precompute");
     if (!s.ok()) { (void)hipFree(bases->d_table); bases->d_table = nullptr; return s; }
     bases->tbl_c = window_bits; bases->tbl_sets = sets; bases->tbl_tables = tables;
+    const vdf_hip_tuning& tune = vdf::tuning();
+    const size_t pbytes = (size_t)vdf::POWER_ROWS * bases->n * sizeof(vdf_affine);
+    if (recommended && tune.power_table && bases->n >= ((size_t)1 << 19) && pbytes <= ((size_t)tune.power_table_budget_gib << 30)) {
+      size_t free_b = 0, total_b = 0;
+      if (hipMemGetInfo(&free_b, &total_b) == hipSuccess && pbytes + ((size_t)4 << 30) <= free_b) (void)power_table_build(ctx, bases, tune.power_width);
+      else (void)hipGetLastError();
+    }
     return Status{};
   });
 }
@@ -870,6 +950,7 @@
     if (bases->d_pts) (void)hipFree(bases->d_pts);
     if (bases->d_table) (void)hipFree(bases->d_table);
     if (bases->d_digits) (void)hipFree(bases->d_digits);
+    if (bases->d_powers) (void)hipFree(bases->d_powers);
     if (bases->d_pts2) (void)hipFree(bases->d_pts2);
   }
   delete bases;
diff --git a/vdf_amd/csrc/internal.h b/vdf_amd/csrc/internal.h
--- a/vdf_amd/csrc/internal.h
+++ b/vdf_amd/csrc/internal.h
@@ -8,6 +8,7 @@
 #include <vector>
 #include "../../include/vdf_hip.h"
 #include "pasta_constants.h"
+#include "power_digits.h"
 
 namespace vdf {
 struct KRecord { const char* name; double bytes; hipEvent_t e0, e1; };
@@ -103,6 +104,9 @@
   bool ephemeral = false;
   int tbl_c = 0, tbl_sets = 0, tbl_tables = 0;
   void* d_table = nullptr;
+  int pw_width = 0;
+  void* d_powers = nullptr;
+  size_t pw_bytes = 0;
   int dg_c = 0, dg_ranges = 0;
   size_t dg_begin[4] = {0, 0, 0, 0}, dg_count[4] = {0, 0, 0, 0}, dg_slot0[4] = {0, 0, 0, 0};
   void* d_digits = nullptr;
@@ -229,10 +233,13 @@
   uint32_t slots = 0;
   uint32_t nthreads = 0;
   uint32_t tstride = 0;
+  int power_w = 0;
+  bool low_part = false;
+  uint32_t red_lb = 0;
   size_t ws_bytes = 0;
 };
 MsmPlan msm_make_plan(int groups, const size_t* n, const size_t* offsets, int c, int sets, int tables, int num_cus, int acc_fill = 0,
-                      int scalar_bits = 256);
+                      int scalar_bits = 256, int power_w = 0);
 Status glv_points(int curve, const void* d_pts, size_t n, void* d_out, hipStream_t stream);
 Status glv_split(int curve, const void* d_scalars, size_t n, bool is_mont, void* d_out, hipStream_t stream);
 inline MsmPlan msm_make_plan(size_t n, int c, int sets, int tables, int num_cus) {
diff --git a/vdf_amd/csrc/msm.hip b/vdf_amd/csrc/msm.hip
--- a/vdf_amd/csrc/msm.hip
+++ b/vdf_amd/csrc/msm.hip
@@ -3,6 +3,7 @@
 #include "internal.h"
 #include "ec.cuh"
 #include "ecq.cuh"
+#include "power_digits.h"
 
 namespace vdf {
 
@@ -59,11 +60,11 @@
   uint32_t bA, bB;
   size_t sums_bytes, scratch_bytes;
 };
-static MatGeom mat_geom(size_t gsets, uint32_t nbk) {
+static MatGeom mat_geom(size_t gsets, uint32_t nbk, uint32_t lb = 0) {
   MatGeom g;
   uint32_t m = 0;
   while ((1u << m) < nbk) ++m;
-  g.Lb = (m + 1) / 2;
+  g.Lb = lb ? lb : (m + 1) / 2;
   g.ncols = 1u << g.Lb;
   g.nrows = nbk >> g.Lb;
   g.nsums = g.nrows + g.ncols;
@@ -105,7 +106,7 @@
   w.red_blocks_per_set = rg.blocks_per_set;
   {
     const size_t seg_bytes = (size_t)p.gsets * w.red_blocks_per_set * 128;
-    const size_t mat_bytes = mat_geom(p.gsets, p.nbk).scratch_bytes;
+    const size_t mat_bytes = mat_geom(p.gsets, p.nbk, p.red_lb).scratch_bytes;
     w.partials = take(seg_bytes > mat_bytes ? seg_bytes : mat_bytes);
   }
   w.wsum = take((size_t)p.gsets * 128);
@@ -129,8 +130,11 @@
   return ((uint64_t)groups * sets << (over > 0 ? over : 0)) <= 8192u;
 }
 
-MsmPlan msm_make_plan(int groups, const size_t* gn, const size_t* goff, int c, int sets, int tables, int num_cus, int acc_fill, int scalar_bits) {
+MsmPlan msm_make_plan(int groups, const size_t* gn, const size_t* goff, int c, int sets, int tables, int num_cus, int acc_fill, int scalar_bits,
+                      int power_w) {
   MsmPlan p;
+  p.power_w = power_w;
+  if (power_w) { c = power_w - 1; sets = 1; tables = POWER_ROWS; }
   p.groups = groups;
   size_t n = 0, nmax = 0;
   for (int g = 0; g < groups; ++g) {
@@ -141,7 +145,7 @@
   }
   p.n = (uint32_t)n;
   p.c = c;
-  p.windows = (scalar_bits + c - 1) / c;
+  p.windows = power_w ? power_max_digits(power_w) : (scalar_bits + c - 1) / c;
   p.signed_scalars = scalar_bits != 256;
   if (sets <= 0 || tables <= 0) { sets = p.windows; tables = 1; }
   p.sets = sets;
@@ -155,6 +159,8 @@
   while (c - 1 - p.pb > fine_max) ++p.pb;
   while (p.pb > 0 && ((uint32_t)p.gsets << p.pb) > 8192u) --p.pb;
   p.fb = c - 1 - p.pb;
+  p.low_part = power_w && use_matrix_reduction(p.nbk) && p.pb > 0 && p.fb > 0;
+  p.red_lb = p.low_part ? (uint32_t)p.fb : 0u;
   p.bins = (uint32_t)p.gsets << p.pb;
   size_t chA = (n + 511) / 512;
   chA = (chA + 255) / 256 * 256;
@@ -210,6 +216,31 @@
   limbs[8 * 256 + threadIdx.x] = 0;
 }
 
+struct LdsLimbs {
+  const uint32_t* col;
+  __device__ __forceinline__ uint32_t operator()(int l) const { return col[l * 256]; }
+};
+__device__ __forceinline__ void split_bucket(uint32_t bk, int pb, int fb, int low_part, uint32_t& part, uint32_t& fine) {
+  if (low_part) { part = bk & ((1u << pb) - 1u); fine = bk >> pb; }
+  else { part = bk >> fb; fine = bk & ((1u << fb) - 1u); }
+}
+template <class F>
+__device__ __forceinline__ void for_each_digit(const uint32_t* col, int c, int windows, int sets, int power_w, uint32_t ssign, F&& f) {
+  if (power_w) {
+    PowerDigitIter<LdsLimbs> it(LdsLimbs{col}, power_w);
+    uint32_t pos, d;
+    while (it.next(pos, d)) f(((d & ~SIGN_BIT) - 1u) >> 1, 0u, pos, d & SIGN_BIT);
+    return;
+  }
+  DigitIter it{col, 0u};
+  for (int w = 0; w < windows; ++w) {
+    const uint32_t d = it.next(w, c) ^ ssign;
+    const uint32_t mag = d & ~SIGN_BIT;
+    if (!mag) continue;
+    f(mag - 1u, (uint32_t)w % (uint32_t)sets, (uint32_t)w / (uint32_t)sets, d & SIGN_BIT);
+  }
+}
+
 struct PartGroups {
   const uint32_t* scalars[MSM_MAX_GROUPS];
   uint32_t n[MSM_MAX_GROUPS], off[MSM_MAX_GROUPS], blk_end[MSM_MAX_GROUPS];
@@ -218,7 +249,7 @@
 };
 
 template <class SP, bool SCATTER>
-__global__ __launch_bounds__(256) void k_part(PartGroups pg, int is_mont, int c, int windows, int sets, int pb, int fb,
+__global__ __launch_bounds__(256) void k_part(PartGroups pg, int is_mont, int c, int windows, int sets, int power_w, int low_part, int pb, int fb,
                                               uint32_t bins, uint32_t chA, uint32_t tstride,
                                               uint32_t* __restrict__ countsA, const uint32_t* __restrict__ pstart,
                                               uint32_t* __restrict__ recsP, uint16_t* __restrict__ recsK, int wave_prio) {
@@ -235,7 +266,6 @@
   const uint32_t n = pg.n[g];
   const uint32_t lo = (blockIdx.x - blk0) * chA;
   const uint32_t hi = (lo + chA < n) ? lo + chA : n;
-  const uint32_t fmask = (1u << fb) - 1u;
   const uint32_t set0 = (uint32_t)g * (uint32_t)sets;
   const uint32_t pbase = pg.off[g];
   uint32_t i = lo + threadIdx.x;
@@ -248,16 +278,12 @@
     uint32_t ssign = 0;
     if (pg.signed_scalars) { ssign = mags.v[7] & SIGN_BIT; mags.v[7] &= ~SIGN_BIT; }
     stage_scalar<SP>(limbs, mags, is_mont);
-    DigitIter it{limbs + threadIdx.x, 0u};
-    for (int w = 0; w < windows; ++w) {
-      const uint32_t d = it.next(w, c) ^ ssign;
-      const uint32_t mag = d & ~SIGN_BIT;
-      if (!mag) continue;
-      const uint32_t s = (uint32_t)w % (uint32_t)sets, j = (uint32_t)w / (uint32_t)sets;
-      const uint32_t bin = ((set0 + s) << pb) | ((mag - 1) >> fb);
-      const uint32_t pos = atomicAdd(&cur[bin], 1u);
-      if (SCATTER) { recsP[pos] = (j * tstride + pbase + i) | (d & SIGN_BIT); recsK[pos] = (uint16_t)((mag - 1) & fmask); }
-    }
+    for_each_digit(limbs + threadIdx.x, c, windows, sets, power_w, ssign, [&](uint32_t bk, uint32_t s, uint32_t j, uint32_t sign) {
+      uint32_t part, fine;
+      split_bucket(bk, pb, fb, low_part, part, fine);
+      const uint32_t pos = atomicAdd(&cur[((set0 + s) << pb) | part], 1u);
+      if (SCATTER) { recsP[pos] = (j * tstride + pbase + i) | sign; recsK[pos] = (uint16_t)fine; }
+    });
   }
   if (!SCATTER) {
     __syncthreads();
@@ -267,7 +293,7 @@
 
 static constexpr uint32_t PART_STAGE_BINS = 512;
 template <class SP>
-__global__ __launch_bounds__(256) void k_part_staged(PartGroups pg, int is_mont, int c, int windows, int sets, int pb, int fb,
+__global__ __launch_bounds__(256) void k_part_staged(PartGroups pg, int is_mont, int c, int windows, int sets, int power_w, int low_part, int pb, int fb,
                                                      uint32_t bins, uint32_t chA, uint32_t tstride,
                                                      const uint32_t* __restrict__ countsA, const uint32_t* __restrict__ pstart,
                                                      uint32_t* __restrict__ recsP, uint16_t* __restrict__ recsK, int wave_prio) {
@@ -288,7 +314,6 @@
   const uint32_t n = pg.n[g];
   const uint32_t lo = (blockIdx.x - blk0) * chA;
   const uint32_t hi = (lo + chA < n) ? lo + chA : n;
-  const uint32_t fmask = (1u << fb) - 1u;
   const uint32_t set0 = (uint32_t)g * (uint32_t)sets;
   const uint32_t pbase = pg.off[g];
   const uint32_t per_lane = (bins + 63) / 64;
@@ -303,12 +328,11 @@
     if (i < hi) {
       if (pg.signed_scalars) { ssign = mags.v[7] & SIGN_BIT; mags.v[7] &= ~SIGN_BIT; }
       stage_scalar<SP>(limbs, mags, is_mont);
-      DigitIter it{limbs + threadIdx.x, 0u};
-      for (int w = 0; w < windows; ++w) {
-        const uint32_t mag = it.next(w, c) & ~SIGN_BIT;
-        if (!mag) continue;
-        atomicAdd(&tcnt[((set0 + (uint32_t)w % (uint32_t)sets) << pb) | ((mag - 1) >> fb)], 1u);
-      }
+      for_each_digit(limbs + threadIdx.x, c, windows, sets, power_w, ssign, [&](uint32_t bk, uint32_t s, uint32_t, uint32_t) {
+        uint32_t part, fine;
+        split_bucket(bk, pb, fb, low_part, part, fine);
+        atomicAdd(&tcnt[((set0 + s) << pb) | part], 1u);
+      });
     }
     __syncthreads();
     if (threadIdx.x < 64) {
@@ -324,17 +348,14 @@
     }
     __syncthreads();
     if (i < hi) {
-      DigitIter it{limbs + threadIdx.x, 0u};
-      for (int w = 0; w < windows; ++w) {
-        const uint32_t d = it.next(w, c) ^ ssign;
-        const uint32_t mag = d & ~SIGN_BIT;
-        if (!mag) continue;
-        const uint32_t s = (uint32_t)w % (uint32_t)sets, j = (uint32_t)w / (uint32_t)sets;
-        const uint32_t bin = ((set0 + s) << pb) | ((mag - 1) >> fb);
+      for_each_digit(limbs + threadIdx.x, c, windows, sets, power_w, ssign, [&](uint32_t bk, uint32_t s, uint32_t j, uint32_t sign) {
+        uint32_t part, fine;
+        split_bucket(bk, pb, fb, low_part, part, fine);
+        const uint32_t bin = ((set0 + s) << pb) | part;
         const uint32_t p = atomicAdd(&tpos[bin], 1u);
-        stage[p] = (j * tstride + pbase + i) | (d & SIGN_BIT);
-        skb[p] = ((mag - 1) & fmask) | (bin << 16);
-      }
+        stage[p] = (j * tstride + pbase + i) | sign;
+        skb[p] = fine | (bin << 16);
+      });
     }
     __syncthreads();
     const uint32_t tile_n = toff[bins];
@@ -818,7 +839,7 @@
 template <class P>
 __global__ __launch_bounds__(256) void k_reduce1(const char* __restrict__ bucket_acc, uint32_t nbk, uint32_t nseg,
                                                  uint32_t threads_per_set, uint32_t blocks_per_set,
-                                                 char* __restrict__ partials, int wave_prio) {
+                                                 char* __restrict__ partials, int odd, int wave_prio) {
   raise_wave_priority(wave_prio);
   extern __shared__ __align__(16) char lds_raw[];
   const uint32_t nlog = blockDim.x >> 2;
@@ -842,6 +863,7 @@
       }
       tot = qpoint_add<P>(tot, m);
     }
+    if (odd) tot = qpoint_add<P>(qpoint_dbl<P>(tot), qpoint_neg<P>(run));
   }
   qpoint_store<P>(lds_raw + (size_t)lt * 128, tot);
   __syncthreads();
@@ -908,7 +930,7 @@
 
 template <class P>
 __global__ __launch_bounds__(256) void k_red_weights(const char* __restrict__ sums, uint32_t nbk, uint32_t Lb, uint32_t bA,
-                                                     uint32_t bB, char* __restrict__ partials, int wave_prio) {
+                                                     uint32_t bB, char* __restrict__ partials, int odd, int wave_prio) {
   raise_wave_priority(wave_prio);
   __shared__ __align__(16) char lds_raw[64 * 128];
   const uint32_t ncols = 1u << Lb, nrows = nbk >> Lb, nsums = nrows + ncols;
@@ -916,7 +938,7 @@
   const uint32_t lt = threadIdx.x >> 2;
   const bool col = blk < bA;
   const uint32_t idx = (col ? blk : blk - bA) * 64 + lt;
-  const uint32_t weight = col ? idx + 1 : idx;
+  const uint32_t weight = odd == 2 ? (col ? idx : 2u * idx + 1u) : col ? (odd ? 2u * idx + 1u : idx + 1u) : idx;
   QPoint<P> tot = qpoint_identity<P>();
   if (idx < (col ? ncols : nrows) && weight) {
     const QPoint<P> pt = qpoint_load<P>(sums + ((size_t)set * nsums + (col ? nrows + idx : idx)) * 128);
@@ -941,8 +963,8 @@
 }
 
 template <class P>
-__global__ __launch_bounds__(256) void k_red_combine(const char* __restrict__ partials, uint32_t Lb, uint32_t bA, uint32_t bB,
-                                                     char* __restrict__ wsum, char* __restrict__ out_jac, int wave_prio) {
+__global__ __launch_bounds__(256) void k_red_combine(const char* __restrict__ partials, uint32_t Lb , uint32_t bA, uint32_t bB,
+                                                     char* __restrict__ wsum, char* __restrict__ out_jac, int dbl_cols, int wave_prio) {
   raise_wave_priority(wave_prio);
   __shared__ __align__(16) char lds_raw[64 * 128];
   const uint32_t set = blockIdx.x;
@@ -960,10 +982,12 @@
     }
     __syncthreads();
   }
-  if (lt == 32) {
+  if (lt == 32 && !dbl_cols) {
     for (uint32_t k = 0; k < Lb; ++k) acc = qpoint_dbl<P>(acc);
     qpoint_store<P>(lds_raw + (size_t)32 * 128, acc);
   }
+  if (lt == 0 && dbl_cols)
+    for (uint32_t k = 0; k < Lb; ++k) acc = qpoint_dbl<P>(acc);
   __syncthreads();
   if (lt == 0) {
     const QPoint<P> res = qpoint_add<P>(acc, qpoint_load<P>(lds_raw + (size_t)32 * 128));
@@ -1318,16 +1342,18 @@
 
 template <class P>
 static Status msm_tail_t(int c, int sets, int groups, uint32_t nbk, const char* bucket_acc, char* partials, char* wsum,
-                         void* d_out, hipStream_t st, int prio) {
+                         void* d_out, hipStream_t st, int prio, int odd = 0, uint32_t red_lb = 0, uint32_t low_pb = 0) {
   const uint32_t gsets = (uint32_t)(groups * sets);
   if (use_matrix_reduction(nbk)) {
-    const MatGeom g = mat_geom(gsets, nbk);
+    const MatGeom g = mat_geom(gsets, nbk, red_lb);
     char* sums = partials;
+    if (low_pb) odd = 2;
     char* parts = partials + g.sums_bytes;
     hipLaunchKernelGGL((k_red_sums<P>), dim3(gsets * g.wgs_per_set), dim3(256), 0, st, bucket_acc, nbk, g.Lb, g.Q, g.wgs_per_set, sums, prio);
-    hipLaunchKernelGGL((k_red_weights<P>), dim3(gsets * (g.bA + g.bB)), dim3(256), 0, st, sums, nbk, g.Lb, g.bA, g.bB, parts, prio);
+    hipLaunchKernelGGL((k_red_weights<P>), dim3(gsets * (g.bA + g.bB)), dim3(256), 0, st, sums, nbk, g.Lb, g.bA, g.bB, parts, odd, prio);
     char* direct = sets == 1 ? bytes_of(d_out) : nullptr;
-    hipLaunchKernelGGL((k_red_combine<P>), dim3(gsets), dim3(256), 0, st, parts, g.Lb, g.bA, g.bB, wsum, direct, prio);
+    hipLaunchKernelGGL((k_red_combine<P>), dim3(gsets), dim3(256), 0, st, parts, odd == 2 ? low_pb + 1u : g.Lb + (odd ? 1u : 0u), g.bA, g.bB, wsum, direct,
+                       odd == 2 ? 1 : 0, prio);
     if (direct) {
       VDF_TRY_HIP(hipGetLastError());
       return Status{};
@@ -1335,7 +1361,7 @@
   } else {
     const RedGeom rg = red_geom((size_t)gsets * nbk, nbk);
     hipLaunchKernelGGL((k_reduce1<P>), dim3(gsets * rg.blocks_per_set), dim3(rg.block * 4), (size_t)rg.block * 128, st,
-                       bucket_acc, nbk, rg.seg, rg.threads_per_set, rg.blocks_per_set, partials, prio);
+                       bucket_acc, nbk, rg.seg, rg.threads_per_set, rg.blocks_per_set, partials, odd, prio);
     hipLaunchKernelGGL((k_reduce2<P>), dim3(gsets), dim3(256), 0, st, partials, rg.blocks_per_set, wsum, prio);
   }
   hipLaunchKernelGGL((k_final<P>), dim3(groups), dim3(64), 0, st, wsum, sets, c, bytes_of(d_out), prio);
@@ -1375,15 +1401,15 @@
   {
   KTimer kt(st, "msm_sort(5 launches)", 0.0);
   hipLaunchKernelGGL((k_part<SP, false>), dim3(p.nblkA), dim3(256), lds_bins, st, pg, is_mont ? 1 : 0, p.c, p.windows,
-                     p.sets, p.pb, p.fb, p.bins, p.chA, p.tstride, countsA, pstart, recsP, recsK, prio);
+                     p.sets, p.power_w, p.low_part ? 1 : 0, p.pb, p.fb, p.bins, p.chA, p.tstride, countsA, pstart, recsP, recsK, prio);
   hipLaunchKernelGGL(k_part_scan, dim3(p.bins), dim3(256), 0, st, countsA, p.bins, p.nblkA, pcount, heavy, heavy + 1 + nkeys + 2, prio);
   hipLaunchKernelGGL(k_scan_keys, dim3(1), dim3(1024), 0, st, pcount, p.bins, pstart, prio);
   if (tuning().sort_staged && p.bins <= PART_STAGE_BINS && p.windows <= 16)
     hipLaunchKernelGGL((k_part_staged<SP>), dim3(p.nblkA), dim3(256), 0, st, pg, is_mont ? 1 : 0, p.c, p.windows,
-                       p.sets, p.pb, p.fb, p.bins, p.chA, p.tstride, countsA, pstart, recsP, recsK, prio);
+                       p.sets, p.power_w, p.low_part ? 1 : 0, p.pb, p.fb, p.bins, p.chA, p.tstride, countsA, pstart, recsP, recsK, prio);
   else
     hipLaunchKernelGGL((k_part<SP, true>), dim3(p.nblkA), dim3(256), lds_bins, st, pg, is_mont ? 1 : 0, p.c, p.windows,
-                       p.sets, p.pb, p.fb, p.bins, p.chA, p.tstride, countsA, pstart, recsP, recsK, prio);
+                       p.sets, p.power_w, p.low_part ? 1 : 0, p.pb, p.fb, p.bins, p.chA, p.tstride, countsA, pstart, recsP, recsK, prio);
   if (tuning().sort_staged && nf <= 256)
     hipLaunchKernelGGL(k_fine_staged<4>, dim3(p.bins), dim3(1024), 0, st, recsP, recsK, pstart, p.bins, nf, bstart, sorted, bucket_acc, p.slots, p.Lfixed,
                        reinterpret_cast<uint32_t*>(base + w.tstart), prio);
@@ -1413,7 +1439,8 @@
                        heavy, tune.heavy_min, tune.giant_span, prio);
   hipLaunchKernelGGL((k_fixup_heavy<P>), dim3(16 * GIANT_PARTS), dim3(64), 0, st, bstart, nkeys, p.slots, p.Lfixed, bucket_acc, heads, heavy,
                      base + w.giant, prio);
-  if (!ext_bucket_acc) VDF_TRY(msm_tail_t<P>(p.c, p.sets, p.groups, p.nbk, bucket_acc, partials, wsum, d_out, st, prio));
+  if (!ext_bucket_acc) VDF_TRY(msm_tail_t<P>(p.c, p.sets, p.groups, p.nbk, bucket_acc, partials, wsum, d_out, st, prio, p.power_w ? 1 : 0, p.red_lb,
+                                           p.low_part ? (uint32_t)p.pb : 0u));
   if (ev) VDF_TRY_HIP(hipEventRecord(ev[3], st));
   VDF_TRY_HIP(hipGetLastError());
   return Status{};
diff --git a/vdf_amd/csrc/power_digits.h b/vdf_amd/csrc/power_digits.h
--- /dev/null
+++ b/vdf_amd/csrc/power_digits.h
@@ -0,0 +1,49 @@
+#pragma once
+#include <stdint.h>
+
+#if defined(__HIPCC__) || defined(__CUDACC__)
+#define VDF_POWER_HD __host__ __device__ __forceinline__
+#else
+#define VDF_POWER_HD inline
+#endif
+
+namespace vdf {
+
+constexpr int POWER_ROWS = 257;
+constexpr int POWER_MIN_WIDTH = 5, POWER_MAX_WIDTH = 20;
+VDF_POWER_HD int power_max_digits(int w) { return 256 / w + 1; }
+
+template <class Limbs>
+struct PowerDigitIter {
+  Limbs limb;
+  int w;
+  uint32_t pos = 0, carry = 0;
+  VDF_POWER_HD PowerDigitIter(Limbs lm, int width) : limb(lm), w(width) {}
+  VDF_POWER_HD bool next(uint32_t& position, uint32_t& digit) {
+    uint32_t p = pos;
+    for (;;) {
+      const uint32_t l = p >> 5;
+      if (l >= 8) {
+        if (!carry) return false;
+        break;
+      }
+      uint32_t word = limb((int)l);
+      if (carry) word = ~word;
+      word >>= (p & 31u);
+      if (word) { p += (uint32_t)__builtin_ctz(word); break; }
+      p = (l + 1) << 5;
+    }
+    const uint32_t l = p >> 5, sh = p & 31u;
+    const uint32_t lo = l < 8 ? limb((int)l) : 0u;
+    const uint32_t hi = l + 1 < 8 ? limb((int)l + 1) : 0u;
+    const uint64_t two = ((uint64_t)hi << 32) | lo;
+    const uint32_t raw = ((uint32_t)(two >> sh) & ((1u << w) - 1u)) | 1u;
+    position = p;
+    pos = p + (uint32_t)w;
+    if (raw >> (w - 1)) { carry = 1; digit = ((1u << w) - raw) | 0x80000000u; }
+    else { carry = 0; digit = raw; }
+    return true;
+  }
+};
+
+}
diff --git a/vdf_amd/hip.py b/vdf_amd/hip.py
--- a/vdf_amd/hip.py
+++ b/vdf_amd/hip.py
@@ -13,7 +13,8 @@
 class HipTuning(C.Structure):
     _fields_ = [("struct_size", C.c_uint32)] + [(k, C.c_int32) for k in (
         "msm_direct", "direct_priority", "direct_fused", "light_priority", "accumulate_fill", "accumulate_lds", "slice_len", "part_bits",
-        "reduction", "reduction_quads", "heavy_min", "giant_span", "nifs_lanes", "shim_cache", "nifs_fused", "fold_u128", "fixup_serial", "sort_staged", "glv")]
+        "reduction", "reduction_quads", "heavy_min", "giant_span", "nifs_lanes", "shim_cache", "nifs_fused", "fold_u128", "fixup_serial", "sort_staged", "glv",
+        "power_table", "power_width", "power_table_budget_gib")]
 
 
 def tuning_get() -> HipTuning:
@@ -98,6 +99,23 @@
     @property
     def window(self) -> int:
         return lib.vdf_bases_window(self.handle)
+
+    def precompute_powers(self, width: int = 0) -> None:
+        self.ctx._check(lib.vdf_bases_precompute_powers(self.ctx.handle, self.handle, width))
+
+    @property
+    def power_width(self) -> int:
+        return lib.vdf_bases_power_width(self.handle)
+
+    @property
+    def power_table_bytes(self) -> int:
+        return lib.vdf_bases_power_table_bytes(self.handle)
+
+    def download_power_row(self, row: int, offset: int = 0, n: Optional[int] = None) -> np.ndarray:
+        n = len(self) - offset if n is None else n
+        out = np.zeros((n, 8), dtype="<u8")
+        self.ctx._check(lib.vdf_bases_power_row_download(self.ctx.handle, self.handle, row, offset, n, _ptr(out)))
+        return out
 
     def precompute_digits(self, ranges, window_bits: int = 0) -> None:
         k = len(ranges)
```

After: 0.9245. -1.5%, worse.
